# manhofer/Line3D

Hardware: AMD Instinct MI355X
Metric: segment-pair affinities/s (higher is better)
Workload: dtype f32

## Files before the change

### include/line3d_amd.h

```cpp
#ifndef LINE3D_AMD_H
#define LINE3D_AMD_H

#include <stddef.h>
#include <stdint.h>

#ifdef __cplusplus
extern "C" {
#endif

#define L3D_OK 0
#define L3D_ERR_INVALID 1
#define L3D_ERR_HIP 2
#define L3D_ERR_NOMEM 3
#define L3D_ERR_NODEVICE 4
#define L3D_ERR_UNSUPPORTED 5

#define L3D_RDD_MAX_ITER 10
#define L3D_DEF_COLLINEARITY_S 2.0f

typedef struct l3d_ctx l3d_ctx;

typedef struct l3d_match {
    uint32_t segID1;
    uint32_t camID2;
// ... 38 lines not shown

int l3d_replicator_dynamics_diffusion(l3d_ctx* ctx, const l3d_edge* A, int nnz, int n, int iters, l3d_edge* out);

int l3d_similarity_coll3D_batch(l3d_ctx* ctx, const l3d_hypothesis* hyp, int n_hyp,
                                const int32_t* pairs, int n_pairs, float sigma_a, float* sim);

typedef struct l3d_affinity_input {
    int32_t n_views;
    const int32_t* seg_base;
    const int32_t* view_hyp_begin;
    int32_t n_hyp;
    const l3d_hypothesis* hyp;
    const float* score;
    const int32_t* hyp_dense;
    const int32_t* best;
    const int64_t* pot_start;
    const int32_t* pot_tgt;
    const int64_t* coll_start;
    const int32_t* coll_other;
    const float* coll_w;
    float sigma_a;
} l3d_affinity_input;
int l3d_affinity_fill(l3d_ctx* ctx, const l3d_affinity_input* in, l3d_edge** edges, int* n_edges, int32_t** node_hyp, int* n_nodes,
                      int* n_candidates);
int l3d_last_fill_counts(l3d_ctx* ctx, int64_t* n_candidates, int64_t* n_passed);

int l3d_clustering_edges(l3d_ctx* ctx, const l3d_edge* A, int nnz, int n_nodes, int perform_diffusion, int iters, l3d_edge* sorted_out);
int l3d_clustering_edges_grouped(l3d_ctx* ctx, const l3d_edge* A, int nnz, int n_nodes, int perform_diffusion, int iters, l3d_edge* sorted_out,
                                 int32_t** group_start, int* n_groups);
int l3d_perform_clustering_device(l3d_ctx* ctx, const l3d_edge* A, int nnz, int n_nodes, int perform_diffusion, int iters, float c, int32_t* labels,
                                  int* n_components);

int l3d_fit_clusters(l3d_ctx* ctx, const int32_t* group_start, int n_groups, const int32_t* member_hyp, const l3d_hypothesis* hyp,
                     const uint32_t* hyp_cam, int n_hyp, const double* Rinv, double scale_inv, const double* tneg,
                     int32_t** seg_count, double** segs, int* n_segs);
int l3d_fit_labelled_clusters(l3d_ctx* ctx, const int32_t* labels, const int32_t* node_hyp, int n_nodes, const l3d_hypothesis* hyp,
                              const uint32_t* hyp_cam, int n_hyp, const double* Rinv, double scale_inv, const double* tneg,
                              int32_t** group_start, int32_t** member_hyp, int* n_groups, int32_t** seg_count, double** segs, int* n_segs);

typedef struct l3d_refine_params { int32_t max_iterations; int32_t pad; double huber_px; } l3d_refine_params;
int l3d_refine_lines(l3d_ctx* ctx, const int32_t* group_start, int n_groups, const int32_t* member_cam, const float* member_seg, const double* member_pts,
                     const double* cameras, int n_cameras, const l3d_refine_params* params, double* line, double* rms_before, double* rms_after,
                     int32_t* iterations, int32_t* status, int32_t** seg_count, double** segs, int* n_segs);
int l3d_test_refine_host(const int32_t* group_start, int n_groups, const int32_t* member_cam, const float* member_seg, const double* member_pts,
                         const double* cameras, int n_cameras, const l3d_refine_params* params, double* line, double* rms_before, double* rms_after,
                         int32_t* iterations, int32_t* status, int32_t** seg_count, double** segs, int* n_segs);
const char* l3d_refine_last_error(void);


typedef struct l3d_chain_view {
    uint32_t view_id;
    const float* src_segs; int32_t S_src;
    const float* RtKinv_src; const float* C_src;
    const float* tgt_segs; int32_t n_tgt;
    const int32_t* offsets; int32_t N;
    const float* F; const float* RtKinv; const float* centers; const float* P;
    const int32_t* to_be_matched; int32_t n_tbm;
    const uint32_t* local2global;
    const int32_t* source_cam; const int32_t* source_index; int32_t n_sources;
    float sigma_p, sigma_a, spatial_k;
} l3d_chain_view;
typedef int (*l3d_chain_callback)(void* user, int index, int verified, const l3d_match* kept, int n_kept,
                                  const float* best_depths, int n_best, int n_candidates);
int l3d_match_chain(l3d_ctx* ctx, const l3d_chain_view* views, int n_views, l3d_chain_callback cb, void* user);

typedef struct l3d_dense_map {
    int32_t n_views;
    const uint32_t* view_ids;
    const int32_t* seg_base;
} l3d_dense_map;
typedef struct l3d_chain_summary {
    int32_t verified;
    int32_t n_kept;
    int64_t n_candidates;
    float median_depth;
    int32_t pad;
} l3d_chain_summary;
int l3d_match_chain_resident(l3d_ctx* ctx, const l3d_chain_view* views, int n_views, const l3d_dense_map* map,
                             l3d_chain_summary* summary, int64_t* n_pot);
int l3d_chain_kept_list(l3d_ctx* ctx, int index, l3d_match** out, int* n);
int l3d_chain_release_records(l3d_ctx* ctx);
int l3d_chain_records_digest(l3d_ctx* ctx, uint64_t* hash, int32_t* n_kept, int n);
int l3d_chain_products_get(l3d_ctx* ctx, int64_t* pot_start, int32_t* pot_tgt, l3d_match* best_match);

typedef struct l3d_view_geometry {
    double RtKinv[9];
    double C[3];
    float k_lower, k_upper;
    float median_depth;
    int32_t n_segments;
    const float* segments;
} l3d_view_geometry;
int l3d_products_hypotheses(l3d_ctx* ctx, const l3d_view_geometry* geometry, int n_views, int32_t* view_hyp_begin, int32_t** hyp_dense, int* n_hyp);
int l3d_affinity_fill_resident(l3d_ctx* ctx, const int64_t* coll_start, const int32_t* coll_other, const float* coll_w, int coll_changed,
                               float sigma_a, l3d_edge** edges, int* n_edges, int32_t** node_hyp, int* n_nodes, int* n_candidates);
int l3d_resident_edges_get(l3d_ctx* ctx, l3d_edge* out, int nnz);
int l3d_products_hypotheses_get(l3d_ctx* ctx, l3d_hypothesis* hyp, float* score);

typedef struct l3d_shard_chain l3d_shard_chain;
void* l3d_ctx_stream(l3d_ctx* ctx);
int l3d_shard_chain_open(l3d_ctx* ctx, const l3d_chain_view* views, int n_views, int rank, int world, int slot_records,
                         l3d_shard_chain** out, size_t* slot_bytes);
int l3d_shard_chain_enqueue(l3d_shard_chain* chain, int k, void* send_slot, const void* gathered_base);
int l3d_shard_chain_mark(l3d_shard_chain* chain, int k);
int l3d_shard_chain_fetch(l3d_shard_chain* chain, int k, l3d_chain_callback cb, void* user);
int l3d_shard_chain_close(l3d_shard_chain* chain);
typedef int (*l3d_exchange_fn)(void* user, int view, const void* send_slot, void* recv_block, size_t slot_bytes, int world, void* stream);
typedef struct l3d_rccl_link { void* comm; void* all_gather; } l3d_rccl_link;
int l3d_shard_chain_run(l3d_shard_chain* chain, l3d_exchange_fn exchange, void* exchange_user, l3d_chain_callback cb, void* cb_user);
int l3d_exchange_rccl(void* user, int view, const void* send_slot, void* recv_block, size_t slot_bytes, int world, void* stream);
int l3d_exchange_local(void* user, int view, const void* send_slot, void* recv_block, size_t slot_bytes, int world, void* stream);
int l3d_exchange_replay(void* user, int view, const void* send_slot, void* recv_block, size_t slot_bytes, int world, void* stream);
const void* l3d_shard_chain_gathered(l3d_shard_chain* chain);
typedef struct l3d_node_comm l3d_node_comm;
int l3d_node_comm_create(const int* devices, int n, l3d_node_comm** out);
void l3d_node_comm_destroy(l3d_node_comm* comm);
int l3d_node_comm_bind(l3d_node_comm* comm, int rank, void* stream);
void l3d_node_comm_abort(l3d_node_comm* comm);
int l3d_exchange_node(void* user, int view, const void* send_slot, void* recv_block, size_t slot_bytes, int world, void* stream);
int l3d_shard_chain_products(l3d_shard_chain* chain, const l3d_dense_map* map, l3d_chain_summary* summary, int64_t* n_pot);
int l3d_shard_chain_info(l3d_shard_chain* chain, size_t* cand_cap, int* slot_records, int* overflow_bits, int* max_candidates, int* max_kept);
long long l3d_shard_chain_arena_needed(l3d_shard_chain* chain);
int l3d_shard_chain_partition(l3d_shard_chain* chain, int own_begin, int own_end);
int l3d_partition_keep_views(const l3d_chain_view* views, int n_views, int own_begin, int own_end, unsigned char* keep, int* reach);
int l3d_turn_handover_plan(const l3d_chain_view* views, int n_views, int world, int32_t* out, int32_t* info);

int l3d_match_chain_blocks(l3d_ctx* ctx, const l3d_chain_view* views, int n_views, const l3d_dense_map* map, l3d_chain_summary* summary, int64_t* n_pot,
                           int rank, int world, int warmup_views, int window, l3d_exchange_fn exchange, void* exchange_user, int* verdict);

int l3d_match_chain_partition(l3d_ctx* ctx, const l3d_chain_view* views, int n_views, const l3d_dense_map* map, l3d_chain_summary* summary, int64_t* n_pot,
                              int rank, int world, int warmup_views, int window, l3d_exchange_fn exchange, void* exchange_user, int* verdict);
int l3d_partition_info(l3d_ctx* ctx, int info[10], int64_t* n_pot_all);
int l3d_affinity_fill_sharded(l3d_ctx* ctx, const int64_t* coll_start, const int32_t* coll_other, const float* coll_w, int coll_changed, float sigma_a,
                              l3d_exchange_fn exchange, void* exchange_user, int* n_edges, int32_t** node_hyp, int* n_nodes,
                              int64_t* n_candidates_all, int32_t* view_hyp_begin_global, int32_t** hyp_dense_global, int* n_hyp_global);

int l3d_register_segments(l3d_ctx* ctx, const float* segments, int n_segments);
int l3d_unregister_segments(l3d_ctx* ctx, const float* segments);
int l3d_register_segments_batch(l3d_ctx* ctx, const float* const* arrays, const int* n_segments, int n_arrays);

int l3d_set_verify_mode(l3d_ctx* ctx, int mode);
int l3d_set_pair_pretest(l3d_ctx* ctx, int mask);
int l3d_set_option(l3d_ctx* ctx, const char* name, int value);
int l3d_get_option(l3d_ctx* ctx, const char* name, int* value);
int l3d_set_verify_lds_budget(size_t bytes);
int l3d_set_chain_capacities(l3d_ctx* ctx, size_t cand_cap, size_t arena_cap);
int l3d_warm_up(l3d_ctx* ctx);
int l3d_reserve_hint(l3d_ctx* ctx, int n_dense, int n_views, int n_neighbors);
int l3d_profile_enable(l3d_ctx* ctx, int on);
int l3d_profile_only(l3d_ctx* ctx, const char* kernel);
int l3d_profile_reset(l3d_ctx* ctx);
int l3d_profile_get(l3d_ctx* ctx, const char* kernel, int64_t* launches, double* total_ms);
const char* l3d_profile_names(void);
int l3d_last_stats(l3d_ctx* ctx, double stats[4]);

int l3d_test_contract_math(l3d_ctx* ctx, const float* x, int n, float* out_expf, float* out_acosf, double* out_acos);
int l3d_test_sq_threshold(l3d_ctx* ctx, const float* u, int n, float* out_walk, float* out_closed);
int l3d_test_exclusive_sum(l3d_ctx* ctx, const int32_t* in, int n, int32_t* out);

typedef struct l3d_line3d l3d_line3d;

int l3d_line3d_create(int device, int matching_neighbors, float uncertainty_t_upper_2D, float uncertainty_t_lower_2D,
                      float sigma_p, float sigma_a, float min_baseline, int use_collinearity, int verbose,
                      l3d_line3d** out);
int l3d_line3d_create_node(const int* devices, int n_devices, int matching_neighbors, float uncertainty_t_upper_2D, float uncertainty_t_lower_2D,
                           float sigma_p, float sigma_a, float min_baseline, int use_collinearity, int verbose, l3d_line3d** out);
// ... 305 lines not shown
```

### line3d_amd/capi.py

```python
from __future__ import annotations

import ctypes as C
import os

import numpy as np

_HERE = os.path.dirname(os.path.abspath(__file__))
LIB_PATH = os.path.join(_HERE, "libline3d_amd.so")
if os.environ.get("L3D_LIBRARY"):
    LIB_PATH = os.environ["L3D_LIBRARY"]

MATCH_DTYPE = np.dtype([("segID1", "<u4"), ("camID2", "<u4"), ("segID2", "<u4"),
                        ("depths", "<f4", (4,)), ("confidence", "<f4")])
EDGE_DTYPE = np.dtype([("i", "<i4"), ("j", "<i4"), ("w", "<f4")])
HYP_DTYPE = np.dtype([("P1", "<f8", (3,)), ("P2", "<f8", (3,)), ("dir", "<f8", (3,)),
                      ("depth_p1", "<f4"), ("depth_p2", "<f4"),
                      ("k_lower", "<f4"), ("k_upper", "<f4"), ("median_depth", "<f4"), ("pad", "<u4")])
REGION_DTYPE = np.dtype([("minpix", "<u4"), ("n_used", "<i4"), ("steps", "<i4"), ("pts", "<i4"), ("alg", "<i4"), ("scored", "<i4"), ("accepted", "<i4"),
                         ("pad", "<i4"), ("hist_n", "<i4", (8,))] + [(k, "<f8") for k in ("cx", "cy", "x1", "y1", "x2", "y2", "width", "theta", "density",
                                                                "fx1", "fy1", "fx2", "fy2", "fwidth", "p", "nfa")])
assert MATCH_DTYPE.itemsize == 32 and EDGE_DTYPE.itemsize == 12 and HYP_DTYPE.itemsize == 96 and REGION_DTYPE.itemsize == 192

_lib = None
_lib_check = None
# ... 811 lines not shown
               "bucket": np.zeros((M, N, 2), np.uint8)}
        n, m = C.c_int(0), C.c_int(0)
        self._chk(self.lib.l3d_test_detect_pixel_stage(self.h, pix, C.c_int(w), C.c_int(h), C.c_int(ch), C.c_size_t(stride), C.c_int(nw), C.c_int(nh),
                                                       _p(out["grey"]), _p(out["img"]), _p(out["mod"]), _p(out["ang"]), _p(out["bucket"]),
                                                       C.byref(n), C.byref(m)))
        if (n.value, m.value) != (N, M):
            raise L3DError("scaled size (%d, %d), expected (%d, %d)" % (n.value, m.value, N, M))
        return out

    def test_detect_label(self, bucket, active):
        bucket = np.ascontiguousarray(bucket, dtype=np.uint8)
        active = np.ascontiguousarray(active, dtype=np.uint8)
        M, N = active.shape
        assert bucket.shape == (M, N, 2)
        parent, key = np.zeros((2, M, N), np.int32), np.zeros((M, N), np.uint32)
        self._chk(self.lib.l3d_test_detect_label(self.h, _p(bucket), _p(active), C.c_int(N), C.c_int(M), _p(parent), _p(key)))
        return parent, key

    def test_detect_regions(self, mod, ang, key, min_reg):
        mod, ang = np.ascontiguousarray(mod, dtype=np.float64), np.ascontiguousarray(ang, dtype=np.float64)
        key = np.ascontiguousarray(key, dtype=np.uint32)
        M, N = key.shape
        assert mod.shape == (M, N) and ang.shape == (M, N)
        rec, n = C.c_void_p(), C.c_int(0)
        active = np.zeros((M, N), np.uint8)
        self._chk(self.lib.l3d_test_detect_regions(self.h, C.c_int(N), C.c_int(M), _p(mod), _p(ang), _p(key), C.c_int(int(min_reg)),
                                                   C.byref(rec), C.byref(n), _p(active)))
        out = np.zeros(n.value, dtype=REGION_DTYPE)
        if n.value:
            C.memmove(out.ctypes.data, rec, n.value * REGION_DTYPE.itemsize)
        self.lib.l3d_free(rec)
        return out, active

    def test_detect_nfa(self, n, k, p, logNT):
        n, k = np.ascontiguousarray(n, dtype=np.int32), np.ascontiguousarray(k, dtype=np.int32)
        p = np.ascontiguousarray(p, dtype=np.float64)
        out = np.zeros(len(n))
        self._chk(self.lib.l3d_test_detect_nfa(self.h, _p(n), _p(k), _p(p), C.c_double(float(logNT)), C.c_int(len(n)), _p(out)))
        return out

    def test_verify_candidates(self, src_segs, tgt_segs, offsets, P, RtKinv_src, C_src, row_start, cand_meta, cand_depths, sigma_p, sigma_a, spatial_k,
                               path=0, gb=0, split_unit=0, mmax=0, wide_max=0, seg_order=None):
        f = lambda a: np.ascontiguousarray(a, dtype=np.float32)
        src_segs, tgt_segs, P, RtKinv_src, C_src, cand_depths = f(src_segs), f(tgt_segs), f(P), f(RtKinv_src), f(C_src), f(cand_depths)
        offsets, row_start = np.ascontiguousarray(offsets, dtype=np.int32), np.ascontiguousarray(row_start, dtype=np.int32)
        cand_meta = np.ascontiguousarray(cand_meta, dtype=np.uint32)
        S, N, R, n_tgt = len(src_segs), len(offsets), len(cand_meta), len(tgt_segs.reshape(-1, 4))
        assert row_start.shape == (S * N + 1,) and cand_meta.shape == (R, 2) and cand_depths.shape == (R, 4) and P.size == N * 12
        sel = VerifyPath(int(path), int(gb), int(split_unit), int(mmax), int(wide_max), 0, 0, 0, None)
        if seg_order is not None:
            seg_order = np.ascontiguousarray(seg_order, dtype=np.int32)
            assert seg_order.shape == (S,)
            sel.seg_order = seg_order.ctypes.data
        conf, kept, best = np.zeros(R, np.float32), np.zeros(S, np.int32), np.zeros((S, 2), np.float32)
        self._chk(self.lib.l3d_test_verify_candidates(self.h, C.c_int(S), C.c_int(N), _p(src_segs), _p(tgt_segs), C.c_int(n_tgt), _p(offsets), _p(P),
                                                      _p(RtKinv_src), _p(C_src), _p(row_start), _p(cand_meta), _p(cand_depths), C.c_int(R),
                                                      C.c_float(float(sigma_p)), C.c_float(float(sigma_a)), C.c_float(float(spatial_k)), C.byref(sel),
                                                      _p(conf), _p(kept), _p(best)))
        return conf, kept, best, int(sel.mmax_used), int(sel.kernels)

    def test_pair_candidates(self, src_segs, tgt_segs, offsets, F, RtKinv, centers, RtKinv_src, C_src, to_be_matched, path=0, pretest=3, spb=0,
                             seg_range=None, ray_tables=None, cand_cap=0, capacity=0):
        f = lambda a: np.ascontiguousarray(a, dtype=np.float32)
        src_segs, tgt_segs, F, RtKinv, centers, RtKinv_src, C_src = f(src_segs), f(tgt_segs), f(F), f(RtKinv), f(centers), f(RtKinv_src), f(C_src)
        offsets, tbm = np.ascontiguousarray(offsets, dtype=np.int32), np.ascontiguousarray(to_be_matched, dtype=np.int32)
        S, N, n_tgt = len(src_segs.reshape(-1, 4)), len(offsets), len(tgt_segs.reshape(-1, 4))
        assert F.size == N * 9 and RtKinv.size == N * 9 and centers.size == N * 3 and RtKinv_src.size == 9 and C_src.size == 3
        s0, s1 = (0, S) if seg_range is None else seg_range
        if ray_tables is None:
            ray_tables = 1 if path in (1, 2) else 0
        sel = PairPath(int(path), int(pretest), int(spb), int(s0), int(s1), int(ray_tables), int(cand_cap), int(capacity))
        out = dict(row_upper=np.zeros(S * N, np.int32), row_count=np.zeros(S * N, np.int32), row_start=np.zeros(S * N + 1, np.int32),
                   cand_meta=np.zeros((int(capacity), 2), np.uint32), cand_depths=np.zeros((int(capacity), 4), np.float32))
        try:
            self._chk(self.lib.l3d_test_pair_candidates(self.h, C.c_int(S), C.c_int(N), _p(src_segs), _p(tgt_segs), C.c_int(n_tgt), _p(offsets), _p(F), _p(RtKinv),
                                                        _p(centers), _p(RtKinv_src), _p(C_src), _p(tbm), C.c_int(len(tbm)), C.byref(sel), _p(out["row_upper"]),
                                                        _p(out["row_count"]), _p(out["row_start"]), _p(out["cand_meta"]), _p(out["cand_depths"])))
        except L3DError as e:
            e.needed = int(sel.needed)
            raise
        out.update(total=int(sel.total), largest=int(sel.largest), spb_used=int(sel.spb_used), overflow=int(sel.overflow), needed=int(sel.needed))
        return out

    def chain_products_get(self, n_dense: int, n_pot: int, slack: int = 0):
        pot_start = np.zeros(n_dense + 1, np.int64)
        pot_tgt = np.full(n_pot + slack, -1, np.int32)
        best = np.zeros(n_dense, dtype=MATCH_DTYPE)
        self._chk(self.lib.l3d_chain_products_get(self.h, _p(pot_start), _p(pot_tgt), _p(best)))
        return pot_start, pot_tgt, best

    def test_products(self, views, view_ids, seg_base, side_arrays=0, early_pairs=0, rows=None, held=None, slack=64, max_blocks=1024):
        n = len(views)
        arr, keep = (ChainView * max(1, n))(), []
        for k, v in enumerate(views):
            l2g = np.ascontiguousarray(v["l2g"], dtype=np.uint32)
            sc, si = np.ascontiguousarray(v["source_cam"], dtype=np.int32), np.ascontiguousarray(v["source_index"], dtype=np.int32)
            assert len(sc) == len(si)
            keep += [l2g, sc, si]
            e = arr[k]
            e.view_id, e.S_src, e.N, e.n_tbm, e.n_sources = int(v["id"]), int(v["S"]), len(l2g), int(v["n_tbm"]), len(sc)
            e.local2global, e.source_cam, e.source_index = l2g.ctypes.data, sc.ctypes.data, si.ctypes.data
        kept = [np.ascontiguousarray(v["kept"], dtype=MATCH_DTYPE) for v in views]
        n_kept = np.array([len(a) for a in kept], np.int32)
        kept_all = np.concatenate(kept) if n else np.zeros(0, MATCH_DTYPE)
        R = np.array([int(v["R"]) for v in views], np.int64)
        best = np.ascontiguousarray(np.concatenate([np.asarray(v["best"], np.float32).reshape(-1, 2) for v in views]), dtype=np.float32)
        bestpos = np.ascontiguousarray(np.concatenate([np.asarray(v["bestpos"], np.int32).reshape(-1) for v in views]), dtype=np.int32)
        assert len(best) == len(bestpos) == sum(int(v["S"]) for v in views)
        ids, sb = np.ascontiguousarray(view_ids, dtype=np.uint32), np.ascontiguousarray(seg_base, dtype=np.int32)
        assert len(sb) == len(ids) + 1
        dm = DenseMap(len(ids), ids.ctypes.data, sb.ctypes.data)
        blk = [np.full(max_blocks, -9, np.int32) for _ in range(3)]
        sel = ProductsPath()
        sel.side_arrays, sel.early_pairs = int(side_arrays), int(early_pairs)
        sel.dv0, sel.dv1 = (0, -1) if rows is None else (int(rows[0]), int(rows[1]))
        hb = None if held is None else np.ascontiguousarray(held, dtype=np.uint8)
        assert hb is None or len(hb) == n
        sel.held = None if hb is None else hb.ctypes.data
        sel.block_capacity = max_blocks
        sel.block_cap, sel.block_staged, sel.block_g = (b.ctypes.data for b in blk)
        summary = np.zeros(max(1, n), dtype=SUMMARY_DTYPE)
        n_pot = C.c_int64(0)
        self._chk(self.lib.l3d_test_products(self.h, arr, C.c_int(n), C.byref(dm), _p(kept_all), _p(n_kept), _p(R), _p(best), _p(bestpos), C.byref(sel),
                                             _p(summary), C.byref(n_pot)))
        nd = int(sb[-1])
        pot_start, pot_tgt, bm = self.chain_products_get(nd, n_pot.value, slack)
        nb = min(max_blocks, int(sel.n_blocks)) if sel.build == PROD_TRANSPOSED else 0
        report = dict(side_arrays_used=int(sel.side_arrays_used), build=int(sel.build), refused=int(sel.refused), n_blocks=int(sel.n_blocks),
                      max_touch=int(sel.max_touch), early_cap=int(sel.early_cap), early_g=int(sel.early_g),
                      block_cap=blk[0][:nb].tolist(), block_staged=blk[1][:nb].tolist(), block_g=blk[2][:nb].tolist())
        return dict(pot_start=pot_start, pot_tgt=pot_tgt, best=bm, n_pot=int(n_pot.value), summary=summary[:n], report=report)

    def compute_collinearity(self, segs, collin_s=2.0):
        segs = np.ascontiguousarray(segs, dtype=np.float32)
        oi, oj, ow = C.POINTER(C.c_int32)(), C.POINTER(C.c_int32)(), C.POINTER(C.c_float)()
        n = C.c_int(0)
        self._chk(self.lib.l3d_compute_collinearity(self.h, _p(segs), C.c_int(len(segs)), C.c_float(collin_s),
                                                    C.byref(oi), C.byref(oj), C.byref(ow), C.byref(n)))
        k = n.value
        i = np.ctypeslib.as_array(oi, (k,)).copy() if k else np.zeros(0, np.int32)
        j = np.ctypeslib.as_array(oj, (k,)).copy() if k else np.zeros(0, np.int32)
        w = np.ctypeslib.as_array(ow, (k,)).copy() if k else np.zeros(0, np.float32)
        for p in (oi, oj, ow):
            self.lib.l3d_free(p)
        return i, j, w

    def compute_collinearity_batch(self, seg_sets, collin_s=2.0):
        sets = [np.ascontiguousarray(s, dtype=np.float32).reshape(-1, 4) for s in seg_sets]
        n = len(sets)
        ptrs = (C.c_void_p * max(n, 1))(*[s.ctypes.data for s in sets])
        ns = np.array([len(s) for s in sets], np.int32)
        start = np.zeros(n + 1, np.int32)
        oi, oj, ow = C.POINTER(C.c_int32)(), C.POINTER(C.c_int32)(), C.POINTER(C.c_float)()
        self._chk(self.lib.l3d_compute_collinearity_batch(self.h, ptrs, _p(ns), C.c_int(n), C.c_float(collin_s),
                                                          C.byref(oi), C.byref(oj), C.byref(ow), _p(start)))
        total = int(start[n])
        i = np.ctypeslib.as_array(oi, (total,)).copy() if total else np.zeros(0, np.int32)
        j = np.ctypeslib.as_array(oj, (total,)).copy() if total else np.zeros(0, np.int32)
        w = np.ctypeslib.as_array(ow, (total,)).copy() if total else np.zeros(0, np.float32)
        for p in (oi, oj, ow):
            self.lib.l3d_free(p)
        return [(i[start[v]:start[v + 1]], j[start[v]:start[v + 1]], w[start[v]:start[v + 1]]) for v in range(n)]

    def compute_pairwise_matches(self, src_segs, RtKinv_src, C_src, tgt_segs, offsets, F, RtKinv, centers, P,
                                 to_be_matched, in_matches, local2global, k_upper, k_lower, sigma_p, sigma_a,
                                 spatial_k, median_depth=1.0, seg_range=None, want_best=False):
# ... 221 lines not shown
```

### line3d_amd/csrc/l3d_chain.hip

```cpp
#include <algorithm>
#include <condition_variable>
#include <deque>
#include <mutex>
#include <thread>
#include <vector>

#include "l3d_ctx.hpp"
#include "l3d_scan.hpp"
#include "l3d_kept.hpp"
#include "l3d_products.hpp"
#include "l3d_chain_common.hpp"
#include "l3d_chain_partition.hpp"
#include "l3d_runtable.hpp"

#ifndef L3D_AHEAD
#define L3D_AHEAD 4
#define L3D_S1AHEAD 8
#endif

using namespace l3d;

namespace l3d {

constexpr int kLongList = 262144;
// ... 494 lines not shown
            launch_early_transposes(c, reinterpret_cast<const EarlyView*>(PE.e_tab.as<int>() + (size_t)n_views * maxN * 2), early_next, k + 1 - early_next, maxN, early_maxSt, dres, cams, PE.e_cnt.as<int>(),
                                    PE.e_poff.as<unsigned>(), PE.e_boff.as<int>(), PE.e_E.as<unsigned>(), PE.e_T.as<unsigned>(), avg_run, sp);
            early_next = k + 1;
        }
        return L3D_OK;
    };

    const double t_loop0 = now_s();
    double kept_total = 0, t_cb = 0, t_wait = 0, t_d2h = 0;
    struct Item { int k; int verified; ChainResult r; };
    std::mutex mu;
    std::condition_variable cv_work, cv_idle;
    std::deque<Item> work;
    bool done = false, busy = false;
    int deliver_rc = L3D_OK;
    std::string deliver_err;
    std::thread deliverer([&]() {
        if (!cb) return;
        (void)hipSetDevice(c->device);
        for (;;) {
            Item it;
            {
                std::unique_lock<std::mutex> lk(mu);
                cv_work.wait(lk, [&]() { return done || !work.empty(); });
                if (work.empty()) return;
                it = work.front();
                work.pop_front();
                busy = true;
            }
            int rc = L3D_OK;
            std::string err;
            if (deliver_rc == L3D_OK) {
                const l3d_chain_view& v = views[it.k];
                const ViewDev& d = vd[(size_t)it.k];
                if (!it.verified) {
                    if (cb(user, it.k, 0, nullptr, 0, nullptr, 0, 0)) { rc = L3D_ERR_INVALID; err = "callback failed"; }
                } else {
                    const double td0 = now_s();
                    hipError_t e = hipSuccess;
                    l3d_match* kept_host = static_cast<l3d_match*>(c->pin_arena.alloc((size_t)it.r.n_kept * sizeof(Match) + 16, &e));
                    if (e == hipSuccess) e = c->ch_pin_best.reserve((size_t)v.S_src * 8 + 16);
                    if (e == hipSuccess && it.r.n_kept)
                        e = hipMemcpyAsync(kept_host, c->ch_kept.as<Match>() + it.r.kept_base, (size_t)it.r.n_kept * sizeof(Match), hipMemcpyDeviceToHost, c->copy_stream);
                    if (e == hipSuccess && v.S_src) e = hipMemcpyAsync(c->ch_pin_best.p, d.best, (size_t)v.S_src * 8, hipMemcpyDeviceToHost, c->copy_stream);
                    if (e == hipSuccess) e = hipStreamSynchronize(c->copy_stream);
                    if (e != hipSuccess) { rc = L3D_ERR_HIP; err = std::string("chain delivery, view ") + std::to_string(it.k) + ": " + hipGetErrorString(e); }
                    else {
                        float* best = c->ch_pin_best.as<float>();
                        int nb = 0;
                        if (it.r.R > 0)
                            for (int s = 0; s < v.S_src; ++s)
                                if (best[2 * s] != -1.0f) { best[2 * nb] = best[2 * s]; best[2 * nb + 1] = best[2 * s + 1]; ++nb; }
                        kept_total += it.r.n_kept;
                        const double tc0 = now_s();
                        t_d2h += tc0 - td0;
                        if (cb(user, it.k, 1, kept_host, it.r.n_kept, best, nb, it.r.R)) { rc = L3D_ERR_INVALID; err = "callback failed"; }
                        t_cb += now_s() - tc0;
                    }
                }
            }
            {
                std::lock_guard<std::mutex> lk(mu);
                if (rc && deliver_rc == L3D_OK) { deliver_rc = rc; deliver_err = err; }
                busy = false;
            }
            cv_idle.notify_all();
        }
    });
    auto hand_over = [&](int k, int verified, const ChainResult& r) {
        if (!cb) { if (verified) kept_total += r.n_kept; return; }
        { std::lock_guard<std::mutex> lk(mu); work.push_back(Item{ k, verified, r }); }
        cv_work.notify_one();
    };
    auto wait_delivered = [&]() {
        if (!cb) return;
        std::unique_lock<std::mutex> lk(mu);
        cv_idle.wait(lk, [&]() { return work.empty() && !busy; });
    };
    auto hip_ok = [&](hipError_t e, const char* what) {
        if (e == hipSuccess) return true;
        rc_final = fail(c, L3D_ERR_HIP, std::string(what) + ": " + hipGetErrorString(e));
        return false;
    };
    for (int k = 0; k < n_views && rc_final == L3D_OK; ++k) {
        while (k_enq < n_views && k_enq <= k + kAhead) { int rc = enqueue_view(k_enq); if (rc) { rc_final = rc; break; } ++k_enq; }
        if (rc_final) break;
        { std::lock_guard<std::mutex> lk(mu); if (deliver_rc) break; }
        const ViewDev& d = vd[(size_t)k];
        if (!d.verified) { hand_over(k, 0, ChainResult()); continue; }
        const double tw0 = now_s();
        if (!hip_ok(hipEventSynchronize(ev[(size_t)k]), "hipEventSynchronize")) break;
        t_wait += now_s() - tw0;
        const ChainResult r = hres[k];
        if (r.overflow) {
            if (!hip_ok(hipStreamSynchronize(st), "hipStreamSynchronize") || !hip_ok(hipStreamSynchronize(s1), "hipStreamSynchronize")) break;
            if (sp && !hip_ok(hipStreamSynchronize(sp), "hipStreamSynchronize")) break;
            const double t_restart0 = now_s();
            wait_delivered();
            if (r.overflow & 1) cand_cap = (size_t)r.R + (size_t)r.R / 4 + 65536;
            if (r.overflow & 2) {
                size_t new_cap = arena_cap * 2;
                const int n_pre = pre ? pre->k1 - pre->k0 : 0, done = k - k_begin + n_pre, span = k_end - k_begin + n_pre;
                if (done >= 4) {
                    const size_t proj = (size_t)((double)r.kept_base / done * span * (2 * done < span ? 1.5 : 1.15)) + 1048576;
                    new_cap = 2 * done < span ? std::max(new_cap, proj) : std::max(proj, arena_cap + arena_cap / 8);
                }
                const size_t need = (size_t)r.kept_base + (size_t)std::max(0, r.n_want) + 65536;
                new_cap = std::max(new_cap, need);
                {
                    size_t fr = 0, tot = 0;
                    if (hipMemGetInfo(&fr, &tot) == hipSuccess) {
                        if (c->opt.regrow_free_mb > 0) fr = std::min(fr, (size_t)c->opt.regrow_free_mb << 20);
                        const size_t per_rec = sizeof(Match) + 4 + (early && new_cap < 0x7ffffff0ull ? 4 : 0) + (map ? 8 : 0);
                        const size_t reserve = turn_room ? 0 : map ? (size_t)((1ll << 28) * 24) + ((size_t)1 << 30) : (size_t)512 << 20;
                        const size_t fits = turn_room ? turn_room : fr > reserve ? (fr - reserve) / per_rec : 0;
                        if (new_cap > fits) {
                            if (fits < need || fits <= arena_cap) {
                                rc_final = fail(c, L3D_ERR_NOMEM, "match_chain: the kept arena of " + std::to_string(arena_cap) + " records is full at view " + std::to_string(k) + " of " + std::to_string(n_views) + " (" +
                                                                      std::to_string((size_t)r.kept_base) + " records in use, the view keeps " + std::to_string(r.n_want) + ") and an arena of " +
                                                                      std::to_string(need) + " records does not fit beside it (room for " + std::to_string(fits) + " at " + std::to_string(per_rec) + " B per record, " +
                                                                      std::to_string(reserve >> 20) + " MB kept back; " + std::to_string(fr >> 20) + " of " + std::to_string(tot >> 20) +
                                                                      " MB free): l3d_set_chain_capacities sizes the arena up front");
                                break;
                            }
                            new_cap = fits;
                        }
                    }
                    (void)hipGetLastError();
                }
                void* np = nullptr;
                const double t_m0 = now_s();
                {
                    const hipError_t me = hipMalloc(&np, new_cap * sizeof(Match));
                    if (me != hipSuccess) {
                        size_t fr = 0, tot = 0;
                        (void)hipMemGetInfo(&fr, &tot);
                        rc_final = fail(c, L3D_ERR_NOMEM, "match_chain: growing the kept arena to " + std::to_string(new_cap * sizeof(Match) >> 20) + " MB at view " + std::to_string(k) + " of " + std::to_string(n_views) +
                                                          " (" + std::to_string((size_t)r.kept_base * sizeof(Match) >> 20) + " MB in use, " + std::to_string(fr >> 20) + " of " + std::to_string(tot >> 20) + " MB free): " + hipGetErrorString(me));
                        break;
                    }
                }
                const double t_m1 = now_s();
                if (!hip_ok(hipMemcpy(np, c->ch_kept.p, (size_t)r.kept_base * sizeof(Match), hipMemcpyDeviceToDevice), "hipMemcpy")) break;
                const double t_m2 = now_s();
                (void)hipFree(c->ch_kept.p);
                if (c->opt.timing) fprintf(stderr, "[l3d match_chain]   arena of %zu MB: hipMalloc %.2f ms, copy of %zu MB %.2f ms, hipFree of the old one %.2f ms\n", new_cap * sizeof(Match) >> 20, (t_m1 - t_m0) * 1e3,
                                           (size_t)r.kept_base * sizeof(Match) >> 20, (t_m2 - t_m1) * 1e3, (now_s() - t_m2) * 1e3);
                c->ch_kept.p = np; c->ch_kept.cap = new_cap * sizeof(Match);
                {
                    void* nc = nullptr;
                    if (!hip_ok(hipMalloc(&nc, new_cap * 4 + 64), "hipMalloc (side words of the kept arena)")) break;
                    if (!hip_ok(hipMemcpy(nc, c->ch_keptcam.p, (size_t)r.kept_base * 4, hipMemcpyDeviceToDevice), "hipMemcpy")) { (void)hipFree(nc); break; }
                    (void)hipFree(c->ch_keptcam.p);
                    c->ch_keptcam.p = nc; c->ch_keptcam.cap = new_cap * 4 + 64;
                }
                if (early && new_cap < 0x7ffffff0ull) {
                    void* ne = nullptr;
                    if (!hip_ok(hipMalloc(&ne, new_cap * 4 + 64), "hipMalloc (transposed entries of the kept arena)")) break;
                    if (!hip_ok(hipMemcpy(ne, PE.e_E.p, (size_t)r.kept_base * 4, hipMemcpyDeviceToDevice), "hipMemcpy")) { (void)hipFree(ne); break; }
                    (void)hipFree(PE.e_E.p);
                    PE.e_E.p = ne; PE.e_E.cap = new_cap * 4 + 64;
                }
                arena_cap = new_cap;
            }
            { int rc = reserve_caps(); if (rc) { rc_final = rc; break; } }
            if (c->opt.timing) fprintf(stderr, "[l3d match_chain] view %d of %d overflowed (%d): candidates %zu, arena %zu records; regrown in %.2f ms, %.2f ms into the loop\n", k, n_views, r.overflow, cand_cap, arena_cap,
                                       (now_s() - t_restart0) * 1e3, (now_s() - t_loop0) * 1e3);
            for (int j = k; j < k_p1; ++j) {
                if (!vd[(size_t)j].verified || views[j].S_src == 0) continue;
                if (j < k_enq) {
                    if (!hip_ok(hipMemsetAsync(vd[(size_t)j].rowcnt, 0, (size_t)views[j].S_src * views[j].N * 4, st), "hipMemsetAsync")) break;
                    if (!fused_rows) launch_row_count(pair_args(j), vd[(size_t)j].rowcnt, st);
                }
                enqueue_fillA(j, st);
            }
            if (rc_final) break;
            k_enq = k;
            early_next = std::min(early_next, k);
            --k;
            continue;
        }
        raw_sum += r.R;
        kept_seen += r.n_kept; views_seen += 1;
        hand_over(k, 1, r);
    }
    { std::lock_guard<std::mutex> lk(mu); done = true; }
    cv_work.notify_one();
    deliverer.join();
    if (rc_final == L3D_OK && deliver_rc) rc_final = fail(c, deliver_rc, deliver_err);
    const double t_prod0 = now_s();
    if (rc_final == L3D_OK && map) {
        std::vector<ProdChainView> pv((size_t)n_views);
        for (int k = 0; k < n_views; ++k) pv[(size_t)k] = ProdChainView{ vd[(size_t)k].verified ? vd[(size_t)k].best : nullptr, vd[(size_t)k].verified ? vd[(size_t)k].bestpos : nullptr, vd[(size_t)k].verified ? 1 : 0,
                                                                         vd[(size_t)k].verified ? vd[(size_t)k].rt : nullptr };
        ProdEarly pe;
        const bool early_done = early && arena_cap < 0x7ffffff0ull;
        if (early_done) {
            if (early_next < n_views) {
                const double avg_run = views_seen > 0 ? kept_seen / views_seen / std::max(1.0, (double)L.maxS * std::max(1, maxN)) : 1.0;
                launch_early_transposes(c, reinterpret_cast<const EarlyView*>(PE.e_tab.as<int>() + (size_t)n_views * maxN * 2), early_next, n_views - early_next, maxN, early_maxSt, c->ch_res.as<ChainResult>(),
                                        c->ch_keptcam.as<unsigned>(), PE.e_cnt.as<int>(), PE.e_poff.as<unsigned>(), PE.e_boff.as<int>(), PE.e_E.as<unsigned>(), PE.e_T.as<unsigned>(), avg_run, st);
                early_next = n_views;
            }
            hipEvent_t e = get_local_event(c);
            (void)hipEventRecord(e, sp);
            (void)hipStreamWaitEvent(st, e, 0);
            put_local_event(c, e);
            pe.pcnt_kq = PE.e_cnt.as<int>(); pe.poff_kq = PE.e_poff.as<unsigned>(); pe.boff = PE.e_boff.as<int>(); pe.E = PE.e_E.as<unsigned>();
            pe.boff_off_host = PE.e_boff_off.data(); pe.maxN = maxN;
        }
        rc_final = build_products(c, views, n_views, pv.data(), hres, map, summary, n_pot, 0, -1, nullptr, c->ch_keptcam.as<unsigned>(), early_done ? &pe : nullptr);
    }
    if (c->opt.timing)
        fprintf(stderr, "[l3d match_chain] setup %.2f ms | enqueue + watch loop %.2f ms (waiting: view results %.2f, stage-1 statistics %.2f) | delivery thread: d2h %.2f, callback %.2f\n",
                (t_loop0 - t_setup0) * 1e3, (t_prod0 - t_loop0) * 1e3, t_wait * 1e3, t_ev1 * 1e3, t_d2h * 1e3, t_cb * 1e3);
    if (c->opt.timing && map) fprintf(stderr, "[l3d match_chain] products on the device %.2f ms\n", (now_s() - t_prod0) * 1e3);
    const double t_tail0 = now_s();
    (void)hipStreamSynchronize(s1);
    if (sp) (void)hipStreamSynchronize(sp);
    (void)hipStreamSynchronize(st);
    if (c->opt.timing) fprintf(stderr, "[l3d match_chain] hipSetDevice %.3f ms, final syncs %.3f ms\n", (t_setup0 - t_enter) * 1e3, (now_s() - t_tail0) * 1e3);
    for (hipEvent_t e : ev) { if (cb) put_event(c, e); else put_local_event(c, e); }
    for (hipEvent_t e : ev1) put_local_event(c, e);
    c->stats[1] = raw_sum;
    c->stats[3] = kept_total;
    if (rc_final == L3D_OK && !c->test_cand_cap && !c->test_arena_cap) {
        c->chain_seen_views = n_views; c->chain_seen_pairs = pairs; c->chain_seen_cand_cap = cand_cap; c->chain_seen_arena_cap = arena_cap; c->chain_seen_kept = kept_seen;
    }
    return rc_final;
}

extern "C" int l3d_match_chain(l3d_ctx* c, const l3d_chain_view* views, int n_views, l3d_chain_callback cb, void* user)
{
    if (c && n_views > 0 && !cb) return fail(c, L3D_ERR_INVALID, "l3d_match_chain: bad argument");
    return run_chain(c, views, n_views, cb, user, nullptr, nullptr, nullptr);
}

extern "C" int l3d_match_chain_resident(l3d_ctx* c, const l3d_chain_view* views, int n_views, const l3d_dense_map* map, l3d_chain_summary* summary, int64_t* n_pot)
{
    if (!c) return L3D_ERR_INVALID;
    if (!map || !map->view_ids || !map->seg_base || map->n_views < 0 || (n_views > 0 && !summary)) return fail(c, L3D_ERR_INVALID, "l3d_match_chain_resident: bad argument");
    if (n_pot) *n_pot = 0;
    return run_chain(c, views, n_views, nullptr, nullptr, map, summary, n_pot);
}

void l3d::warm_chain() { touch_kernel(reinterpret_cast<const void*>(&k_exist_count)); }
```

### line3d_amd/csrc/l3d_ctx.hpp

```cpp
#pragma once

#include <algorithm>
#include <chrono>
#include <cstdio>
#include <cstdlib>
#include <cstring>
#include <map>
#include <mutex>
#include <string>
#include <unordered_map>
#include <vector>

#include "../../include/line3d_amd.h"
#include "l3d_kernels.hpp"
#include "l3d_options.hpp"

namespace l3d {

struct DevBuf {
    void* p = nullptr;
    size_t cap = 0;
    hipError_t reserve(size_t bytes)
    {
        if (bytes <= cap) return hipSuccess;
        if (p) { hipError_t e = hipFree(p); p = nullptr; cap = 0; if (e != hipSuccess) return e; }
        size_t want = bytes + bytes / 4 + 256;
        hipError_t e = hipMalloc(&p, want);
        if (e == hipSuccess) cap = want;
        return e;
    }
    hipError_t reserve_exact(size_t bytes)
    {
        if (bytes <= cap) return hipSuccess;
        if (p) { hipError_t e = hipFree(p); p = nullptr; cap = 0; if (e != hipSuccess) return e; }
        hipError_t e = hipMalloc(&p, bytes + 256);
        if (e == hipSuccess) cap = bytes + 256;
        return e;
    }
    template <class T> T* as() const { return reinterpret_cast<T*>(p); }
    void release() { if (p) (void)hipFree(p); p = nullptr; cap = 0; }
};

struct PinBuf {
    void* p = nullptr;
    size_t cap = 0;
    unsigned flags = hipHostMallocDefault;
    hipError_t reserve(size_t bytes)
    {
        if (bytes <= cap) return hipSuccess;
        if (p) { (void)hipHostFree(p); p = nullptr; cap = 0; }
        size_t want = bytes + bytes / 2 + 4096;
        hipError_t e = hipHostMalloc(&p, want, flags);
        if (e == hipSuccess) cap = want;
        return e;
    }
    template <class T> T* as() const { return reinterpret_cast<T*>(p); }
    void release() { if (p) (void)hipHostFree(p); p = nullptr; cap = 0; }
};

struct PinArena {
    static constexpr size_t kChunk = 64u << 20;
    std::vector<PinBuf> chunks;
    size_t cur = 0, used = 0;
    void reset() { cur = 0; used = 0; }
    void* alloc(size_t bytes, hipError_t* err)
    {
        *err = hipSuccess;
        bytes = (bytes + 255) & ~(size_t)255;
        for (;;) {
            if (cur < chunks.size()) {
                if (used + bytes <= chunks[cur].cap) { void* r = static_cast<char*>(chunks[cur].p) + used; used += bytes; return r; }
                ++cur; used = 0;
                continue;
            }
            chunks.emplace_back();
            *err = chunks.back().reserve(std::max(bytes, kChunk));
            if (*err != hipSuccess) { chunks.pop_back(); return nullptr; }
        }
    }
    void release() { for (auto& b : chunks) b.release(); chunks.clear(); reset(); }
};

struct ProductsPart {
    bool active = false;
    int rank = 0, world = 1;
    int own_dv0 = 0, own_dv1 = 0;
    int row_dv0 = 0, row_dv1 = 0;
    int held_dv0 = 0, held_dv1 = 0;
    long long n_pot_all = 0;
    int recovery_rounds = 0;
    int blocks_rerun = 0;
};

struct ProductsReport {
    int build = 0;
    int refused = 0;
    int n_blocks = 0, max_touch = 0;
    int early_cap = -1, early_g = -1;
    std::vector<int> block_cap, block_staged, block_g;
};

struct Products {
    bool valid = false, hyp_valid = false;
    ProductsPart part;
    ProductsReport report;
    int n_dense = 0, n_views_all = 0, n_chain = 0, n_hyp = 0;
    long long n_pot = 0, total_kept = 0;
    DevBuf keys, keys2, flag, pos, tmp, pot_start, pot_tgt, best_ref, median, tables, ttab, rowstage, tstage;
    DevBuf e_cnt, e_poff, e_boff, e_E, e_T, e_tab;
    std::vector<int> e_boff_off;
    DevBuf geo, hyp_of, score, hyp_dense, best_hyp, coll, aux;
    long long coll_n = 0;
    unsigned long long coll_sig = 0;
    std::vector<int> seg_base;
    std::vector<unsigned> view_ids;
    std::vector<l3d::ChainResult> res;
    std::vector<int> chain_view;
    std::vector<char> chain_verified;
    std::vector<int> view_hyp_begin;
    std::vector<std::vector<int>> early_src_index, early_src_cam;
    std::vector<unsigned> chain_view_id;
    void release()
    {
        DevBuf* b[] = { &keys, &keys2, &flag, &pos, &tmp, &pot_start, &pot_tgt, &best_ref, &median, &tables, &ttab, &rowstage, &tstage, &e_cnt, &e_poff, &e_boff, &e_E, &e_T, &e_tab, &geo, &hyp_of, &score, &hyp_dense, &best_hyp, &coll, &aux };
        for (DevBuf* x : b) x->release();
        valid = hyp_valid = false; coll_n = 0; coll_sig = 0;
    }
};

struct FillPart { int h0 = 0, h1 = 0; unsigned long long pos_base = 0; const int* loc2glob = nullptr; int assume_symmetric = 0; };

struct DetectBufs {
    DevBuf lens;
    DevBuf rflags, smask, valid;
    DevBuf vgrey, vaux, vimg, vdef;
    DevBuf pixels, undist, grey, aux, img, mod, ang, bucket, active, parent, size, count, keys, keys2, vals, vals2, flag, pos, start, tmp, cand, ckeys, ckeys2, cvals, cvals2, cimg, cimg2, prm, out, ktab, scal;
    DevBuf jcoef, jplanes;
    PinBuf jstage;
    DevBuf ingest;
    std::vector<unsigned char> ingest_host;
    hipEvent_t dev_event = nullptr;
    int tab_w = 0, tab_h = 0;
    int vdef_n = 0, vdef_m = 0;
    void release()
    {
        for (DevBuf* x : all()) x->release();
        jstage.release();
        if (dev_event) { (void)hipEventDestroy(dev_event); dev_event = nullptr; }
        tab_w = tab_h = 0;
        vdef_n = vdef_m = 0;
    }
    size_t held()
    {
        size_t n = 0;
        for (DevBuf* x : all()) n += x->cap;
        return n;
    }
    std::vector<DevBuf*> all()
    {
        return { &pixels, &undist, &grey, &aux, &img, &mod, &ang, &bucket, &active, &parent, &size, &count, &keys, &keys2, &vals, &vals2, &flag, &pos, &start, &tmp, &cand, &ckeys, &ckeys2, &cvals, &cvals2, &cimg, &cimg2, &prm, &out, &ktab, &scal, &jcoef, &jplanes, &ingest, &lens, &rflags, &smask, &valid, &vgrey, &vaux, &vimg, &vdef };
    }
};

struct ProfEntry {
    std::vector<std::pair<hipEvent_t, hipEvent_t>> pending;
    int64_t launches = 0;
    double ms = 0.0;
};

}

struct l3d_ctx {
    int device = 0;
    l3d::Options opt;
    hipStream_t stream = nullptr;
    hipStream_t copy_stream = nullptr;
    hipStream_t prod_stream = nullptr;
    hipStream_t stage1_stream = nullptr;
    std::string err;
    std::mutex err_mu;
    l3d::DevBuf src_segs, tgt_segs, tables, tbm, l2g, exist, mask, rowcnt, row_start, cand_meta, cand_depths, cand_conf;
    l3d::DevBuf kept_cnt, kept_start, best, kept, scal, stamps, vw_scratch;
    l3d::PinBuf pin_tab, pin_ex, pin_scal, pin_best, pin_kept;
    l3d::DevBuf ch_tables, ch_mask, ch_rowcnt, ch_cursor, ch_best, ch_kept, ch_keptcam, ch_res, ch_flags, ch_send, ch_gathered, ch_stage, ch_rowA, ch_ringA_meta, ch_ringA_depths, ch_segorder, ch_rays, ch_rt, ch_rtinfo, ch_rtjobs, ch_existpart;
    l3d::PinBuf ch_pin_tables, ch_pin_res, ch_pin_kept, ch_pin_best;
    l3d::DevBuf ch_hdr;
    l3d::DevBuf ch_bestpos;
    l3d::Products products;
    l3d::DetectBufs det;
    std::vector<l3d::RayJob> ray_jobs;
    l3d::PinArena pin_arena;
    std::vector<int> h_cnt;
    int mmax_seen = 0;
    l3d::DevBuf vw_bstart, vw_segstate;
    size_t part_arena_seen = 0;
    bool turn_share = false;
    bool fill_collective_only = false;
    void (*fill_gate)(void*, int) = nullptr;
    void* fill_gate_user = nullptr;
    size_t turn_arena_room = 0;
    bool records_released = false;
    std::vector<int> shard_view_kept;
    size_t test_cand_cap = 0, test_arena_cap = 0;
    int chain_seen_views = 0; double chain_seen_pairs = 0; size_t chain_seen_cand_cap = 0, chain_seen_arena_cap = 0; double chain_seen_kept = 0;
    unsigned long long* pair_dbg = nullptr;
    int wedge_pretest = 3;
    int verify_mode = 0;
    l3d::DevBuf g0, g1, g2, g3, g4, g5, g6, g7;
// ... 129 lines not shown
```

### line3d_amd/csrc/l3d_products.hip

```cpp
#include "l3d_sort.hpp"

#include <algorithm>
#include <vector>

#include "l3d_products.hpp"
#include "l3d_linalg.hpp"
#include "l3d_unproject.hpp"
#include "l3d_runtable.hpp"

using namespace l3d;

namespace l3d {

struct ProdView {
    long long kept_base;
    int n_kept, R;
    int dense_base, S;
    int early, pad;
    const int* bestpos;
    const float2* best;
};
struct ProdBlock {
    int d0, d1;
    long long slots;
// ... 322 lines not shown
    const ChainResult r = res[v.k];
    const int St = v.St[q];
    unsigned long long off = r.kept_base;
    for (int j = 0; j < q; ++j) off += (unsigned)pcnt_kq[(size_t)v.k * maxN + j];
    if (threadIdx.x == 0) poff_kq[(size_t)v.k * maxN + q] = (unsigned)off;
    if (r.overflow || r.n_kept == 0 || St <= 0) return;
    pair_transpose_wg(qt_arena + r.kept_base, v.rt + (size_t)q * v.S, v.rt + (size_t)(q + 1) * v.S, v.S, St, g, boff + v.boff_off[q], E + off, T ? T + off : nullptr, cap, s_h, s_w, &s_kb);
}

template <int MODE>
__global__ __launch_bounds__(256) void k_prod_early_rt(const ProdView* __restrict__ pv, const ProdViewQ* __restrict__ vq, const ProdSrc* __restrict__ ps, const int* __restrict__ ps_slot,
                                                       const int* __restrict__ src_list, int d0, int d1, int* __restrict__ cnt, const int* __restrict__ bstart,
                                                       unsigned* __restrict__ ent, unsigned long long* __restrict__ best_ref, int* __restrict__ list_len)
{
    const int q = src_list ? src_list[blockIdx.y] : (int)blockIdx.y;
    const ProdSrc e = ps[q];
    const int slot = ps_slot[q];
    if (slot < 0 || (MODE != 0 && e.alias_base < 0)) return;
    const ProdView v = pv[e.view], s = pv[e.src];
    const ProdViewQ sq = vq[e.src];
    if (!sq.rt || s.n_kept == 0) return;
    const int* r0 = sq.rt + (size_t)slot * s.S;
    const int* r1 = r0 + s.S;
    constexpr int g = 16;
    const int grp = threadIdx.x / g, gl = threadIdx.x % g, ngrp = 256 / g;
    int n_mine = 0;
    for (int sg = blockIdx.x * ngrp + grp; sg < s.S; sg += gridDim.x * ngrp) {
        const int ra = r0[sg], rb = r1[sg];
        for (int i = ra + gl; i < rb; i += g) {
            const unsigned w = sq.qt[i];
            const int u = (int)(w & 0xffffu);
            if (MODE == 0) {
                ++n_mine;
                if (u < v.S && !e.pad) atomicMin(&best_ref[v.dense_base + u], ((unsigned long long)e.rank << 40) | (unsigned long long)(s.kept_base + i));
            } else if (u < v.S && sg < e.alias_S) {
                const int ai = v.dense_base + u, di = e.alias_base + sg;
                if (ai >= d0 && ai < d1) {
                    if (MODE == 1) atomicAdd(&cnt[ai - d0], 1);
                    else ent[bstart[ai - d0] + atomicSub(&cnt[ai - d0], 1) - 1] = (unsigned)di;
                }
                if (di >= d0 && di < d1) {
                    if (MODE == 1) atomicAdd(&cnt[di - d0], 1);
                    else ent[bstart[di - d0] + atomicSub(&cnt[di - d0], 1) - 1] = (unsigned)ai;
                }
            }
        }
    }
    if (MODE == 0) {
        for (int d = 32; d > 0; d >>= 1) n_mine += __shfl_down(n_mine, d);
        if ((threadIdx.x & 63) == 0 && n_mine) atomicAdd(&list_len[e.view], n_mine);
    }
}

template <bool SCATTER>
__global__ __launch_bounds__(256) void k_prodt_early(const Match* __restrict__ arena, const ProdView* __restrict__ pv, const ProdSrc* __restrict__ ps,
                                                     const int* __restrict__ src_list, const unsigned* __restrict__ chain_view_id, int d0, int d1, int* __restrict__ cnt,
                                                     const int* __restrict__ bstart, unsigned* __restrict__ ent)
{
    const int q = src_list[blockIdx.y];
    const ProdSrc e = ps[q];
    if (e.alias_base < 0) return;
    const ProdView v = pv[e.view], s = pv[e.src];
    const unsigned vid = chain_view_id[e.view];
    for (int i = blockIdx.x * 256 + threadIdx.x; i < s.n_kept; i += gridDim.x * 256) {
        const Match r = arena[s.kept_base + i];
        if (r.camID2 != vid || (int)r.segID2 >= v.S || (int)r.segID1 >= e.alias_S) continue;
        const int ai = v.dense_base + (int)r.segID2, di = e.alias_base + (int)r.segID1;
        if (ai >= d0 && ai < d1) {
            if (!SCATTER) atomicAdd(&cnt[ai - d0], 1);
            else ent[bstart[ai - d0] + atomicSub(&cnt[ai - d0], 1) - 1] = (unsigned)di;
        }
        if (di >= d0 && di < d1) {
            if (!SCATTER) atomicAdd(&cnt[di - d0], 1);
            else ent[bstart[di - d0] + atomicSub(&cnt[di - d0], 1) - 1] = (unsigned)ai;
        }
    }
}

template <bool WRITE>
__global__ __launch_bounds__(256) void k_prodv_rows(const ProdRowView* __restrict__ rv, int x0, int d0, const ProdViewQ* __restrict__ vq, const ProdTouch* __restrict__ tl,
                                                    const ProdPair* __restrict__ pairs, const int* __restrict__ poff, const int* __restrict__ boff, const unsigned* __restrict__ E,
                                                    const int* __restrict__ bstart, const unsigned* __restrict__ ent, int* __restrict__ ucnt, const int* __restrict__ ustart,
                                                    long long base, int* __restrict__ pot_tgt, int* __restrict__ stage,
                                                    const unsigned* __restrict__ poff_kq, int maxN)
{
    constexpr int kWords = 512;
    __shared__ unsigned s_bm[4][kWords];
    const int wave = threadIdx.x >> 6, lane = threadIdx.x & 63;
    const ProdRowView v = rv[x0 + blockIdx.y];
    const int u = blockIdx.x * 4 + wave;
    if (u >= v.S) return;
    unsigned* bm = s_bm[wave];
    const int row = v.dense_base + u - d0;
    const unsigned* fq = nullptr;
    const int* frt = nullptr;
    if (v.own_k >= 0) { const ProdViewQ o = vq[v.own_k]; if (o.rt) { fq = o.qt; frt = o.rt; } }
    const int e0 = bstart ? bstart[row] : 0, ne = bstart ? bstart[row + 1] - e0 : 0;
    int total = 0;
    long long o = WRITE ? base + ustart[row] : 0;
    if (!WRITE && stage && lane == 63) stage[(size_t)row * 64 + 63] = 0;
    if (WRITE && stage && stage[(size_t)row * 64 + 63] == -2) {
        const int n = ustart[row + 1] - ustart[row];
        if (lane < n) pot_tgt[o + lane] = stage[(size_t)row * 64 + lane];
        return;
    }
    for (int t0 = v.t0; t0 < v.t1; t0 += 64) {
        const int j = t0 + lane;
        ProdTouch e;
        e.y_base = 0; e.y_S = 0; e.fq = -1; e.pair = -1;
        int f_a = 0, f_n = 0, b_a = 0, b_n = 0;
        if (j < v.t1) {
            e = tl[j];
            if (e.fq >= 0 && frt) { f_a = frt[(size_t)e.fq * v.S + u]; f_n = frt[(size_t)(e.fq + 1) * v.S + u] - f_a; }
            if (e.pair >= 0) {
                const ProdPair pr = pairs[e.pair];
                const int* bo = boff + pr.off_off;
                const int a = bo[u];
                b_n = bo[u + 1] - a;
                b_a = (poff_kq ? (int)poff_kq[(size_t)pr.k * maxN + pr.q] : poff[e.pair]) + a;
            }
        }
        const int cnt = min(64, v.t1 - t0);
        if (v.t1 - v.t0 <= 64) {
            const int mine = f_n + b_n;
            int incl = mine;
            for (int d = 1; d < 64; d <<= 1) { const int x = __shfl_up(incl, d); if (lane >= d) incl += x; }
            const int excl = incl - mine, tot = __shfl(incl, 63);
            if (tot + ne <= 64) {
                int id = 0x7fffffff;
                int l = 0;
                for (int step = 32; step > 0; step >>= 1) { const int cand = l + step; const int ex = __shfl(excl, cand & 63); if (cand < 64 && ex <= lane) l = cand; }
                const int off = lane - __shfl(excl, l), ofn = __shfl(f_n, l), ofa = __shfl(f_a, l), oba = __shfl(b_a, l), oyS = __shfl(e.y_S, l), oyb = __shfl(e.y_base, l);
                if (lane < tot) {
                    const unsigned t = off < ofn ? (fq[ofa + off] & 0xffffu) : E[oba + off - ofn];
                    if ((int)t < oyS) id = oyb + (int)t;
                } else if (lane < tot + ne) id = (int)ent[e0 + lane - tot];
                int rank = 0;
                for (int k = 0; k < 64; ++k) { const int other = __shfl(id, k); rank += (other < id || (other == id && k < lane)) ? 1 : 0; }
                const int sorted = __builtin_amdgcn_ds_permute(rank << 2, id);
                const int before = __shfl_up(sorted, 1);
                const bool keep = sorted != 0x7fffffff && (lane == 0 || before != sorted);
                const unsigned long long km = __ballot(keep);
                if (!WRITE) {
                    const int n = __popcll(km);
                    if (lane == 0) ucnt[row] = n;
                    if (stage && n < 64) {
                        if (keep) stage[(size_t)row * 64 + __popcll(km & ((1ull << lane) - 1ull))] = sorted;
                        if (lane == 63) stage[(size_t)row * 64 + 63] = -2;
                    }
                }
                else if (keep) pot_tgt[o + __popcll(km & ((1ull << lane) - 1ull))] = sorted;
                return;
            }
        }
        for (int k = 0; k < cnt; ++k) {
            const int fn = __shfl(f_n, k), bn = __shfl(b_n, k);
            if (fn + bn + ne == 0) continue;
            const int fa = __shfl(f_a, k), ba = __shfl(b_a, k), yS = __shfl(e.y_S, k), yb = __shfl(e.y_base, k);
            const int nw = (yS + 31) >> 5;
            for (int w = lane; w < nw; w += 64) bm[w] = 0u;
            __builtin_amdgcn_fence(__ATOMIC_SEQ_CST, "workgroup");
            __builtin_amdgcn_wave_barrier();
            for (int i = lane; i < fn; i += 64) { const unsigned t = fq[fa + i] & 0xffffu; if ((int)t < yS) atomicOr(&bm[t >> 5], 1u << (t & 31u)); }
            for (int i = lane; i < bn; i += 64) { const unsigned t = E[ba + i]; if ((int)t < yS) atomicOr(&bm[t >> 5], 1u << (t & 31u)); }
            for (int i = lane; i < ne; i += 64) { const unsigned t = ent[e0 + i] - (unsigned)yb; if (t < (unsigned)yS) atomicOr(&bm[t >> 5], 1u << (t & 31u)); }
            __builtin_amdgcn_fence(__ATOMIC_SEQ_CST, "workgroup");
            __builtin_amdgcn_wave_barrier();
            if (!WRITE) {
                for (int w = lane; w < nw; w += 64) total += __popc(bm[w]);
            } else {
                for (int wb = 0; wb < nw; wb += 64) {
                    const int w = wb + lane;
                    unsigned word = w < nw ? bm[w] : 0u;
                    if (__ballot(word != 0u) == 0ull) continue;
                    const int pc = __popc(word);
                    int incl = pc;
                    for (int d = 1; d < 64; d <<= 1) { const int x = __shfl_up(incl, d); if (lane >= d) incl += x; }
                    long long p = o + (incl - pc);
                    while (word) { const int bit = __ffs(word) - 1; pot_tgt[p++] = yb + (w << 5) + bit; word &= word - 1u; }
                    o += __shfl(incl, 63);
                }
            }
            __builtin_amdgcn_fence(__ATOMIC_SEQ_CST, "workgroup");
            __builtin_amdgcn_wave_barrier();
        }
    }
    if (!WRITE) {
        for (int d = 32; d > 0; d >>= 1) total += __shfl_down(total, d);
        if (lane == 0) ucnt[row] = total;
    }
}

__global__ __launch_bounds__(256) void k_prodt_row_starts(const int* __restrict__ ustart, int rows, long long base, long long* __restrict__ pot_start_at)
{
    const int r = blockIdx.x * 256 + threadIdx.x;
    if (r <= rows) pot_start_at[r] = base + ustart[r];
}

}

namespace {

int bits_for(int n) { int b = 1; while ((1ll << b) <= (long long)n) ++b; return b; }

}

void l3d::launch_prod_shift_rows(const long long* piece, long long n_rows, long long base, long long* pot_start_at, hipStream_t st)
{
    if (n_rows > 0) hipLaunchKernelGGL(k_prod_shift_rows, dim3((unsigned)((n_rows + 255) / 256)), dim3(256), 0, st, piece, n_rows, base, pot_start_at);
}

void l3d::launch_early_transposes(l3d_ctx* c, const EarlyView* views_dev, int k0, int nb, int maxN, int maxSt, const ChainResult* res,
                                  const unsigned* qt_arena, int* pcnt_kq, unsigned* poff_kq, int* boff, unsigned* E, unsigned* T, double avg_run, hipStream_t st)
{
    if (maxN <= 0 || nb <= 0) return;
    int g = 1;
    while (g < 64 && g < avg_run / 4.0) g <<= 1;
    if (c->opt.prod_pair_g >= 0) g = c->opt.prod_pair_g;
    int cap = 0;
    if (T) {
        cap = 12288;
        while (cap > 1024 && ((size_t)maxSt + 2 + 2 * (size_t)cap) * 4 > 64 * 1024) cap -= 1024;
        if (((size_t)maxSt + 2 + 2 * (size_t)cap) * 4 > 64 * 1024) cap = 0;
    }
    c->products.report.early_cap = cap; c->products.report.early_g = g;
    ProfScope p(c, "prod_keys", st);
    hipLaunchKernelGGL(k_prode_counts, dim3((unsigned)maxN, (unsigned)nb), dim3(256), 0, st, views_dev, k0, maxN, res, pcnt_kq);
    hipLaunchKernelGGL(k_prode_transpose, dim3((unsigned)maxN, (unsigned)nb), dim3(kPairThreads), ((size_t)maxSt + 2 + 2 * (size_t)cap) * 4, st, views_dev, k0, maxN, res, qt_arena, (const int*)pcnt_kq, poff_kq, g,
                       boff, E, cap ? T : (unsigned*)nullptr, cap);
}

int l3d::build_products(l3d_ctx* c, const l3d_chain_view* views, int n_views, const ProdChainView* pvh, const ChainResult* hres,
                        const l3d_dense_map* map, l3d_chain_summary* summary, int64_t* n_pot_out, int dv0, int dv1, const char* held, const unsigned* qt_arena, const ProdEarly* early)
{
    Products& P = c->products;
    P.valid = false; P.hyp_valid = false;
    c->records_released = false;
    ProductsReport& rep = P.report;
    rep.build = 0; rep.refused = 0; rep.n_blocks = 0; rep.max_touch = 0;
    rep.block_cap.clear(); rep.block_staged.clear(); rep.block_g.clear();
    hipStream_t st = c->stream;
    const int nv = map->n_views;
    if (nv <= 0) return fail(c, L3D_ERR_INVALID, "products: empty dense map");
    for (int i = 0; i < nv; ++i) {
        if (map->seg_base[i + 1] < map->seg_base[i] || (i && map->view_ids[i] <= map->view_ids[i - 1]) || map->seg_base[0] != 0)
            return fail(c, L3D_ERR_INVALID, "products: the dense map must ascend");
    }
    const int nd = map->seg_base[nv];
    if (nd <= 0) return fail(c, L3D_ERR_INVALID, "products: no segments");
    const bool partial = dv1 >= 0;
    if (!partial) { dv0 = 0; dv1 = nv; }
    if (dv0 < 0 || dv1 > nv || dv0 > dv1) return fail(c, L3D_ERR_INVALID, "products: bad view range");
    P.seg_base.assign(map->seg_base, map->seg_base + nv + 1);
    P.view_ids.assign(map->view_ids, map->view_ids + nv);
    P.res.assign(hres, hres + n_views);
    P.n_dense = nd; P.n_views_all = nv; P.n_chain = n_views;
    P.chain_view.assign((size_t)n_views, -1);
    P.chain_verified.assign((size_t)n_views, 0);
    for (int k = 0; k < n_views; ++k) P.chain_verified[(size_t)k] = pvh[k].verified ? 1 : 0;
    P.chain_view_id.resize((size_t)n_views);
    P.early_src_index.assign((size_t)n_views, {}); P.early_src_cam.assign((size_t)n_views, {});
    auto view_of = [&](unsigned id) { auto it = std::lower_bound(P.view_ids.begin(), P.view_ids.end(), id); return it != P.view_ids.end() && *it == id ? (int)(it - P.view_ids.begin()) : -1; };

    std::vector<ProdView> pv((size_t)n_views);
    std::vector<ProdSrc> ps;
    std::vector<int> ps_alias_view;
    long long total_kept = 0, early_slots = 0;
    for (int k = 0; k < n_views; ++k) if (pvh[k].verified) total_kept = std::max(total_kept, (long long)hres[k].kept_base + hres[k].n_kept);
    if (total_kept > kBestIndexMask) return fail(c, L3D_ERR_UNSUPPORTED, "products: " + std::to_string(total_kept) + " kept matches in the arena -- best-match references hold 40-bit positions");
    int max_kept = 0, maxS = 1;
    for (int k = 0; k < n_views; ++k) {
        const l3d_chain_view& v = views[k];
        const int vi = view_of(v.view_id);
        if (vi < 0 || P.seg_base[(size_t)vi + 1] - P.seg_base[(size_t)vi] != v.S_src) return fail(c, L3D_ERR_INVALID, "products: a chain view is missing from the dense map");
        P.chain_view[(size_t)k] = vi; P.chain_view_id[(size_t)k] = v.view_id;
        ProdView& o = pv[(size_t)k];
        o.kept_base = pvh[k].verified ? hres[k].kept_base : 0; o.n_kept = pvh[k].verified ? hres[k].n_kept : 0; o.R = pvh[k].verified ? hres[k].R : 0;
        o.dense_base = P.seg_base[(size_t)vi]; o.S = v.S_src; o.early = pvh[k].verified ? 0 : 1; o.pad = 0;
        o.bestpos = pvh[k].bestpos; o.best = pvh[k].best;
        max_kept = std::max(max_kept, o.n_kept); maxS = std::max(maxS, o.S);
        if (!pvh[k].verified) {
            P.early_src_index[(size_t)k].assign(v.source_index, v.source_index + v.n_sources);
            P.early_src_cam[(size_t)k].assign(v.source_cam, v.source_cam + v.n_sources);
            for (int q = 0; q < v.n_sources; ++q) {
                const int si = v.source_index[q];
                if (si < 0 || si >= k || !pvh[si].verified) continue;
                ProdSrc e;
                e.view = k; e.src = si; e.rank = q; e.pad = 0;
                const int av = view_of((unsigned)v.source_cam[q]);
                e.alias_base = av >= 0 ? P.seg_base[(size_t)av] : -1; e.alias_S = av >= 0 ? P.seg_base[(size_t)av + 1] - P.seg_base[(size_t)av] : 0;
                e.out_off = 0;
                early_slots += 2 * (long long)hres[si].n_kept;
                ps.push_back(e);
                ps_alias_view.push_back(av);
            }
        }
    }
    const long long slots_all = 2 * total_kept + early_slots;
    const int nb = bits_for(nd);
    P.total_kept = total_kept;

    std::vector<std::vector<int>> touch_view((size_t)nv), touch_src((size_t)nv);
    for (int k = 0; k < n_views; ++k) {
        if (!pvh[k].verified || hres[k].n_kept == 0) continue;
        touch_view[(size_t)P.chain_view[(size_t)k]].push_back(k);
        for (int q = 0; q < views[k].N; ++q) {
            const int t = view_of(views[k].local2global[q]);
            if (t >= 0 && t != P.chain_view[(size_t)k]) touch_view[(size_t)t].push_back(k);
        }
    }
    for (size_t q = 0; q < ps.size(); ++q) {
        if (hres[ps[q].src].n_kept == 0) continue;
        const int a = P.chain_view[(size_t)ps[q].view], b = ps_alias_view[q];
        touch_src[(size_t)a].push_back((int)q);
        if (b >= 0 && b != a) touch_src[(size_t)b].push_back((int)q);
    }
    long long budget = 1ll << 28;
    if (c->opt.prod_block_keys > 0) budget = c->opt.prod_block_keys;
    else if (slots_all > budget) {
        size_t fr = 0, tot = 0;
        if (hipMemGetInfo(&fr, &tot) == hipSuccess) budget = std::max(budget, std::min<long long>((long long)(fr / 4 / 24), (1ll << 30) - 64));
    }
    std::vector<ProdBlock> blocks;
    std::vector<long long> off_tab;
    auto plan_blocks = [&]() -> int {
        blocks.clear(); off_tab.clear();
        std::vector<int> mark_v((size_t)n_views, -1), mark_s(ps.size(), -1);
        int x = dv0;
        while (x < dv1) {
            const int bi = (int)blocks.size();
            ProdBlock B;
            B.d0 = P.seg_base[(size_t)x]; B.slots = 0;
            B.off_view = off_tab.size();
            off_tab.resize(off_tab.size() + (size_t)n_views + ps.size(), -1);
            B.off_src = B.off_view + (size_t)n_views;
            int x1 = x;
            for (; x1 < dv1; ++x1) {
                long long add = 0;
                for (int k : touch_view[(size_t)x1]) if (mark_v[(size_t)k] != bi) add += 2 * (long long)hres[k].n_kept;
                for (int q : touch_src[(size_t)x1]) if (mark_s[(size_t)q] != bi) add += 2 * (long long)hres[ps[(size_t)q].src].n_kept;
                if (x1 > x && B.slots + add > budget) break;
                for (int k : touch_view[(size_t)x1]) if (mark_v[(size_t)k] != bi) { mark_v[(size_t)k] = bi; off_tab[B.off_view + (size_t)k] = B.slots; B.slots += 2 * (long long)hres[k].n_kept; }
                for (int q : touch_src[(size_t)x1]) if (mark_s[(size_t)q] != bi) { mark_s[(size_t)q] = bi; off_tab[B.off_src + (size_t)q] = B.slots; B.slots += 2 * (long long)hres[ps[(size_t)q].src].n_kept; }
            }
            B.d1 = P.seg_base[(size_t)x1];
            if (B.slots > 0x7ffffff0ll) return fail(c, L3D_ERR_UNSUPPORTED, "products: one view and its neighbours hold more than 2^30 kept matches");
            blocks.push_back(B);
            x = x1;
        }
        return L3D_OK;
    };
    if (int rc = plan_blocks()) return rc;
    long long max_slots = 0;
    for (const ProdBlock& B : blocks) max_slots = std::max(max_slots, B.slots);
    long long n_keys_max = max_slots + 1;

    auto al = [](size_t b) { return (b + 255) & ~(size_t)255; };
    const size_t o_pv = 0, o_ps = o_pv + al(pv.size() * sizeof(ProdView)), o_ids = o_ps + al(ps.size() * sizeof(ProdSrc) + 16),
                 o_sb = o_ids + al((size_t)nv * 4), o_cv = o_sb + al((size_t)(nv + 1) * 4), o_off = o_cv + al((size_t)n_views * 4), o_evq = o_off + al(off_tab.size() * 8 + 16),
                 o_slot = o_evq + al((size_t)n_views * sizeof(ProdViewQ) + 16), tab_total = o_slot + al(ps.size() * 4 + 16);
    HIPCHK(c, P.tables.reserve(tab_total));
    bool native_rt = qt_arena != nullptr && c->opt.prod_transpose != 0;
    for (int k = 0; k < n_views; ++k) if (pvh[k].verified && hres[k].n_kept > 0 && !pvh[k].rt) native_rt = false;
    std::vector<ProdViewQ> evq((size_t)n_views);
    for (int k = 0; k < n_views; ++k) {
        const bool has = native_rt && pvh[k].verified && hres[k].n_kept > 0;
        evq[(size_t)k] = ProdViewQ{ has ? qt_arena + hres[k].kept_base : nullptr, has ? pvh[k].rt : nullptr, 0, views[k].N };
    }
    std::vector<int> ps_slot(ps.size() + 1, -1);
    for (size_t q = 0; q < ps.size(); ++q) {
        const l3d_chain_view& sv = views[ps[q].src];
        for (int j = 0; j < sv.N; ++j) if (sv.local2global[j] == P.chain_view_id[(size_t)ps[q].view]) { ps_slot[q] = j; break; }
    }
    char* tb = P.tables.as<char>();
    std::vector<char> tblob(tab_total);
    {
        auto put = [&](size_t off, const void* src, size_t bytes) { if (bytes) memcpy(tblob.data() + off, src, bytes); };
        put(o_pv, pv.data(), pv.size() * sizeof(ProdView)); put(o_ps, ps.data(), ps.size() * sizeof(ProdSrc)); put(o_ids, P.view_ids.data(), (size_t)nv * 4);
        put(o_sb, P.seg_base.data(), (size_t)(nv + 1) * 4); put(o_cv, P.chain_view_id.data(), (size_t)n_views * 4); put(o_off, off_tab.data(), off_tab.size() * 8);
        put(o_evq, evq.data(), evq.size() * sizeof(ProdViewQ)); put(o_slot, ps_slot.data(), ps_slot.size() * 4);
    }
    HIPCHK(c, hipMemcpyAsync(tb, tblob.data(), tblob.size(), hipMemcpyHostToDevice, st));
    const ProdView* dpv = reinterpret_cast<const ProdView*>(tb + o_pv);
    const ProdSrc* dps = reinterpret_cast<const ProdSrc*>(tb + o_ps);
    const unsigned* dids = reinterpret_cast<const unsigned*>(tb + o_ids);
    const int* dsb = reinterpret_cast<const int*>(tb + o_sb);
    const unsigned* dcv = reinterpret_cast<const unsigned*>(tb + o_cv);
    const long long* doff = reinterpret_cast<const long long*>(tb + o_off);
    const ProdViewQ* devq = reinterpret_cast<const ProdViewQ*>(tb + o_evq);
    const int* dslot = reinterpret_cast<const int*>(tb + o_slot);

    const double t_res0 = now_s();
    HIPCHK(c, P.pot_start.reserve(((size_t)nd + 2) * 8));
    HIPCHK(c, P.best_ref.reserve((size_t)nd * 8 + 64));
    HIPCHK(c, P.median.reserve((size_t)n_views * 8 + 64));
    if (c->opt.timing) fprintf(stderr, "[l3d products] %zu block(s) of up to %lld keys, table of up to %lld entries: buffers reserved in %.2f ms\n", blocks.size(), n_keys_max, slots_all, (now_s() - t_res0) * 1e3);
    int* d_list_len = reinterpret_cast<int*>(P.median.as<float>() + n_views);
    HIPCHK(c, hipMemsetAsync(d_list_len, 0, (size_t)n_views * 4, st));
    const Match* arena = c->ch_kept.as<Match>();
    HIPCHK(c, hipMemsetAsync(P.best_ref.p, 0xff, (size_t)nd * 8, st));
    const unsigned gx = (unsigned)std::max(1, std::min(512, (max_kept + 1023) / 1024));
    {
        ProfScope p(c, "prod_keys", st);
        if (!ps.empty() && native_rt)
            hipLaunchKernelGGL(HIP_KERNEL_NAME(k_prod_early_rt<0>), dim3((unsigned)std::max(1, std::min(256, (maxS + 15) / 16)), (unsigned)ps.size()), dim3(256), 0, st, dpv, devq, dps, dslot, (const int*)nullptr, 0, 0,
                               (int*)nullptr, (const int*)nullptr, (unsigned*)nullptr, P.best_ref.as<unsigned long long>(), d_list_len);
        else if (!ps.empty()) hipLaunchKernelGGL(k_prod_keys_early, dim3(gx, (unsigned)ps.size()), dim3(256), 0, st, arena, dpv, dps, (const long long*)nullptr, dcv, nb, 0, 0,
                                                 (unsigned long long*)nullptr, P.best_ref.as<unsigned long long>(), d_list_len);
        hipLaunchKernelGGL(k_prod_best, dim3((maxS + 255) / 256, n_views), dim3(256), 0, st, dpv, P.best_ref.as<long long>());
        hipLaunchKernelGGL(k_prod_median, dim3(n_views), dim3(256), 0, st, dpv, P.median.as<float>());
    }
    constexpr int kSortInstead = -12345;
    auto transposed = [&](long long& n_pot_out) -> int {
        const double t_t0 = now_s();
        auto seg_count = [&](int x) { return P.seg_base[(size_t)x + 1] - P.seg_base[(size_t)x]; };
        for (int x = dv0; x < dv1; ++x) if (seg_count(x) > 16000) { rep.refused = 1; return kSortInstead; }
        const bool rebuild = !native_rt;
        const bool use_early = early && !rebuild && early->E && early->boff && early->poff_kq;
        std::vector<int> nbv_off((size_t)n_views + 1, 0), nbv;
        for (int k = 0; k < n_views; ++k) {
            nbv_off[(size_t)k] = (int)nbv.size();
            if (pvh[k].verified) for (int q = 0; q < views[k].N; ++q) nbv.push_back(view_of(views[k].local2global[q]));
        }
        nbv_off[(size_t)n_views] = (int)nbv.size();
        std::vector<std::vector<int>> T((size_t)nv);
        for (int x = 0; x < nv; ++x) T[(size_t)x].reserve(32);
        for (int k = 0; k < n_views; ++k) {
            if (!pvh[k].verified) continue;
            const int vi = P.chain_view[(size_t)k];
            for (int q = 0; q < views[k].N; ++q) {
                const int t = nbv[(size_t)nbv_off[(size_t)k] + q];
                if (t >= 0) { T[(size_t)vi].push_back(t); T[(size_t)t].push_back(vi); }
            }
        }
        for (size_t q = 0; q < ps.size(); ++q) {
            const int a = P.chain_view[(size_t)ps[q].view], b = ps_alias_view[q];
            if (b >= 0) { T[(size_t)a].push_back(b); T[(size_t)b].push_back(a); }
        }
        for (int x = 0; x < nv; ++x) { std::vector<int>& t = T[(size_t)x]; std::sort(t.begin(), t.end()); t.erase(std::unique(t.begin(), t.end()), t.end()); }
        std::vector<int> nb_off((size_t)n_views, 0);
        std::vector<ProdNbQ> nbt;
        std::vector<unsigned> ids_sorted;
        std::vector<int> qs_sorted;
        std::vector<std::vector<ProdPair>> pairs_of((size_t)nv);
        std::vector<int> own_k((size_t)nv, -1);
        std::vector<std::pair<unsigned, int>> byid;
        nbt.reserve(nbv.size()); ids_sorted.reserve(nbv.size()); qs_sorted.reserve(nbv.size());
        for (int k = 0; k < n_views; ++k) {
            nb_off[(size_t)k] = (int)nbt.size();
            if (!pvh[k].verified) continue;
            const int vi = P.chain_view[(size_t)k], N = views[k].N;
            if (hres[k].n_kept > 0) own_k[(size_t)vi] = k;
            byid.clear();
            for (int q = 0; q < N; ++q) {
                const int t = nbv[(size_t)nbv_off[(size_t)k] + q];
                nbt.push_back(ProdNbQ{ t >= 0 ? P.seg_base[(size_t)t] : -1, t >= 0 ? seg_count(t) : 0 });
                byid.push_back({ views[k].local2global[q], q });
                if (t >= 0 && hres[k].n_kept > 0) pairs_of[(size_t)t].push_back(ProdPair{ k, q, 0, 0 });
            }
            std::sort(byid.begin(), byid.end());
            for (auto& e : byid) { ids_sorted.push_back(e.first); qs_sorted.push_back(e.second); }
        }
        std::vector<ProdRowView> rv((size_t)nv);
        std::vector<ProdPair> pairs;
        std::vector<ProdTouch> tl;
        pairs.reserve(nbv.size()); tl.reserve(2 * nbv.size() + 64);
        int max_touch = 0;
        for (int x = 0; x < nv; ++x) {
            ProdRowView& r = rv[(size_t)x];
            r.dense_base = P.seg_base[(size_t)x]; r.S = seg_count(x); r.own_k = own_k[(size_t)x]; r.t0 = r.t1 = 0; r.pad = 0;
            if (x < dv0 || x >= dv1) continue;
            const int pair0 = (int)pairs.size();
            for (const ProdPair& pr : pairs_of[(size_t)x]) pairs.push_back(pr);
            r.t0 = (int)tl.size();
            for (int y : T[(size_t)x]) {
                ProdTouch e;
                e.y_base = P.seg_base[(size_t)y]; e.y_S = seg_count(y); e.fq = -1; e.pair = -1;
                if (r.own_k >= 0) for (int q = 0; q < views[r.own_k].N; ++q) if (nbv[(size_t)nbv_off[(size_t)r.own_k] + q] == y) { e.fq = q; break; }
                for (int p = pair0; p < (int)pairs.size(); ++p) if (P.chain_view[(size_t)pairs[(size_t)p].k] == y) { e.pair = p; break; }
                tl.push_back(e);
            }
            r.t1 = (int)tl.size();
            max_touch = std::max(max_touch, r.t1 - r.t0);
        }
        rep.max_touch = max_touch;
        std::vector<int> pair_begin((size_t)nv + 1, 0);
        {
            int p = 0;
            for (int x = 0; x < nv; ++x) { pair_begin[(size_t)x] = p; if (x >= dv0 && x < dv1) p += (int)pairs_of[(size_t)x].size(); }
            pair_begin[(size_t)nv] = p;
        }
        struct TBlock { int x0, x1; size_t item0, n_items, src0, n_srcs; long long rec_n, rt_n, boff_n, early_n; int maxS, pair0, pair1; };
        std::vector<TBlock> tblocks;
        std::vector<int> items;
        std::vector<int> srcs;
        const long long t_budget = c->opt.prod_block_keys > 0 ? c->opt.prod_block_keys : (1ll << 30) - 64;
        {
            std::vector<int> mark_v((size_t)n_views, -1), mark_s(ps.size(), -1);
            int x = dv0;
            while (x < dv1) {
                const int bi = (int)tblocks.size();
                TBlock B;
                B.x0 = x; B.item0 = items.size(); B.src0 = srcs.size(); B.rec_n = 0; B.rt_n = 0; B.boff_n = 0; B.early_n = 0; B.maxS = 1; B.pair0 = pair_begin[(size_t)x];
                int x1 = x;
                for (; x1 < dv1; ++x1) {
                    long long add = 0;
                    for (int k : touch_view[(size_t)x1]) if (mark_v[(size_t)k] != bi) add += hres[k].n_kept;
                    for (int q : touch_src[(size_t)x1]) if (mark_s[(size_t)q] != bi) add += 2 * (long long)hres[ps[(size_t)q].src].n_kept;
                    if (x1 > x && B.rec_n + B.early_n + add > t_budget) break;
                    for (int k : touch_view[(size_t)x1]) if (mark_v[(size_t)k] != bi) {
                        mark_v[(size_t)k] = bi; items.push_back(k); B.rec_n += hres[k].n_kept; B.rt_n += ((long long)views[k].N + 1) * views[k].S_src;
                    }
                    for (int q : touch_src[(size_t)x1]) if (mark_s[(size_t)q] != bi) { mark_s[(size_t)q] = bi; srcs.push_back(q); B.early_n += 2 * (long long)hres[ps[(size_t)q].src].n_kept; }
                    B.maxS = std::max(B.maxS, seg_count(x1));
                    for (int p = pair_begin[(size_t)x1]; p < pair_begin[(size_t)x1 + 1]; ++p) {
                        if (use_early) { pairs[(size_t)p].off_off = early->boff_off_host[(size_t)pairs[(size_t)p].k * early->maxN + pairs[(size_t)p].q]; continue; }
                        pairs[(size_t)p].off_off = (int)B.boff_n; B.boff_n += seg_count(x1) + 1;
                    }
                }
                B.x1 = x1; B.n_items = items.size() - B.item0; B.n_srcs = srcs.size() - B.src0; B.pair1 = pair_begin[(size_t)x1];
                if (B.rec_n > 0x7ffffff0ll || B.early_n > 0x7ffffff0ll || B.boff_n > 0x7ffffff0ll || B.rt_n > 0x7ffffff0ll)
                    return fail(c, L3D_ERR_UNSUPPORTED, "products: one view and its neighbours hold more than 2^31 kept matches");
                tblocks.push_back(B);
                x = x1;
            }
        }
        long long max_rec = 0, max_rt = 0, max_boff = 0, max_early = 0;
        int max_rows = 0, max_pairs = 0;
        for (const TBlock& B : tblocks) {
            max_rec = std::max(max_rec, B.rec_n); max_rt = std::max(max_rt, B.rt_n); max_boff = std::max(max_boff, B.boff_n); max_early = std::max(max_early, B.early_n);
            max_rows = std::max(max_rows, P.seg_base[(size_t)B.x1] - P.seg_base[(size_t)B.x0]); max_pairs = std::max(max_pairs, B.pair1 - B.pair0);
        }
        std::vector<ProdViewQ> vqh((size_t)n_views);
        for (int k = 0; k < n_views; ++k) {
            ProdViewQ& o = vqh[(size_t)k];
            o.nb_off = nb_off[(size_t)k]; o.N = views[k].N;
            const bool has = pvh[k].verified && hres[k].n_kept > 0 && !rebuild;
            o.qt = has ? qt_arena + hres[k].kept_base : nullptr; o.rt = has ? pvh[k].rt : nullptr;
        }
        const size_t q_vq = 0, q_nb = q_vq + al(vqh.size() * sizeof(ProdViewQ) + 16), q_ids = q_nb + al(nbt.size() * sizeof(ProdNbQ) + 16), q_qs = q_ids + al(ids_sorted.size() * 4 + 16),
                     q_rv = q_qs + al(qs_sorted.size() * 4 + 16), q_tl = q_rv + al(rv.size() * sizeof(ProdRowView)), q_pr = q_tl + al(tl.size() * sizeof(ProdTouch) + 16),
                     q_sr = q_pr + al(pairs.size() * sizeof(ProdPair) + 16), q_job = q_sr + al(srcs.size() * 4 + 16), q_total = q_job + al((size_t)n_views * sizeof(RtJob) + 16);
        HIPCHK(c, P.ttab.reserve(q_total));
        char* tt = P.ttab.as<char>();
        std::vector<char> blob(q_job);
        auto put = [&](size_t off, const void* src, size_t bytes) { if (bytes) memcpy(blob.data() + off, src, bytes); };
        put(q_vq, vqh.data(), vqh.size() * sizeof(ProdViewQ)); put(q_nb, nbt.data(), nbt.size() * sizeof(ProdNbQ)); put(q_ids, ids_sorted.data(), ids_sorted.size() * 4);
        put(q_qs, qs_sorted.data(), qs_sorted.size() * 4); put(q_rv, rv.data(), rv.size() * sizeof(ProdRowView)); put(q_tl, tl.data(), tl.size() * sizeof(ProdTouch));
        put(q_pr, pairs.data(), pairs.size() * sizeof(ProdPair)); put(q_sr, srcs.data(), srcs.size() * 4);
        HIPCHK(c, hipMemcpyAsync(tt, blob.data(), blob.size(), hipMemcpyHostToDevice, st));
        const ProdViewQ* dvq = reinterpret_cast<const ProdViewQ*>(tt + q_vq);
        const ProdNbQ* dnb = reinterpret_cast<const ProdNbQ*>(tt + q_nb);
        const unsigned* dids = reinterpret_cast<const unsigned*>(tt + q_ids);
        const int* dqs = reinterpret_cast<const int*>(tt + q_qs);
        const ProdRowView* drv = reinterpret_cast<const ProdRowView*>(tt + q_rv);
        const ProdTouch* dtl = reinterpret_cast<const ProdTouch*>(tt + q_tl);
        const ProdPair* dpr = reinterpret_cast<const ProdPair*>(tt + q_pr);
        const int* dsr = reinterpret_cast<const int*>(tt + q_sr);
        RtJob* djob = reinterpret_cast<RtJob*>(tt + q_job);
        const size_t ra = ((size_t)max_rows + 18 + 63) & ~(size_t)63;
        const size_t pa = ((size_t)max_pairs + 2 + 63) & ~(size_t)63;
        const double t_res1 = now_s();
        HIPCHK(c, P.keys2.reserve(((use_early ? 0 : (size_t)max_rec) + (size_t)max_early) * 4 + 256));
        HIPCHK(c, P.flag.reserve((5 * ra + 2 * pa + (size_t)max_boff) * 4 + 256));
        if (rebuild) { HIPCHK(c, P.keys.reserve((size_t)max_rec * 4 + 256)); HIPCHK(c, P.pos.reserve((size_t)max_rt * 4 + 256)); HIPCHK(c, P.tstage.reserve((size_t)max_rec * 4 + 256)); }
        size_t tbs = 0;
        HIPCHK(c, exclusive_sum_int(nullptr, tbs, nullptr, nullptr, std::max(max_rows, max_pairs) + 1, st));
        HIPCHK(c, P.tmp.reserve(tbs + 256));
        if (tblocks.size() > 1) HIPCHK(c, P.pot_tgt.reserve(((size_t)slots_all + 2) * 4));
        if (c->opt.timing) fprintf(stderr, "[l3d products] transposed (%s side arrays): %zu block(s), <= %lld records, %d pairs, %d rows, a row touches <= %d views: tables in %.2f ms, buffers in %.2f ms\n",
                                   rebuild ? "rebuilt" : "the chain's", tblocks.size(), max_rec, max_pairs, max_rows, max_touch, (t_res1 - t_t0) * 1e3, (now_s() - t_res1) * 1e3);
        unsigned* E = use_early ? const_cast<unsigned*>(early->E) : P.keys2.as<unsigned>();
        int* cnt = P.flag.as<int>();
        int *bstart = cnt + ra, *ucnt = cnt + 2 * ra, *ustart = cnt + 3 * ra, *spare = cnt + 4 * ra, *pcnt = cnt + 5 * ra, *poff = pcnt + pa, *boff = use_early ? const_cast<int*>(early->boff) : poff + pa;
        const unsigned* poff_kq = use_early ? early->poff_kq : nullptr;
        const int e_maxN = use_early ? early->maxN : 0;
        int* err = spare + ra - 8;
        HIPCHK(c, hipMemsetAsync(err, 0, 4, st));
        long long base = 0;
        std::vector<RtJob> jobs;
        for (const TBlock& B : tblocks) {
            const int d0 = P.seg_base[(size_t)B.x0], d1 = P.seg_base[(size_t)B.x1], rows = d1 - d0, n_pairs = B.pair1 - B.pair0;
            int scal[2] = { 0, 0 };
            rep.block_cap.push_back(-1); rep.block_staged.push_back(0); rep.block_g.push_back(-1);
            if (rows > 0) {
                unsigned* ent = use_early ? P.keys2.as<unsigned>() : E + B.rec_n;
                {
                    ProfScope p(c, "prod_keys", st);
                    if (rebuild) {
                        jobs.clear();
                        long long qo = 0, ro = 0;
                        int max_n = 0, max_cells = 0;
                        for (size_t i = 0; i < B.n_items; ++i) {
                            const int k = items[B.item0 + i];
                            RtJob j;
                            j.recs = arena + hres[k].kept_base; j.qt = P.keys.as<unsigned>() + qo; j.rt = P.pos.as<int>() + ro;
                            j.ids = dids + nb_off[(size_t)k]; j.qs = dqs + nb_off[(size_t)k]; j.n = hres[k].n_kept; j.S = views[k].S_src; j.N = views[k].N; j.pad = 0;
                            j.skey = P.tstage.as<unsigned>() + qo;
                            vqh[(size_t)k].qt = j.qt; vqh[(size_t)k].rt = j.rt;
                            qo += j.n; ro += ((long long)j.N + 1) * j.S;
                            max_n = std::max(max_n, j.n); max_cells = std::max(max_cells, (j.N + 1) * j.S);
                            jobs.push_back(j);
                        }
                        HIPCHK(c, hipMemcpyAsync(djob, jobs.data(), jobs.size() * sizeof(RtJob), hipMemcpyHostToDevice, st));
                        HIPCHK(c, hipMemcpyAsync(tt + q_vq, vqh.data(), vqh.size() * sizeof(ProdViewQ), hipMemcpyHostToDevice, st));
                        launch_qt_from_records(djob, (int)jobs.size(), max_n, err, st);
                        launch_rt_from_qt(djob, (int)jobs.size(), max_cells, st);
                        HIPCHK(c, hipMemcpyAsync(&scal[1], err, 4, hipMemcpyDeviceToHost, st));
                        HIPCHK(c, hipStreamSynchronize(st));
                        if (scal[1]) { rep.refused = 2; return kSortInstead; }
                    }
                    if (n_pairs > 0 && !use_early) {
                        hipLaunchKernelGGL(k_prodv_pair_counts, dim3((unsigned)n_pairs), dim3(256), 0, st, dpr + B.pair0, dvq, dpv, pcnt);
                        HIPCHK(c, hipMemsetAsync(pcnt + n_pairs, 0, 4, st));
                        size_t t1 = tbs;
                        HIPCHK(c, exclusive_sum_int(P.tmp.p, t1, pcnt, poff, n_pairs + 1, st));
                        double recs = 0, cells = 0;
                        for (size_t i = 0; i < B.n_items; ++i) { const int k = items[B.item0 + i]; recs += hres[k].n_kept; cells += (double)views[k].N * views[k].S_src; }
                        int g = 1;
                        while (g < 64 && g < recs / std::max(1.0, cells) / 4.0) g <<= 1;
                        if (c->opt.prod_pair_g >= 0) g = c->opt.prod_pair_g;
                        int cap = 12288;
                        unsigned* T = nullptr;
                        while (cap > 1024 && ((size_t)B.maxS + 2 + 2 * (size_t)cap) * 4 > 64 * 1024) cap -= 1024;
                        if (((size_t)B.maxS + 2 + 2 * (size_t)cap) * 4 <= 64 * 1024) { HIPCHK(c, P.tstage.reserve((size_t)max_rec * 4 + 256)); T = P.tstage.as<unsigned>(); } else cap = 0;
                        hipLaunchKernelGGL(k_prodv_pair_transpose, dim3((unsigned)n_pairs), dim3(kPairThreads), ((size_t)B.maxS + 2 + 2 * (size_t)cap) * 4, st, dpr + B.pair0, dvq, dpv, dnb,
                                           (const int*)poff, g, boff, E, T, cap);
                        rep.block_cap.back() = cap; rep.block_g.back() = g;
                    }
                    if (B.n_srcs) {
                        HIPCHK(c, hipMemsetAsync(cnt, 0, ((size_t)rows + 1) * 4, st));
                        const dim3 eg((unsigned)std::max(1, std::min(256, (maxS + 15) / 16)), (unsigned)B.n_srcs);
                        if (!rebuild) hipLaunchKernelGGL(HIP_KERNEL_NAME(k_prod_early_rt<1>), eg, dim3(256), 0, st, dpv, dvq, dps, dslot, dsr + B.src0, d0, d1, cnt, (const int*)bstart, ent,
                                                         (unsigned long long*)nullptr, (int*)nullptr);
                        else hipLaunchKernelGGL(HIP_KERNEL_NAME(k_prodt_early<false>), dim3(gx, (unsigned)B.n_srcs), dim3(256), 0, st, arena, dpv, dps, dsr + B.src0, dcv, d0, d1, cnt, (const int*)bstart, ent);
                        size_t t1 = tbs;
                        HIPCHK(c, exclusive_sum_int(P.tmp.p, t1, cnt, bstart, rows + 1, st));
                        if (!rebuild) hipLaunchKernelGGL(HIP_KERNEL_NAME(k_prod_early_rt<2>), eg, dim3(256), 0, st, dpv, dvq, dps, dslot, dsr + B.src0, d0, d1, cnt, (const int*)bstart, ent,
                                                         (unsigned long long*)nullptr, (int*)nullptr);
                        else hipLaunchKernelGGL(HIP_KERNEL_NAME(k_prodt_early<true>), dim3(gx, (unsigned)B.n_srcs), dim3(256), 0, st, arena, dpv, dps, dsr + B.src0, dcv, d0, d1, cnt, (const int*)bstart, ent);
                    }
                }
                const dim3 rg((unsigned)((B.maxS + 3) / 4), (unsigned)(B.x1 - B.x0));
                const int* bs = B.n_srcs ? bstart : nullptr;
                int* stage = nullptr;
                if (2.0 * (double)B.rec_n <= 48.0 * rows && (size_t)rows * 256 <= ((size_t)1 << 30)) { HIPCHK(c, P.rowstage.reserve((size_t)rows * 256 + 256)); stage = P.rowstage.as<int>(); }
                rep.block_staged.back() = stage ? 1 : 0;
                {
                    ProfScope p(c, "prod_rows", st);
                    HIPCHK(c, hipMemsetAsync(ucnt + rows, 0, 4, st));
                    hipLaunchKernelGGL(HIP_KERNEL_NAME(k_prodv_rows<false>), rg, dim3(256), 0, st, drv, B.x0, d0, dvq, dtl, dpr, (const int*)poff - B.pair0, (const int*)boff,
                                       (const unsigned*)E, bs, (const unsigned*)ent, ucnt, (const int*)ustart, base, (int*)nullptr, stage, poff_kq, e_maxN);
                    size_t t1 = tbs;
                    HIPCHK(c, exclusive_sum_int(P.tmp.p, t1, ucnt, ustart, rows + 1, st));
                }
                HIPCHK(c, hipMemcpyAsync(&scal[0], ustart + rows, 4, hipMemcpyDeviceToHost, st));
                HIPCHK(c, hipMemcpyAsync(&scal[1], err, 4, hipMemcpyDeviceToHost, st));
                HIPCHK(c, hipStreamSynchronize(st));
                if (scal[1]) { rep.refused = 2; return kSortInstead; }
                if (tblocks.size() == 1) HIPCHK(c, P.pot_tgt.reserve(((size_t)scal[0] + 2) * 4));
                {
                    ProfScope p(c, "prod_rows", st);
                    hipLaunchKernelGGL(HIP_KERNEL_NAME(k_prodv_rows<true>), rg, dim3(256), 0, st, drv, B.x0, d0, dvq, dtl, dpr, (const int*)poff - B.pair0, (const int*)boff,
                                       (const unsigned*)E, bs, (const unsigned*)ent, ucnt, (const int*)ustart, base, P.pot_tgt.as<int>(), stage, poff_kq, e_maxN);
                    hipLaunchKernelGGL(k_prodt_row_starts, dim3((unsigned)((rows + 256) / 256)), dim3(256), 0, st, (const int*)ustart, rows, base, P.pot_start.as<long long>() + d0);
                }
            } else {
                hipLaunchKernelGGL(k_prod_fill_rows, dim3(1), dim3(256), 0, st, P.pot_start.as<long long>(), (long long)d0, (long long)d0 + 1, base);
            }
            base += scal[0];
        }
        if (tblocks.empty()) HIPCHK(c, P.pot_tgt.reserve(64));
        rep.build = 1; rep.n_blocks = (int)tblocks.size();
        n_pot_out = base;
        return L3D_OK;
    };
    long long n_pot = 0;
    bool rows_built = false;
    if (c->opt.prod_transpose != 0) {
        const int rc = transposed(n_pot);
        if (rc == L3D_OK) rows_built = true;
        else if (rc != kSortInstead) return rc;
        else if (c->opt.timing) fprintf(stderr, "[l3d products] transposed build refused (a slice is not ordered by segment, or a target outside the bit space): sorting instead\n");
    }
    if (!rows_built) {
        if (blocks.size() > 1 && max_kept > 0) {
            HIPCHK(c, P.flag.reserve((size_t)n_views * nv + 256));
            HIPCHK(c, hipMemsetAsync(P.flag.p, 0, (size_t)n_views * nv, st));
            hipLaunchKernelGGL(k_prod_names, dim3(gx, n_views), dim3(256), 0, st, arena, dpv, dids, nv, P.flag.as<unsigned char>());
            std::vector<unsigned char> names((size_t)n_views * nv);
            HIPCHK(c, hipMemcpyAsync(names.data(), P.flag.p, names.size(), hipMemcpyDeviceToHost, st));
            HIPCHK(c, hipStreamSynchronize(st));
            bool added = false;
            for (int k = 0; k < n_views; ++k) for (int t = 0; t < nv; ++t) {
                std::vector<int>& tv = touch_view[(size_t)t];
                if (names[(size_t)k * nv + t] && std::find(tv.begin(), tv.end(), k) == tv.end()) { tv.push_back(k); added = true; }
            }
            if (added) {
                if (int rc = plan_blocks()) return rc;
                max_slots = 0;
                for (const ProdBlock& B : blocks) max_slots = std::max(max_slots, B.slots);
                n_keys_max = max_slots + 1;
                HIPCHK(c, P.ttab.reserve(off_tab.size() * 8 + 256));
                HIPCHK(c, hipMemcpyAsync(P.ttab.p, off_tab.data(), off_tab.size() * 8, hipMemcpyHostToDevice, st));
                HIPCHK(c, hipStreamSynchronize(st));
                doff = P.ttab.as<long long>();
            }
        }
        rep.build = 2; rep.n_blocks = (int)blocks.size();
        rep.block_cap.clear(); rep.block_staged.clear(); rep.block_g.clear();
        HIPCHK(c, P.keys.reserve((size_t)n_keys_max * 8 + 64));
        HIPCHK(c, P.keys2.reserve((size_t)n_keys_max * 8 + 64));
        HIPCHK(c, P.flag.reserve(((size_t)n_keys_max + 2) * 4));
        HIPCHK(c, P.pos.reserve(((size_t)n_keys_max + 2) * 4));
        HIPCHK(c, P.pot_tgt.reserve(((size_t)slots_all + 2) * 4));
        unsigned long long* keys = P.keys.as<unsigned long long>();
        unsigned long long* keys2 = P.keys2.as<unsigned long long>();
        size_t tb1 = 0, tb2 = 0;
        HIPCHK(c, sort_keys_u64(nullptr, tb1, keys, keys2, (int)n_keys_max, 0, std::min(64, 2 * nb), st));
        HIPCHK(c, exclusive_sum_int(nullptr, tb2, P.flag.as<int>(), P.pos.as<int>(), (int)n_keys_max + 1, st));
        HIPCHK(c, P.tmp.reserve(std::max(tb1, tb2) + 256));
        long long base = 0;
        for (size_t bi = 0; bi < blocks.size(); ++bi) {
            const ProdBlock& B = blocks[bi];
            const long long n_keys = B.slots + 1;
            {
                ProfScope p(c, "prod_keys", st);
                HIPCHK(c, hipMemsetAsync(keys + B.slots, 0xff, 8, st));
                if (max_kept > 0) hipLaunchKernelGGL(k_prod_keys, dim3(gx, n_views), dim3(256), 0, st, arena, dpv, doff + B.off_view, dids, dsb, nv, nb, B.d0, B.d1, keys);
                if (!ps.empty()) hipLaunchKernelGGL(k_prod_keys_early, dim3(gx, (unsigned)ps.size()), dim3(256), 0, st, arena, dpv, dps, doff + B.off_src, dcv, nb, B.d0, B.d1,
                                                    keys, P.best_ref.as<unsigned long long>(), d_list_len);
            }
            {
                ProfScope p(c, "prod_sort", st);
                size_t t1 = tb1, t2 = tb2;
                HIPCHK(c, sort_keys_u64(P.tmp.p, t1, keys, keys2, (int)n_keys, 0, std::min(64, 2 * nb), st));
                const unsigned nblk = (unsigned)((n_keys + 255) / 256);
                HIPCHK(c, hipMemsetAsync(P.flag.as<int>() + n_keys, 0, 4, st));
                hipLaunchKernelGGL(k_prod_flags, dim3(nblk), dim3(256), 0, st, keys2, n_keys, P.flag.as<int>());
                HIPCHK(c, exclusive_sum_int(P.tmp.p, t2, P.flag.as<int>(), P.pos.as<int>(), (int)n_keys + 1, st));
                hipLaunchKernelGGL(k_prod_csr, dim3(nblk), dim3(256), 0, st, keys2, P.flag.as<int>(), P.pos.as<int>(), n_keys, nb, B.d0, B.d1, base, P.pot_start.as<long long>(), P.pot_tgt.as<int>());
            }
            if (bi + 1 < blocks.size()) {
                int n_unique = 0;
                HIPCHK(c, hipMemcpyAsync(&n_unique, P.pos.as<int>() + n_keys, 4, hipMemcpyDeviceToHost, st));
                HIPCHK(c, hipStreamSynchronize(st));
                base += n_unique;
            }
        }
        const long long last_keys = blocks.empty() ? 0 : blocks.back().slots + 1;
        int n_last = 0;
        if (!blocks.empty()) HIPCHK(c, hipMemcpyAsync(&n_last, P.pos.as<int>() + last_keys, 4, hipMemcpyDeviceToHost, st));
        HIPCHK(c, hipStreamSynchronize(st));
        n_pot = base + n_last;
    }
    std::vector<float> med((size_t)2 * n_views, 1.0f);
    HIPCHK(c, hipMemcpyAsync(med.data(), P.median.p, (size_t)n_views * 8, hipMemcpyDeviceToHost, st));
    HIPCHK(c, hipStreamSynchronize(st));
    { hipError_t e_ = hipGetLastError(); if (e_ != hipSuccess) return fail(c, L3D_ERR_HIP, std::string("products: ") + hipGetErrorString(e_)); }
    P.n_pot = n_pot;
    if (held) {
        const long long r0 = dv0 >= dv1 ? (long long)nd + 1 : (long long)P.seg_base[(size_t)dv0], r1 = dv0 >= dv1 ? (long long)nd + 1 : (long long)P.seg_base[(size_t)dv1] + 1;
        if (r0 > 0) hipLaunchKernelGGL(k_prod_fill_rows, dim3((unsigned)((std::min<long long>(r0, nd + 1) + 255) / 256)), dim3(256), 0, st, P.pot_start.as<long long>(), 0ll, std::min<long long>(r0, nd + 1), 0ll);
        if (r1 <= nd) hipLaunchKernelGGL(k_prod_fill_rows, dim3((unsigned)(((long long)nd + 1 - r1 + 255) / 256)), dim3(256), 0, st, P.pot_start.as<long long>(), r1, (long long)nd + 1, n_pot);
        HIPCHK(c, hipStreamSynchronize(st));
        if (c->opt.part_release != 0) { P.keys.release(); P.keys2.release(); P.flag.release(); P.pos.release(); P.tmp.release(); }
    }
    for (int k = 0; k < n_views; ++k) {
        l3d_chain_summary& s = summary[k];
        s.verified = pvh[k].verified; s.n_kept = pvh[k].verified ? hres[k].n_kept : reinterpret_cast<const int*>(med.data() + n_views)[k];
        s.n_candidates = pvh[k].verified ? hres[k].R : 0;
        s.median_depth = med[(size_t)k]; s.pad = 0;
    }
    if (n_pot_out) *n_pot_out = n_pot;
    P.valid = !partial;
    return L3D_OK;
}

namespace l3d {

struct ViewGeo {
    double RtKinv[9], C[3];
    float k_lower, k_upper, median_depth;
    int pad;
    const float4* segs;
};

__global__ __launch_bounds__(256) void k_hyp_flag(const long long* __restrict__ best_ref, int nd, int* __restrict__ flag)
{
    const int d = blockIdx.x * 256 + threadIdx.x;
    if (d < nd) flag[d] = best_ref[d] >= 0 ? 1 : 0;
}

__global__ __launch_bounds__(256) void k_hyp_build(const Match* __restrict__ arena, const long long* __restrict__ best_ref, const int* __restrict__ hyp_of,
                                                   const int* __restrict__ seg_base, int nv, const ViewGeo* __restrict__ geo, int nd,
                                                   Hypothesis* __restrict__ hyp, float* __restrict__ score, int* __restrict__ hyp_dense, int* __restrict__ best_hyp,
                                                   int* __restrict__ view_hyp_begin)
{
    const int d = blockIdx.x * 256 + threadIdx.x;
    if (d <= nv) view_hyp_begin[d] = hyp_of[seg_base[d]];
    if (d >= nd) return;
    const long long ref = best_ref[d];
    if (ref < 0) { best_hyp[d] = -1; return; }
    int lo = 0, hi = nv;
    while (hi - lo > 1) { const int mid = (lo + hi) >> 1; if (seg_base[mid] <= d) lo = mid; else hi = mid; }
    const ViewGeo g = geo[lo];
    const Match r = arena[ref & kBestIndexMask];
    const bool rev = (ref & kBestReversed) != 0;
    const float d1 = rev ? r.depths[2] : r.depths[0], d2 = rev ? r.depths[3] : r.depths[1];
    const float conf = rev ? 0.0f : r.confidence;
    const float4 sg = g.segs[d - seg_base[lo]];
    la::M3 M;
    for (int i = 0; i < 9; ++i) M.m[i] = g.RtKinv[i];
    la::V3 P1, P2, dir;
    unproject_segment_f64(M, la::V3{ g.C[0], g.C[1], g.C[2] }, sg.x, sg.y, sg.z, sg.w, d1, d2, P1, P2, dir);
    const int h = hyp_of[d];
    Hypothesis o;
    o.P1[0] = P1.x; o.P1[1] = P1.y; o.P1[2] = P1.z; o.P2[0] = P2.x; o.P2[1] = P2.y; o.P2[2] = P2.z; o.dir[0] = dir.x; o.dir[1] = dir.y; o.dir[2] = dir.z;
    o.depth_p1 = d1; o.depth_p2 = d2; o.k_lower = g.k_lower; o.k_upper = g.k_upper; o.median_depth = g.median_depth; o.pad = 0;
    hyp[h] = o;
    score[h] = fminf(conf, 1.0f);
    hyp_dense[h] = d;
    best_hyp[d] = h;
}

__global__ __launch_bounds__(256) void k_prod_best_records(const Match* __restrict__ arena, const long long* __restrict__ best_ref, const int* __restrict__ seg_base, int nv,
                                                           const unsigned* __restrict__ early_cam, int nd, Match* __restrict__ out)
{
    const int d = blockIdx.x * 256 + threadIdx.x;
    if (d >= nd) return;
    const long long ref = best_ref[d];
    Match o;
    o.segID1 = 0xffffffffu; o.camID2 = 0; o.segID2 = 0; o.depths[0] = o.depths[1] = o.depths[2] = o.depths[3] = 0.0f; o.confidence = 0.0f;
    if (ref >= 0) {
        int lo = 0, hi = nv;
        while (hi - lo > 1) { const int mid = (lo + hi) >> 1; if (seg_base[mid] <= d) lo = mid; else hi = mid; }
        const Match r = arena[ref & kBestIndexMask];
        if (ref & kBestReversed) {
            o.segID1 = r.segID2; o.segID2 = r.segID1; o.camID2 = early_cam ? early_cam[d] : 0;
            o.depths[0] = r.depths[2]; o.depths[1] = r.depths[3]; o.depths[2] = r.depths[0]; o.depths[3] = r.depths[1];
        } else o = r;
    }
    out[d] = o;
}

}

extern "C" {

int l3d_products_hypotheses(l3d_ctx* c, const l3d_view_geometry* geometry, int n_views, int32_t* view_hyp_begin, int32_t** hyp_dense_out, int* n_hyp_out)
{
    if (!c) return L3D_ERR_INVALID;
    Products& P = c->products;
// ... 28 lines not shown
    HIPCHK(c, hipMemsetAsync(flag + nd, 0, 4, st));
    ProfScope p(c, "hypotheses", st);
    hipLaunchKernelGGL(k_hyp_flag, dim3((nd + 255) / 256), dim3(256), 0, st, P.best_ref.as<long long>(), nd, flag);
    size_t tb = 0;
    HIPCHK(c, exclusive_sum_int(nullptr, tb, flag, hyp_of, nd + 1, st));
    HIPCHK(c, P.tmp.reserve(tb + 256));
    HIPCHK(c, exclusive_sum_int(P.tmp.p, tb, flag, hyp_of, nd + 1, st));
    HIPCHK(c, c->aff_hyp.reserve((size_t)nd * sizeof(Hypothesis) + 64));
    HIPCHK(c, P.score.reserve((size_t)nd * 4 + 64));
    HIPCHK(c, P.hyp_dense.reserve((size_t)nd * 4 + 64));
    HIPCHK(c, P.best_hyp.reserve((size_t)nd * 4 + 64));
    hipLaunchKernelGGL(k_hyp_build, dim3((std::max(nd, nv + 1) + 255) / 256), dim3(256), 0, st, c->ch_kept.as<Match>(), P.best_ref.as<long long>(), hyp_of,
                       reinterpret_cast<const int*>(gb + o_sb), nv, reinterpret_cast<const ViewGeo*>(gb + o_geo), nd, c->aff_hyp.as<Hypothesis>(), P.score.as<float>(),
                       P.hyp_dense.as<int>(), P.best_hyp.as<int>(), reinterpret_cast<int*>(gb + o_vhb));
    HIPCHK(c, hipMemcpyAsync(view_hyp_begin, gb + o_vhb, (size_t)(nv + 1) * 4, hipMemcpyDeviceToHost, st));
    HIPCHK(c, hipStreamSynchronize(st));
    const int nh = view_hyp_begin[nv];
    int32_t* hd = static_cast<int32_t*>(malloc((size_t)nh * 4 + 4));
    if (!hd) return fail(c, L3D_ERR_NOMEM, "malloc");
    if (nh > 0) {
        hipError_t e = hipMemcpyAsync(hd, P.hyp_dense.p, (size_t)nh * 4, hipMemcpyDeviceToHost, st);
        if (e == hipSuccess) e = hipStreamSynchronize(st);
        if (e != hipSuccess) { free(hd); return fail(c, L3D_ERR_HIP, std::string("l3d_products_hypotheses: ") + hipGetErrorString(e)); }
    }
    { hipError_t e_ = hipGetLastError(); if (e_ != hipSuccess) { free(hd); return fail(c, L3D_ERR_HIP, std::string("l3d_products_hypotheses: ") + hipGetErrorString(e_)); } }
    P.view_hyp_begin.assign(view_hyp_begin, view_hyp_begin + nv + 1);
    P.n_hyp = nh; P.hyp_valid = true;
    c->resident_hyp = nh;
    *hyp_dense_out = hd; *n_hyp_out = nh;
    return L3D_OK;
}

int l3d_products_hypotheses_get(l3d_ctx* c, l3d_hypothesis* hyp, float* score)
{
    if (!c) return L3D_ERR_INVALID;
    Products& P = c->products;
    if (!P.valid || !P.hyp_valid) return fail(c, L3D_ERR_INVALID, "no resident hypotheses");
    HIPCHK(c, hipSetDevice(c->device));
    if (hyp && P.n_hyp) HIPCHK(c, hipMemcpyAsync(hyp, c->aff_hyp.p, (size_t)P.n_hyp * sizeof(Hypothesis), hipMemcpyDeviceToHost, c->stream));
    if (score && P.n_hyp) HIPCHK(c, hipMemcpyAsync(score, P.score.p, (size_t)P.n_hyp * 4, hipMemcpyDeviceToHost, c->stream));
    HIPCHK(c, hipStreamSynchronize(c->stream));
    return L3D_OK;
}

int l3d_chain_kept_list(l3d_ctx* c, int index, l3d_match** out, int* n)
{
    if (!c) return L3D_ERR_INVALID;
    Products& P = c->products;
    if (!out || !n) return fail(c, L3D_ERR_INVALID, "bad argument");
    *out = nullptr; *n = 0;
    if (!P.valid || index < 0 || index >= P.n_chain) return fail(c, L3D_ERR_INVALID, "l3d_chain_kept_list: no such view in the resident products");
    if (c->records_released) return fail(c, L3D_ERR_INVALID, "l3d_chain_kept_list: the kept records of this chain were released (l3d_chain_release_records)");
    HIPCHK(c, hipSetDevice(c->device));
    auto fetch = [&](int k, std::vector<l3d_match>& v) -> int {
        const ChainResult& r = P.res[(size_t)k];
        v.resize((size_t)r.n_kept);
        if (r.n_kept) HIPCHK(c, hipMemcpy(v.data(), c->ch_kept.as<Match>() + r.kept_base, (size_t)r.n_kept * sizeof(Match), hipMemcpyDeviceToHost));
        return L3D_OK;
    };
    std::vector<l3d_match> lst;
    if (P.chain_verified[(size_t)index]) { if (int rc = fetch(index, lst)) return rc; }
    if (!P.chain_verified[(size_t)index]) {
        lst.clear();
        std::vector<l3d_match> src;
        const unsigned vid = P.chain_view_id[(size_t)index];
        for (size_t q = 0; q < P.early_src_index[(size_t)index].size(); ++q) {
            if (int rc = fetch(P.early_src_index[(size_t)index][q], src)) return rc;
            for (const l3d_match& mp : src) {
                if (mp.camID2 != vid) continue;
                l3d_match r;
                r.segID1 = mp.segID2; r.segID2 = mp.segID1; r.confidence = 0.0f; r.camID2 = (uint32_t)P.early_src_cam[(size_t)index][q];
                r.depths[0] = mp.depths[2]; r.depths[1] = mp.depths[3]; r.depths[2] = mp.depths[0]; r.depths[3] = mp.depths[1];
                lst.push_back(r);
            }
        }
    }
    l3d_match* o = static_cast<l3d_match*>(malloc(lst.size() * sizeof(l3d_match) + 32));
    if (!o) return fail(c, L3D_ERR_NOMEM, "malloc");
    if (!lst.empty()) memcpy(o, lst.data(), lst.size() * sizeof(l3d_match));
    *out = o; *n = (int)lst.size();
    return L3D_OK;
}

int l3d_chain_products_get(l3d_ctx* c, int64_t* pot_start, int32_t* pot_tgt, l3d_match* best_match)
{
    if (!c) return L3D_ERR_INVALID;
    Products& P = c->products;
    if (!P.valid) return fail(c, L3D_ERR_INVALID, "no resident products");
    if (best_match && c->records_released) return fail(c, L3D_ERR_INVALID, "l3d_chain_products_get: the kept records of this chain were released (l3d_chain_release_records)");
    HIPCHK(c, hipSetDevice(c->device));
    hipStream_t st = c->stream;
    if (pot_start) HIPCHK(c, hipMemcpyAsync(pot_start, P.pot_start.p, ((size_t)P.n_dense + 1) * 8, hipMemcpyDeviceToHost, st));
    if (pot_tgt && P.n_pot) HIPCHK(c, hipMemcpyAsync(pot_tgt, P.pot_tgt.p, (size_t)P.n_pot * 4, hipMemcpyDeviceToHost, st));
    if (best_match) {
        std::vector<unsigned> cam((size_t)P.n_dense, 0u);
        bool any_early = false;
        std::vector<long long> ref((size_t)P.n_dense);
        HIPCHK(c, hipMemcpyAsync(ref.data(), P.best_ref.p, (size_t)P.n_dense * 8, hipMemcpyDeviceToHost, st));
        HIPCHK(c, hipStreamSynchronize(st));
        for (int k = 0; k < P.n_chain; ++k) {
            if (P.chain_verified[(size_t)k]) continue;
            any_early = true;
            const int vi = P.chain_view[(size_t)k];
            for (int d = P.seg_base[(size_t)vi]; d < P.seg_base[(size_t)vi + 1]; ++d) {
                if (ref[(size_t)d] < 0) continue;
                const long long idx = ref[(size_t)d] & kBestIndexMask;
                for (size_t q = 0; q < P.early_src_index[(size_t)k].size(); ++q) {
                    const ChainResult& r = P.res[(size_t)P.early_src_index[(size_t)k][q]];
                    if (idx >= r.kept_base && idx < (long long)r.kept_base + r.n_kept) { cam[(size_t)d] = (unsigned)P.early_src_cam[(size_t)k][q]; break; }
                }
            }
        }
        HIPCHK(c, P.keys.reserve((size_t)P.n_dense * (sizeof(Match) + 4) + 256));
        Match* dout = P.keys.as<Match>();
        unsigned* dcam = reinterpret_cast<unsigned*>(P.keys.as<char>() + (((size_t)P.n_dense * sizeof(Match) + 255) & ~(size_t)255));
        if (any_early) HIPCHK(c, hipMemcpyAsync(dcam, cam.data(), (size_t)P.n_dense * 4, hipMemcpyHostToDevice, st));
        HIPCHK(c, P.flag.reserve(((size_t)P.n_views_all + 2) * 4 + 256));
        int* dsb = P.flag.as<int>();
        HIPCHK(c, hipMemcpyAsync(dsb, P.seg_base.data(), ((size_t)P.n_views_all + 1) * 4, hipMemcpyHostToDevice, st));
        hipLaunchKernelGGL(k_prod_best_records, dim3((P.n_dense + 255) / 256), dim3(256), 0, st, c->ch_kept.as<Match>(), P.best_ref.as<long long>(), dsb, P.n_views_all,
                           any_early ? dcam : nullptr, P.n_dense, dout);
        HIPCHK(c, hipMemcpyAsync(best_match, dout, (size_t)P.n_dense * sizeof(Match), hipMemcpyDeviceToHost, st));
    }
    HIPCHK(c, hipStreamSynchronize(st));
    return L3D_OK;
}

int l3d_test_products(l3d_ctx* c, const l3d_chain_view* views, int n_views, const l3d_dense_map* map, const l3d_match* kept, const int32_t* n_kept,
                      const int64_t* n_candidates, const float* best, const int32_t* bestpos, l3d_test_products_path* sel,
                      l3d_chain_summary* summary, int64_t* n_pot)
{
    if (!c) return L3D_ERR_INVALID;
    if (!views || n_views <= 0 || !map || !map->view_ids || !map->seg_base || !n_kept || !n_candidates || !best || !bestpos || !sel || !summary)
        return fail(c, L3D_ERR_INVALID, "l3d_test_products: bad argument");
    if ((sel->side_arrays | 1) != 1 || (sel->early_pairs | 1) != 1 || (sel->early_pairs && !sel->side_arrays))
        return fail(c, L3D_ERR_INVALID, "l3d_test_products: side_arrays and early_pairs are 0 or 1, early_pairs needs side_arrays");
    if (n_pot) *n_pot = 0;
    sel->side_arrays_used = 0; sel->build = 0; sel->refused = 0; sel->n_blocks = 0; sel->max_touch = 0; sel->early_cap = -1; sel->early_g = -1;
    const size_t nvs = (size_t)n_views;
    std::vector<ChainResult> hres(nvs);
    std::vector<ProdChainView> pvh(nvs);
    std::vector<size_t> seg_off(nvs + 1, 0), rt_off(nvs + 1, 0);
    long long total = 0;
    int maxN = 0, maxS = 1;
    for (int k = 0; k < n_views; ++k) {
        const l3d_chain_view& v = views[k];
        const std::string w = "l3d_test_products: view " + std::to_string(k);
        if (v.S_src < 0 || v.S_src > 16384 || v.N < 0 || v.N > 255 || (v.N > 0 && !v.local2global)) return fail(c, L3D_ERR_INVALID, w + ": segments or neighbours out of range");
        if (v.n_sources < 0 || (v.n_sources > 0 && (!v.source_cam || !v.source_index))) return fail(c, L3D_ERR_INVALID, w + ": bad source list");
        if (n_kept[k] < 0 || (n_kept[k] > 0 && (!kept || v.n_tbm <= 0))) return fail(c, L3D_ERR_INVALID, w + ": records without a list to hold them");
        if (n_candidates[k] < 0 || n_candidates[k] > 0x7fffffffll) return fail(c, L3D_ERR_INVALID, w + ": candidate count out of range");
        const bool verified = v.n_tbm > 0;
        if (verified) for (int s = 0; s < v.S_src; ++s) {
            const int p = bestpos[seg_off[(size_t)k] + (size_t)s];
            if (p < -1 || p >= n_kept[k]) return fail(c, L3D_ERR_INVALID, w + ": a best position outside the list");
        }
        ChainResult& r = hres[(size_t)k];
        r.kept_base = (uint64_t)total; r.n_kept = verified ? n_kept[k] : 0; r.R = verified ? (int)n_candidates[k] : 0; r.overflow = 0; r.n_want = 0;
        total += r.n_kept;
        seg_off[(size_t)k + 1] = seg_off[(size_t)k] + (size_t)v.S_src;
        rt_off[(size_t)k + 1] = rt_off[(size_t)k] + (verified ? ((size_t)v.N + 1) * (size_t)v.S_src : 0);
        maxN = std::max(maxN, v.N); maxS = std::max(maxS, v.S_src);
    }
    if (total > 0x7ffffff0ll) return fail(c, L3D_ERR_INVALID, "l3d_test_products: too many records");
    HIPCHK(c, hipSetDevice(c->device));
    hipStream_t st = c->stream;
// ... 137 lines not shown
```

### line3d_amd/csrc/l3d_products.hpp

```cpp
#pragma once

#include "l3d_ctx.hpp"

namespace l3d {

struct ProdChainView {
    const float2* best;
    const int* bestpos;
    int verified;
    const int* rt;
};

struct ProdEarly {
    const int* pcnt_kq = nullptr;
    const unsigned* poff_kq = nullptr;
    const int* boff = nullptr;
    const unsigned* E = nullptr;
    const int* boff_off_host = nullptr;
    int maxN = 0;
};
int build_products(l3d_ctx* c, const l3d_chain_view* views, int n_views, const ProdChainView* pv, const ChainResult* hres,
                   const l3d_dense_map* map, l3d_chain_summary* summary, int64_t* n_pot, int dv0 = 0, int dv1 = -1, const char* held = nullptr,
                   const unsigned* qt_arena = nullptr, const ProdEarly* early = nullptr);

struct EarlyView { const int* rt; const int* St; const int* boff_off; int k, S, N, pad; };
void launch_early_transposes(l3d_ctx* c, const EarlyView* views_dev, int k0, int nb, int maxN, int maxSt, const ChainResult* res,
                             const unsigned* qt_arena, int* pcnt_kq, unsigned* poff_kq, int* boff, unsigned* E, unsigned* T, double avg_run, hipStream_t st);

void launch_prod_shift_rows(const long long* piece, long long n_rows, long long base, long long* pot_start_at, hipStream_t st);

constexpr long long kBestReversed = 1ll << 62;
constexpr long long kBestIndexMask = (1ll << 40) - 1;

}
```

### line3d_amd/csrc/l3d_sort.hip

```cpp
#include "l3d_rocprim_arch.gen.hpp"
#include <hipcub/hipcub.hpp>

#include "l3d_sort.hpp"
#include "l3d_kernels.hpp"

namespace l3d {

namespace {

inline size_t al256(size_t b) { return (b + 255) & ~(size_t)255; }

__global__ __launch_bounds__(256) void k_widen_keys(const unsigned* __restrict__ in, unsigned long long* __restrict__ out, int n)
{
    const int i = blockIdx.x * 256 + threadIdx.x;
    if (i < n) out[i] = in[i];
}
__global__ __launch_bounds__(256) void k_narrow_keys(const unsigned long long* __restrict__ in, unsigned* __restrict__ out, int n)
{
    const int i = blockIdx.x * 256 + threadIdx.x;
    if (i < n) out[i] = (unsigned)in[i];
}

constexpr int kScanTile = 2048;
__global__ __launch_bounds__(256) void k_scan_tile_sums(const int* __restrict__ in, int n, int* __restrict__ sums)
{
    __shared__ int s_w[4];
    const int base = blockIdx.x * kScanTile + threadIdx.x * 8;
    int t = 0;
#pragma unroll
    for (int k = 0; k < 8; ++k) if (base + k < n) t += in[base + k];
    for (int o = 32; o > 0; o >>= 1) t += __shfl_down(t, o);
    if ((threadIdx.x & 63) == 0) s_w[threadIdx.x >> 6] = t;
    __syncthreads();
    if (threadIdx.x == 0) sums[blockIdx.x] = s_w[0] + s_w[1] + s_w[2] + s_w[3];
}
__global__ __launch_bounds__(256) void k_scan_tile(const int* __restrict__ in, int n, const int* __restrict__ offsets, int* __restrict__ out)
{
    __shared__ int s_w[4];
    const int lane = threadIdx.x & 63, wave = threadIdx.x >> 6;
    const int base = blockIdx.x * kScanTile + threadIdx.x * 8;
    int v[8], t = 0;
#pragma unroll
    for (int k = 0; k < 8; ++k) { v[k] = base + k < n ? in[base + k] : 0; t += v[k]; }
    int incl = t;
    for (int o = 1; o < 64; o <<= 1) { const int u = __shfl_up(incl, o); if (lane >= o) incl += u; }
    if (lane == 63) s_w[wave] = incl;
    __syncthreads();
    int run = incl - t + (offsets ? offsets[blockIdx.x] : 0);
    for (int w = 0; w < wave; ++w) run += s_w[w];
#pragma unroll
    for (int k = 0; k < 8; ++k) { if (base + k < n) out[base + k] = run; run += v[k]; }
}

}

hipError_t sort_pairs_u64_u32(void* tmp, size_t& bytes, const unsigned long long* keys_in, unsigned long long* keys_out, const unsigned* vals_in, unsigned* vals_out,
                              int n, int begin_bit, int end_bit, hipStream_t st)
{
    return hipcub::DeviceRadixSort::SortPairs(tmp, bytes, keys_in, keys_out, vals_in, vals_out, n, begin_bit, end_bit, st);
}

hipError_t sort_pairs_u32_u32(void* tmp, size_t& bytes, const unsigned* keys_in, unsigned* keys_out, const unsigned* vals_in, unsigned* vals_out,
                              int n, int begin_bit, int end_bit, hipStream_t st)
{
    size_t inner = 0;
    hipError_t e = sort_pairs_u64_u32(nullptr, inner, nullptr, nullptr, nullptr, nullptr, n, begin_bit, end_bit, st);
    if (e != hipSuccess) return e;
    const size_t kb = al256((size_t)(n > 0 ? n : 1) * 8), need = al256(inner) + 2 * kb + 256;
    if (!tmp) { bytes = need; return hipSuccess; }
    if (bytes < need) return hipErrorInvalidValue;
    if (n <= 0) return hipSuccess;
    unsigned char* p = static_cast<unsigned char*>(tmp);
    unsigned long long* a = reinterpret_cast<unsigned long long*>(p + al256(inner));
    unsigned long long* b = reinterpret_cast<unsigned long long*>(p + al256(inner) + kb);
    const unsigned grid = (unsigned)((n + 255) / 256);
    hipLaunchKernelGGL(k_widen_keys, dim3(grid), dim3(256), 0, st, keys_in, a, n);
    e = sort_pairs_u64_u32(p, inner, a, b, vals_in, vals_out, n, begin_bit, end_bit, st);
    if (e != hipSuccess) return e;
    hipLaunchKernelGGL(k_narrow_keys, dim3(grid), dim3(256), 0, st, b, keys_out, n);
    return hipGetLastError();
}

hipError_t sort_keys_u64(void* tmp, size_t& bytes, const unsigned long long* keys_in, unsigned long long* keys_out, int n, int begin_bit, int end_bit, hipStream_t st)
{
    return hipcub::DeviceRadixSort::SortKeys(tmp, bytes, keys_in, keys_out, n, begin_bit, end_bit, st);
}

hipError_t exclusive_sum_int(void* tmp, size_t& bytes, const int* in, int* out, int n, hipStream_t st)
{
    size_t need = 256;
    for (long long m = n; m > kScanTile;) { m = (m + kScanTile - 1) / kScanTile; need += 2 * al256((size_t)m * 4); }
    if (!tmp) { bytes = need; return hipSuccess; }
    if (bytes < need) return hipErrorInvalidValue;
    if (n <= 0) return hipSuccess;
    if (n <= kScanTile) { hipLaunchKernelGGL(k_scan_tile, dim3(1), dim3(256), 0, st, in, n, (const int*)nullptr, out); return hipGetLastError(); }
    const int tiles = (n + kScanTile - 1) / kScanTile;
    unsigned char* p = static_cast<unsigned char*>(tmp);
    int* sums = reinterpret_cast<int*>(p);
    int* offs = reinterpret_cast<int*>(p + al256((size_t)tiles * 4));
    unsigned char* rest = p + 2 * al256((size_t)tiles * 4);
    size_t rest_bytes = bytes - 2 * al256((size_t)tiles * 4);
    hipLaunchKernelGGL(k_scan_tile_sums, dim3(tiles), dim3(256), 0, st, in, n, sums);
    const hipError_t e = exclusive_sum_int(rest, rest_bytes, sums, offs, tiles, st);
    if (e != hipSuccess) return e;
    hipLaunchKernelGGL(k_scan_tile, dim3(tiles), dim3(256), 0, st, in, n, (const int*)offs, out);
    return hipGetLastError();
}

__global__ void k_sort_touch() {}
void warm_sort() { touch_kernel(reinterpret_cast<const void*>(&k_sort_touch)); }

}
```

### line3d_amd/csrc/l3d_sort.hpp

```cpp
#pragma once

#include <hip/hip_runtime.h>

#include <cstddef>

namespace l3d {

hipError_t sort_pairs_u64_u32(void* tmp, size_t& bytes, const unsigned long long* keys_in, unsigned long long* keys_out, const unsigned* vals_in, unsigned* vals_out,
                              int n, int begin_bit, int end_bit, hipStream_t st);
hipError_t sort_pairs_u32_u32(void* tmp, size_t& bytes, const unsigned* keys_in, unsigned* keys_out, const unsigned* vals_in, unsigned* vals_out,
                              int n, int begin_bit, int end_bit, hipStream_t st);
hipError_t sort_keys_u64(void* tmp, size_t& bytes, const unsigned long long* keys_in, unsigned long long* keys_out, int n, int begin_bit, int end_bit, hipStream_t st);
hipError_t exclusive_sum_int(void* tmp, size_t& bytes, const int* in, int* out, int n, hipStream_t st);

}
```

Baseline: 116.9 billion.

## Plan product schedule ahead on host and drop the count round trip

Builds the host-side products schedule (view maps, touch lists, pairs) once all views are enqueued, overlapping it with GPU chain work instead of doing it after. The transposed build now writes row totals to device memory and reads the entry count back with the median copy through pinned memory, against a host-computed bound with write guards, which removes a synchronizing device-to-host read. It also adds a single-pass front-sum scan kernel, side work on a separate stream joined by an event, and a report API. The trade-offs are more state and cache-validity checks, plus possible wasted overallocation when the bound is loose.

```diff
diff --git a/include/line3d_amd.h b/include/line3d_amd.h
--- a/include/line3d_amd.h
+++ b/include/line3d_amd.h
@@ -144,6 +144,7 @@
 int l3d_chain_release_records(l3d_ctx* ctx);
 int l3d_chain_records_digest(l3d_ctx* ctx, uint64_t* hash, int32_t* n_kept, int n);
 int l3d_chain_products_get(l3d_ctx* ctx, int64_t* pot_start, int32_t* pot_tgt, l3d_match* best_match);
+int l3d_products_report(l3d_ctx* ctx, int32_t out[6]);
 
 typedef struct l3d_view_geometry {
     double RtKinv[9];
diff --git a/line3d_amd/capi.py b/line3d_amd/capi.py
--- a/line3d_amd/capi.py
+++ b/line3d_amd/capi.py
@@ -917,6 +917,11 @@
         out.update(total=int(sel.total), largest=int(sel.largest), spb_used=int(sel.spb_used), overflow=int(sel.overflow), needed=int(sel.needed))
         return out
 
+    def products_report(self):
+        out = np.zeros(6, np.int32)
+        self._chk(self.lib.l3d_products_report(self.h, _p(out)))
+        return dict(zip(("build", "refused", "n_blocks", "max_touch", "planned_ahead", "no_round_trip"), (int(x) for x in out)))
+
     def chain_products_get(self, n_dense: int, n_pot: int, slack: int = 0):
         pot_start = np.zeros(n_dense + 1, np.int64)
         pot_tgt = np.full(n_pot + slack, -1, np.int32)
diff --git a/line3d_amd/csrc/l3d_chain.hip b/line3d_amd/csrc/l3d_chain.hip
--- a/line3d_amd/csrc/l3d_chain.hip
+++ b/line3d_amd/csrc/l3d_chain.hip
@@ -600,9 +600,14 @@
         rc_final = fail(c, L3D_ERR_HIP, std::string(what) + ": " + hipGetErrorString(e));
         return false;
     };
+    std::vector<ProdChainView> pv((size_t)(map ? n_views : 0));
+    if (map) for (int k = 0; k < n_views; ++k) pv[(size_t)k] = ProdChainView{ vd[(size_t)k].verified ? vd[(size_t)k].best : nullptr, vd[(size_t)k].verified ? vd[(size_t)k].bestpos : nullptr, vd[(size_t)k].verified ? 1 : 0,
+                                                                                      vd[(size_t)k].verified ? vd[(size_t)k].rt : nullptr };
+    bool planned = false;
     for (int k = 0; k < n_views && rc_final == L3D_OK; ++k) {
         while (k_enq < n_views && k_enq <= k + kAhead) { int rc = enqueue_view(k_enq); if (rc) { rc_final = rc; break; } ++k_enq; }
         if (rc_final) break;
+        if (map && !planned && k_enq == n_views) { plan_products(c, views, n_views, pv.data(), map); planned = true; }
         { std::lock_guard<std::mutex> lk(mu); if (deliver_rc) break; }
         const ViewDev& d = vd[(size_t)k];
         if (!d.verified) { hand_over(k, 0, ChainResult()); continue; }
@@ -707,10 +712,8 @@
     deliverer.join();
     if (rc_final == L3D_OK && deliver_rc) rc_final = fail(c, deliver_rc, deliver_err);
     const double t_prod0 = now_s();
+    if (rc_final != L3D_OK && map) plan_products(c, nullptr, 0, nullptr, nullptr);
     if (rc_final == L3D_OK && map) {
-        std::vector<ProdChainView> pv((size_t)n_views);
-        for (int k = 0; k < n_views; ++k) pv[(size_t)k] = ProdChainView{ vd[(size_t)k].verified ? vd[(size_t)k].best : nullptr, vd[(size_t)k].verified ? vd[(size_t)k].bestpos : nullptr, vd[(size_t)k].verified ? 1 : 0,
-                                                                         vd[(size_t)k].verified ? vd[(size_t)k].rt : nullptr };
         ProdEarly pe;
         const bool early_done = early && arena_cap < 0x7ffffff0ull;
         if (early_done) {
diff --git a/line3d_amd/csrc/l3d_ctx.hpp b/line3d_amd/csrc/l3d_ctx.hpp
--- a/line3d_amd/csrc/l3d_ctx.hpp
+++ b/line3d_amd/csrc/l3d_ctx.hpp
@@ -6,6 +6,7 @@
 #include <cstdlib>
 #include <cstring>
 #include <map>
+#include <memory>
 #include <mutex>
 #include <string>
 #include <unordered_map>
@@ -96,9 +97,13 @@
     int build = 0;
     int refused = 0;
     int n_blocks = 0, max_touch = 0;
+    int planned_ahead = 0;
+    int no_round_trip = 0;
     int early_cap = -1, early_g = -1;
     std::vector<int> block_cap, block_staged, block_g;
 };
+
+struct ProdSchedule;
 
 struct Products {
     bool valid = false, hyp_valid = false;
@@ -107,6 +112,8 @@
     int n_dense = 0, n_views_all = 0, n_chain = 0, n_hyp = 0;
     long long n_pot = 0, total_kept = 0;
     DevBuf keys, keys2, flag, pos, tmp, pot_start, pot_tgt, best_ref, median, tables, ttab, rowstage, tstage;
+    PinBuf pin_tables, pin_ttab, pin_out;
+    std::shared_ptr<ProdSchedule> sched;
     DevBuf e_cnt, e_poff, e_boff, e_E, e_T, e_tab;
     std::vector<int> e_boff_off;
     DevBuf geo, hyp_of, score, hyp_dense, best_hyp, coll, aux;
@@ -124,6 +131,7 @@
     {
         DevBuf* b[] = { &keys, &keys2, &flag, &pos, &tmp, &pot_start, &pot_tgt, &best_ref, &median, &tables, &ttab, &rowstage, &tstage, &e_cnt, &e_poff, &e_boff, &e_E, &e_T, &e_tab, &geo, &hyp_of, &score, &hyp_dense, &best_hyp, &coll, &aux };
         for (DevBuf* x : b) x->release();
+        pin_tables.release(); pin_ttab.release(); pin_out.release();
         valid = hyp_valid = false; coll_n = 0; coll_sig = 0;
     }
 };
diff --git a/line3d_amd/csrc/l3d_products.hip b/line3d_amd/csrc/l3d_products.hip
--- a/line3d_amd/csrc/l3d_products.hip
+++ b/line3d_amd/csrc/l3d_products.hip
@@ -428,7 +428,7 @@
                                                     const ProdPair* __restrict__ pairs, const int* __restrict__ poff, const int* __restrict__ boff, const unsigned* __restrict__ E,
                                                     const int* __restrict__ bstart, const unsigned* __restrict__ ent, int* __restrict__ ucnt, const int* __restrict__ ustart,
                                                     long long base, int* __restrict__ pot_tgt, int* __restrict__ stage,
-                                                    const unsigned* __restrict__ poff_kq, int maxN)
+                                                    const unsigned* __restrict__ poff_kq, int maxN, long long pot_cap)
 {
     constexpr int kWords = 512;
     __shared__ unsigned s_bm[4][kWords];
@@ -444,10 +444,11 @@
     const int e0 = bstart ? bstart[row] : 0, ne = bstart ? bstart[row + 1] - e0 : 0;
     int total = 0;
     long long o = WRITE ? base + ustart[row] : 0;
+    const bool fits = !WRITE || base + ustart[row + 1] <= pot_cap;
     if (!WRITE && stage && lane == 63) stage[(size_t)row * 64 + 63] = 0;
     if (WRITE && stage && stage[(size_t)row * 64 + 63] == -2) {
         const int n = ustart[row + 1] - ustart[row];
-        if (lane < n) pot_tgt[o + lane] = stage[(size_t)row * 64 + lane];
+        if (lane < n && fits) pot_tgt[o + lane] = stage[(size_t)row * 64 + lane];
         return;
     }
     for (int t0 = v.t0; t0 < v.t1; t0 += 64) {
@@ -495,7 +496,7 @@
                         if (lane == 63) stage[(size_t)row * 64 + 63] = -2;
                     }
                 }
-                else if (keep) pot_tgt[o + __popcll(km & ((1ull << lane) - 1ull))] = sorted;
+                else if (keep && fits) pot_tgt[o + __popcll(km & ((1ull << lane) - 1ull))] = sorted;
                 return;
             }
         }
@@ -523,7 +524,7 @@
                     int incl = pc;
                     for (int d = 1; d < 64; d <<= 1) { const int x = __shfl_up(incl, d); if (lane >= d) incl += x; }
                     long long p = o + (incl - pc);
-                    while (word) { const int bit = __ffs(word) - 1; pot_tgt[p++] = yb + (w << 5) + bit; word &= word - 1u; }
+                    while (word && fits) { const int bit = __ffs(word) - 1; pot_tgt[p++] = yb + (w << 5) + bit; word &= word - 1u; }
                     o += __shfl(incl, 63);
                 }
             }
@@ -537,10 +538,11 @@
     }
 }
 
-__global__ __launch_bounds__(256) void k_prodt_row_starts(const int* __restrict__ ustart, int rows, long long base, long long* __restrict__ pot_start_at)
+__global__ __launch_bounds__(256) void k_prodt_row_starts(const int* __restrict__ ustart, int rows, long long base, long long* __restrict__ pot_start_at, int* __restrict__ n_rows_out)
 {
     const int r = blockIdx.x * 256 + threadIdx.x;
     if (r <= rows) pot_start_at[r] = base + ustart[r];
+    if (r == rows && n_rows_out) *n_rows_out = ustart[r];
 }
 
 }
@@ -549,6 +551,193 @@
 
 int bits_for(int n) { int b = 1; while ((1ll << b) <= (long long)n) ++b; return b; }
 
+}
+
+struct l3d::ProdSchedule {
+    bool valid = false;
+    const l3d_chain_view* views = nullptr;
+    const l3d_dense_map* map = nullptr;
+    int n_views = 0, dv0 = 0, dv1 = 0;
+    bool with_transposed = false;
+    std::vector<char> verified, nz;
+    int nv = 0, nd = 0, maxS = 1;
+    std::vector<int> seg_base, chain_view;
+    std::vector<unsigned> view_ids, chain_view_id;
+    std::vector<std::vector<int>> early_src_index, early_src_cam;
+    std::vector<ProdSrc> ps;
+    std::vector<int> ps_alias_view, ps_slot;
+    std::vector<std::vector<int>> touch_view, touch_src;
+    bool too_wide = false;
+    std::vector<int> nbv_off, nbv, nb_off, qs_sorted, own_k, pair_begin;
+    std::vector<ProdNbQ> nbt;
+    std::vector<unsigned> ids_sorted;
+    std::vector<ProdRowView> rv;
+    std::vector<ProdPair> pairs;
+    std::vector<ProdTouch> tl;
+    int max_touch = 0;
+
+    bool made_from(const l3d_chain_view* v, int n, const l3d_dense_map* m, int a, int b, bool wt, const std::vector<char>& ver, const std::vector<char>& z) const
+    {
+        return valid && views == v && n_views == n && map == m && dv0 == a && dv1 == b && with_transposed == wt && verified == ver && nz == z;
+    }
+};
+
+namespace {
+
+int make_schedule(ProdSchedule& S, const l3d_chain_view* views, int n_views, const l3d_dense_map* map, int dv0, int dv1, bool with_transposed,
+                  const std::vector<char>& verified, const std::vector<char>& nz, std::string& err)
+{
+    S.valid = false;
+    S.views = views; S.map = map; S.n_views = n_views; S.dv0 = dv0; S.dv1 = dv1; S.with_transposed = with_transposed; S.verified = verified; S.nz = nz;
+    const int nv = map->n_views;
+    S.nv = nv;
+    if (nv <= 0) { err = "products: empty dense map"; return L3D_ERR_INVALID; }
+    for (int i = 0; i < nv; ++i) {
+        if (map->seg_base[i + 1] < map->seg_base[i] || (i && map->view_ids[i] <= map->view_ids[i - 1]) || map->seg_base[0] != 0) { err = "products: the dense map must ascend"; return L3D_ERR_INVALID; }
+    }
+    S.nd = map->seg_base[nv];
+    if (S.nd <= 0) { err = "products: no segments"; return L3D_ERR_INVALID; }
+    if (dv0 < 0 || dv1 > nv || dv0 > dv1) { err = "products: bad view range"; return L3D_ERR_INVALID; }
+    S.seg_base.assign(map->seg_base, map->seg_base + nv + 1);
+    S.view_ids.assign(map->view_ids, map->view_ids + nv);
+    S.chain_view.assign((size_t)n_views, -1);
+    S.chain_view_id.resize((size_t)n_views);
+    S.early_src_index.assign((size_t)n_views, {}); S.early_src_cam.assign((size_t)n_views, {});
+    auto view_of = [&](unsigned id) { auto it = std::lower_bound(S.view_ids.begin(), S.view_ids.end(), id); return it != S.view_ids.end() && *it == id ? (int)(it - S.view_ids.begin()) : -1; };
+    auto seg_count = [&](int x) { return S.seg_base[(size_t)x + 1] - S.seg_base[(size_t)x]; };
+    S.ps.clear(); S.ps_alias_view.clear();
+    S.maxS = 1;
+    for (int k = 0; k < n_views; ++k) {
+        const l3d_chain_view& v = views[k];
+        const int vi = view_of(v.view_id);
+        if (vi < 0 || seg_count(vi) != v.S_src) { err = "products: a chain view is missing from the dense map"; return L3D_ERR_INVALID; }
+        S.chain_view[(size_t)k] = vi; S.chain_view_id[(size_t)k] = v.view_id;
+        S.maxS = std::max(S.maxS, v.S_src);
+        if (!verified[(size_t)k]) {
+            S.early_src_index[(size_t)k].assign(v.source_index, v.source_index + v.n_sources);
+            S.early_src_cam[(size_t)k].assign(v.source_cam, v.source_cam + v.n_sources);
+            for (int q = 0; q < v.n_sources; ++q) {
+                const int si = v.source_index[q];
+                if (si < 0 || si >= k || !verified[(size_t)si]) continue;
+                ProdSrc e;
+                e.view = k; e.src = si; e.rank = q; e.pad = 0;
+                const int av = view_of((unsigned)v.source_cam[q]);
+                e.alias_base = av >= 0 ? S.seg_base[(size_t)av] : -1; e.alias_S = av >= 0 ? seg_count(av) : 0;
+                e.out_off = 0;
+                S.ps.push_back(e);
+                S.ps_alias_view.push_back(av);
+            }
+        }
+    }
+    const std::vector<ProdSrc>& ps = S.ps;
+    S.nbv_off.assign((size_t)n_views + 1, 0); S.nbv.clear();
+    for (int k = 0; k < n_views; ++k) {
+        S.nbv_off[(size_t)k] = (int)S.nbv.size();
+        if (verified[(size_t)k]) for (int q = 0; q < views[k].N; ++q) S.nbv.push_back(view_of(views[k].local2global[q]));
+    }
+    S.nbv_off[(size_t)n_views] = (int)S.nbv.size();
+    const std::vector<int>&nbv = S.nbv, &nbv_off = S.nbv_off;
+    S.touch_view.assign((size_t)nv, {}); S.touch_src.assign((size_t)nv, {});
+    for (int k = 0; k < n_views; ++k) {
+        if (!nz[(size_t)k]) continue;
+        S.touch_view[(size_t)S.chain_view[(size_t)k]].push_back(k);
+        for (int q = 0; q < views[k].N; ++q) {
+            const int t = nbv[(size_t)nbv_off[(size_t)k] + q];
+            if (t >= 0 && t != S.chain_view[(size_t)k]) S.touch_view[(size_t)t].push_back(k);
+        }
+    }
+    for (size_t q = 0; q < ps.size(); ++q) {
+        if (!nz[(size_t)ps[q].src]) continue;
+        const int a = S.chain_view[(size_t)ps[q].view], b = S.ps_alias_view[q];
+        S.touch_src[(size_t)a].push_back((int)q);
+        if (b >= 0 && b != a) S.touch_src[(size_t)b].push_back((int)q);
+    }
+    S.ps_slot.assign(ps.size() + 1, -1);
+    for (size_t q = 0; q < ps.size(); ++q) {
+        const l3d_chain_view& sv = views[ps[q].src];
+        for (int j = 0; j < sv.N; ++j) if (sv.local2global[j] == S.chain_view_id[(size_t)ps[q].view]) { S.ps_slot[q] = j; break; }
+    }
+    S.too_wide = false;
+    for (int x = dv0; x < dv1; ++x) if (seg_count(x) > 16000) S.too_wide = true;
+    S.nb_off.clear(); S.nbt.clear(); S.ids_sorted.clear(); S.qs_sorted.clear(); S.own_k.clear(); S.rv.clear(); S.pairs.clear(); S.tl.clear(); S.pair_begin.clear();
+    S.max_touch = 0;
+    if (with_transposed && !S.too_wide) {
+        std::vector<std::vector<int>> T((size_t)nv);
+        for (int x = 0; x < nv; ++x) T[(size_t)x].reserve(32);
+        for (int k = 0; k < n_views; ++k) {
+            if (!verified[(size_t)k]) continue;
+            const int vi = S.chain_view[(size_t)k];
+            for (int q = 0; q < views[k].N; ++q) {
+                const int t = nbv[(size_t)nbv_off[(size_t)k] + q];
+                if (t >= 0) { T[(size_t)vi].push_back(t); T[(size_t)t].push_back(vi); }
+            }
+        }
+        for (size_t q = 0; q < ps.size(); ++q) {
+            const int a = S.chain_view[(size_t)ps[q].view], b = S.ps_alias_view[q];
+            if (b >= 0) { T[(size_t)a].push_back(b); T[(size_t)b].push_back(a); }
+        }
+        for (int x = 0; x < nv; ++x) { std::vector<int>& t = T[(size_t)x]; std::sort(t.begin(), t.end()); t.erase(std::unique(t.begin(), t.end()), t.end()); }
+        S.nb_off.assign((size_t)n_views, 0);
+        std::vector<std::vector<ProdPair>> pairs_of((size_t)nv);
+        S.own_k.assign((size_t)nv, -1);
+        std::vector<std::pair<unsigned, int>> byid;
+        S.nbt.reserve(nbv.size()); S.ids_sorted.reserve(nbv.size()); S.qs_sorted.reserve(nbv.size());
+        for (int k = 0; k < n_views; ++k) {
+            S.nb_off[(size_t)k] = (int)S.nbt.size();
+            if (!verified[(size_t)k]) continue;
+            const int vi = S.chain_view[(size_t)k], N = views[k].N;
+            if (nz[(size_t)k]) S.own_k[(size_t)vi] = k;
+            byid.clear();
+            for (int q = 0; q < N; ++q) {
+                const int t = nbv[(size_t)nbv_off[(size_t)k] + q];
+                S.nbt.push_back(ProdNbQ{ t >= 0 ? S.seg_base[(size_t)t] : -1, t >= 0 ? seg_count(t) : 0 });
+                byid.push_back({ views[k].local2global[q], q });
+                if (t >= 0 && nz[(size_t)k]) pairs_of[(size_t)t].push_back(ProdPair{ k, q, 0, 0 });
+            }
+            std::sort(byid.begin(), byid.end());
+            for (auto& e : byid) { S.ids_sorted.push_back(e.first); S.qs_sorted.push_back(e.second); }
+        }
+        S.rv.resize((size_t)nv);
+        std::vector<ProdPair>& pairs = S.pairs;
+        pairs.reserve(nbv.size()); S.tl.reserve(2 * nbv.size() + 64);
+        for (int x = 0; x < nv; ++x) {
+            ProdRowView& r = S.rv[(size_t)x];
+            r.dense_base = S.seg_base[(size_t)x]; r.S = seg_count(x); r.own_k = S.own_k[(size_t)x]; r.t0 = r.t1 = 0; r.pad = 0;
+            if (x < dv0 || x >= dv1) continue;
+            const int pair0 = (int)pairs.size();
+            for (const ProdPair& pr : pairs_of[(size_t)x]) pairs.push_back(pr);
+            r.t0 = (int)S.tl.size();
+            for (int y : T[(size_t)x]) {
+                ProdTouch e;
+                e.y_base = S.seg_base[(size_t)y]; e.y_S = seg_count(y); e.fq = -1; e.pair = -1;
+                if (r.own_k >= 0) for (int q = 0; q < views[r.own_k].N; ++q) if (nbv[(size_t)nbv_off[(size_t)r.own_k] + q] == y) { e.fq = q; break; }
+                for (int p = pair0; p < (int)pairs.size(); ++p) if (S.chain_view[(size_t)pairs[(size_t)p].k] == y) { e.pair = p; break; }
+                S.tl.push_back(e);
+            }
+            r.t1 = (int)S.tl.size();
+            S.max_touch = std::max(S.max_touch, r.t1 - r.t0);
+        }
+        S.pair_begin.assign((size_t)nv + 1, 0);
+        int p = 0;
+        for (int x = 0; x < nv; ++x) { S.pair_begin[(size_t)x] = p; if (x >= dv0 && x < dv1) p += (int)pairs_of[(size_t)x].size(); }
+        S.pair_begin[(size_t)nv] = p;
+    }
+    S.valid = true;
+    return L3D_OK;
+}
+
+}
+
+void l3d::plan_products(l3d_ctx* c, const l3d_chain_view* views, int n_views, const ProdChainView* pvh, const l3d_dense_map* map)
+{
+    Products& P = c->products;
+    if (!P.sched) P.sched = std::make_shared<ProdSchedule>();
+    P.sched->valid = false;
+    if (!map || !map->view_ids || !map->seg_base || n_views <= 0) return;
+    std::vector<char> verified((size_t)n_views);
+    for (int k = 0; k < n_views; ++k) verified[(size_t)k] = pvh[k].verified ? 1 : 0;
+    std::string err;
+    (void)make_schedule(*P.sched, views, n_views, map, 0, map->n_views, c->opt.prod_transpose != 0, verified, verified, err);
 }
 
 void l3d::launch_prod_shift_rows(const long long* piece, long long n_rows, long long base, long long* pot_start_at, hipStream_t st)
@@ -583,84 +772,54 @@
     P.valid = false; P.hyp_valid = false;
     c->records_released = false;
     ProductsReport& rep = P.report;
-    rep.build = 0; rep.refused = 0; rep.n_blocks = 0; rep.max_touch = 0;
+    rep.build = 0; rep.refused = 0; rep.n_blocks = 0; rep.max_touch = 0; rep.planned_ahead = 0; rep.no_round_trip = 0;
     rep.block_cap.clear(); rep.block_staged.clear(); rep.block_g.clear();
     hipStream_t st = c->stream;
     const int nv = map->n_views;
-    if (nv <= 0) return fail(c, L3D_ERR_INVALID, "products: empty dense map");
-    for (int i = 0; i < nv; ++i) {
-        if (map->seg_base[i + 1] < map->seg_base[i] || (i && map->view_ids[i] <= map->view_ids[i - 1]) || map->seg_base[0] != 0)
-            return fail(c, L3D_ERR_INVALID, "products: the dense map must ascend");
-    }
-    const int nd = map->seg_base[nv];
-    if (nd <= 0) return fail(c, L3D_ERR_INVALID, "products: no segments");
     const bool partial = dv1 >= 0;
     if (!partial) { dv0 = 0; dv1 = nv; }
-    if (dv0 < 0 || dv1 > nv || dv0 > dv1) return fail(c, L3D_ERR_INVALID, "products: bad view range");
-    P.seg_base.assign(map->seg_base, map->seg_base + nv + 1);
-    P.view_ids.assign(map->view_ids, map->view_ids + nv);
+    if (!P.sched) P.sched = std::make_shared<ProdSchedule>();
+    ProdSchedule& S = *P.sched;
+    {
+        std::vector<char> verified((size_t)n_views), nz((size_t)n_views);
+        for (int k = 0; k < n_views; ++k) { verified[(size_t)k] = pvh[k].verified ? 1 : 0; nz[(size_t)k] = pvh[k].verified && hres[k].n_kept > 0 ? 1 : 0; }
+        const bool ahead = S.made_from(views, n_views, map, dv0, dv1, c->opt.prod_transpose != 0, verified, nz);
+        if (!ahead) {
+            std::string err;
+            if (int rc = make_schedule(S, views, n_views, map, dv0, dv1, c->opt.prod_transpose != 0, verified, nz, err)) return fail(c, rc, err);
+        }
+        S.valid = false;
+        rep.planned_ahead = ahead ? 1 : 0;
+        if (c->opt.timing) fprintf(stderr, "[l3d products] schedule tables %s\n", ahead ? "made ahead, while the chain ran" : "made now");
+    }
+    const int nd = S.nd;
+    P.seg_base = S.seg_base; P.view_ids = S.view_ids; P.chain_view = S.chain_view; P.chain_view_id = S.chain_view_id;
+    P.early_src_index = S.early_src_index; P.early_src_cam = S.early_src_cam;
     P.res.assign(hres, hres + n_views);
     P.n_dense = nd; P.n_views_all = nv; P.n_chain = n_views;
-    P.chain_view.assign((size_t)n_views, -1);
     P.chain_verified.assign((size_t)n_views, 0);
     for (int k = 0; k < n_views; ++k) P.chain_verified[(size_t)k] = pvh[k].verified ? 1 : 0;
-    P.chain_view_id.resize((size_t)n_views);
-    P.early_src_index.assign((size_t)n_views, {}); P.early_src_cam.assign((size_t)n_views, {});
-    auto view_of = [&](unsigned id) { auto it = std::lower_bound(P.view_ids.begin(), P.view_ids.end(), id); return it != P.view_ids.end() && *it == id ? (int)(it - P.view_ids.begin()) : -1; };
 
     std::vector<ProdView> pv((size_t)n_views);
-    std::vector<ProdSrc> ps;
-    std::vector<int> ps_alias_view;
+    const std::vector<ProdSrc>& ps = S.ps;
     long long total_kept = 0, early_slots = 0;
     for (int k = 0; k < n_views; ++k) if (pvh[k].verified) total_kept = std::max(total_kept, (long long)hres[k].kept_base + hres[k].n_kept);
     if (total_kept > kBestIndexMask) return fail(c, L3D_ERR_UNSUPPORTED, "products: " + std::to_string(total_kept) + " kept matches in the arena -- best-match references hold 40-bit positions");
-    int max_kept = 0, maxS = 1;
+    int max_kept = 0;
+    const int maxS = S.maxS;
     for (int k = 0; k < n_views; ++k) {
-        const l3d_chain_view& v = views[k];
-        const int vi = view_of(v.view_id);
-        if (vi < 0 || P.seg_base[(size_t)vi + 1] - P.seg_base[(size_t)vi] != v.S_src) return fail(c, L3D_ERR_INVALID, "products: a chain view is missing from the dense map");
-        P.chain_view[(size_t)k] = vi; P.chain_view_id[(size_t)k] = v.view_id;
         ProdView& o = pv[(size_t)k];
         o.kept_base = pvh[k].verified ? hres[k].kept_base : 0; o.n_kept = pvh[k].verified ? hres[k].n_kept : 0; o.R = pvh[k].verified ? hres[k].R : 0;
-        o.dense_base = P.seg_base[(size_t)vi]; o.S = v.S_src; o.early = pvh[k].verified ? 0 : 1; o.pad = 0;
+        o.dense_base = P.seg_base[(size_t)P.chain_view[(size_t)k]]; o.S = views[k].S_src; o.early = pvh[k].verified ? 0 : 1; o.pad = 0;
         o.bestpos = pvh[k].bestpos; o.best = pvh[k].best;
-        max_kept = std::max(max_kept, o.n_kept); maxS = std::max(maxS, o.S);
-        if (!pvh[k].verified) {
-            P.early_src_index[(size_t)k].assign(v.source_index, v.source_index + v.n_sources);
-            P.early_src_cam[(size_t)k].assign(v.source_cam, v.source_cam + v.n_sources);
-            for (int q = 0; q < v.n_sources; ++q) {
-                const int si = v.source_index[q];
-                if (si < 0 || si >= k || !pvh[si].verified) continue;
-                ProdSrc e;
-                e.view = k; e.src = si; e.rank = q; e.pad = 0;
-                const int av = view_of((unsigned)v.source_cam[q]);
-                e.alias_base = av >= 0 ? P.seg_base[(size_t)av] : -1; e.alias_S = av >= 0 ? P.seg_base[(size_t)av + 1] - P.seg_base[(size_t)av] : 0;
-                e.out_off = 0;
-                early_slots += 2 * (long long)hres[si].n_kept;
-                ps.push_back(e);
-                ps_alias_view.push_back(av);
-            }
-        }
-    }
+        max_kept = std::max(max_kept, o.n_kept);
+    }
+    for (const ProdSrc& e : ps) early_slots += 2 * (long long)hres[e.src].n_kept;
     const long long slots_all = 2 * total_kept + early_slots;
     const int nb = bits_for(nd);
     P.total_kept = total_kept;
 
-    std::vector<std::vector<int>> touch_view((size_t)nv), touch_src((size_t)nv);
-    for (int k = 0; k < n_views; ++k) {
-        if (!pvh[k].verified || hres[k].n_kept == 0) continue;
-        touch_view[(size_t)P.chain_view[(size_t)k]].push_back(k);
-        for (int q = 0; q < views[k].N; ++q) {
-            const int t = view_of(views[k].local2global[q]);
-            if (t >= 0 && t != P.chain_view[(size_t)k]) touch_view[(size_t)t].push_back(k);
-        }
-    }
-    for (size_t q = 0; q < ps.size(); ++q) {
-        if (hres[ps[q].src].n_kept == 0) continue;
-        const int a = P.chain_view[(size_t)ps[q].view], b = ps_alias_view[q];
-        touch_src[(size_t)a].push_back((int)q);
-        if (b >= 0 && b != a) touch_src[(size_t)b].push_back((int)q);
-    }
+    std::vector<std::vector<int>>&touch_view = S.touch_view, &touch_src = S.touch_src;
     long long budget = 1ll << 28;
     if (c->opt.prod_block_keys > 0) budget = c->opt.prod_block_keys;
     else if (slots_all > budget) {
@@ -713,20 +872,18 @@
         const bool has = native_rt && pvh[k].verified && hres[k].n_kept > 0;
         evq[(size_t)k] = ProdViewQ{ has ? qt_arena + hres[k].kept_base : nullptr, has ? pvh[k].rt : nullptr, 0, views[k].N };
     }
-    std::vector<int> ps_slot(ps.size() + 1, -1);
-    for (size_t q = 0; q < ps.size(); ++q) {
-        const l3d_chain_view& sv = views[ps[q].src];
-        for (int j = 0; j < sv.N; ++j) if (sv.local2global[j] == P.chain_view_id[(size_t)ps[q].view]) { ps_slot[q] = j; break; }
-    }
+    const std::vector<int>& ps_slot = S.ps_slot;
     char* tb = P.tables.as<char>();
-    std::vector<char> tblob(tab_total);
+    HIPCHK(c, P.pin_tables.reserve(tab_total));
     {
-        auto put = [&](size_t off, const void* src, size_t bytes) { if (bytes) memcpy(tblob.data() + off, src, bytes); };
+        char* tblob = P.pin_tables.as<char>();
+        memset(tblob, 0, tab_total);
+        auto put = [&](size_t off, const void* src, size_t bytes) { if (bytes) memcpy(tblob + off, src, bytes); };
         put(o_pv, pv.data(), pv.size() * sizeof(ProdView)); put(o_ps, ps.data(), ps.size() * sizeof(ProdSrc)); put(o_ids, P.view_ids.data(), (size_t)nv * 4);
         put(o_sb, P.seg_base.data(), (size_t)(nv + 1) * 4); put(o_cv, P.chain_view_id.data(), (size_t)n_views * 4); put(o_off, off_tab.data(), off_tab.size() * 8);
         put(o_evq, evq.data(), evq.size() * sizeof(ProdViewQ)); put(o_slot, ps_slot.data(), ps_slot.size() * 4);
     }
-    HIPCHK(c, hipMemcpyAsync(tb, tblob.data(), tblob.size(), hipMemcpyHostToDevice, st));
+    HIPCHK(c, hipMemcpyAsync(tb, P.pin_tables.p, tab_total, hipMemcpyHostToDevice, st));
     const ProdView* dpv = reinterpret_cast<const ProdView*>(tb + o_pv);
     const ProdSrc* dps = reinterpret_cast<const ProdSrc*>(tb + o_ps);
     const unsigned* dids = reinterpret_cast<const unsigned*>(tb + o_ids);
@@ -742,100 +899,51 @@
     HIPCHK(c, P.median.reserve((size_t)n_views * 8 + 64));
     if (c->opt.timing) fprintf(stderr, "[l3d products] %zu block(s) of up to %lld keys, table of up to %lld entries: buffers reserved in %.2f ms\n", blocks.size(), n_keys_max, slots_all, (now_s() - t_res0) * 1e3);
     int* d_list_len = reinterpret_cast<int*>(P.median.as<float>() + n_views);
-    HIPCHK(c, hipMemsetAsync(d_list_len, 0, (size_t)n_views * 4, st));
+    int* d_n_rows = d_list_len + n_views;
     const Match* arena = c->ch_kept.as<Match>();
-    HIPCHK(c, hipMemsetAsync(P.best_ref.p, 0xff, (size_t)nd * 8, st));
     const unsigned gx = (unsigned)std::max(1, std::min(512, (max_kept + 1023) / 1024));
-    {
-        ProfScope p(c, "prod_keys", st);
-        if (!ps.empty() && native_rt)
-            hipLaunchKernelGGL(HIP_KERNEL_NAME(k_prod_early_rt<0>), dim3((unsigned)std::max(1, std::min(256, (maxS + 15) / 16)), (unsigned)ps.size()), dim3(256), 0, st, dpv, devq, dps, dslot, (const int*)nullptr, 0, 0,
-                               (int*)nullptr, (const int*)nullptr, (unsigned*)nullptr, P.best_ref.as<unsigned long long>(), d_list_len);
-        else if (!ps.empty()) hipLaunchKernelGGL(k_prod_keys_early, dim3(gx, (unsigned)ps.size()), dim3(256), 0, st, arena, dpv, dps, (const long long*)nullptr, dcv, nb, 0, 0,
-                                                 (unsigned long long*)nullptr, P.best_ref.as<unsigned long long>(), d_list_len);
-        hipLaunchKernelGGL(k_prod_best, dim3((maxS + 255) / 256, n_views), dim3(256), 0, st, dpv, P.best_ref.as<long long>());
-        hipLaunchKernelGGL(k_prod_median, dim3(n_views), dim3(256), 0, st, dpv, P.median.as<float>());
-    }
+    struct SideWork {
+        l3d_ctx* c; hipStream_t sb; hipEvent_t up, done; bool launched = false, joined = false;
+        ~SideWork() { if (launched && !joined) (void)hipStreamSynchronize(sb); put_local_event(c, up); put_local_event(c, done); }
+    } side{ c, nullptr, get_local_event(c), get_local_event(c) };
+    (void)hipEventRecord(side.up, st);
+    auto launch_side = [&]() -> int {
+        if (!c->prod_stream) HIPCHK(c, hipStreamCreateWithFlags(&c->prod_stream, hipStreamNonBlocking));
+        hipStream_t sb = side.sb = c->prod_stream;
+        (void)hipStreamWaitEvent(sb, side.up, 0);
+        side.launched = true;
+        HIPCHK(c, hipMemsetAsync(d_list_len, 0, (size_t)n_views * 4, sb));
+        HIPCHK(c, hipMemsetAsync(P.best_ref.p, 0xff, (size_t)nd * 8, sb));
+        {
+            ProfScope p(c, "prod_keys", sb);
+            if (!ps.empty() && native_rt)
+                hipLaunchKernelGGL(HIP_KERNEL_NAME(k_prod_early_rt<0>), dim3((unsigned)std::max(1, std::min(256, (maxS + 15) / 16)), (unsigned)ps.size()), dim3(256), 0, sb, dpv, devq, dps, dslot, (const int*)nullptr, 0, 0,
+                                   (int*)nullptr, (const int*)nullptr, (unsigned*)nullptr, P.best_ref.as<unsigned long long>(), d_list_len);
+            else if (!ps.empty()) hipLaunchKernelGGL(k_prod_keys_early, dim3(gx, (unsigned)ps.size()), dim3(256), 0, sb, arena, dpv, dps, (const long long*)nullptr, dcv, nb, 0, 0,
+                                                     (unsigned long long*)nullptr, P.best_ref.as<unsigned long long>(), d_list_len);
+            hipLaunchKernelGGL(k_prod_best, dim3((maxS + 255) / 256, n_views), dim3(256), 0, sb, dpv, P.best_ref.as<long long>());
+            hipLaunchKernelGGL(k_prod_median, dim3(n_views), dim3(256), 0, sb, dpv, P.median.as<float>());
+        }
+        (void)hipEventRecord(side.done, sb);
+        return L3D_OK;
+    };
     constexpr int kSortInstead = -12345;
+    bool n_pot_pending = false;
+    long long n_pot_bound = 0;
     auto transposed = [&](long long& n_pot_out) -> int {
         const double t_t0 = now_s();
         auto seg_count = [&](int x) { return P.seg_base[(size_t)x + 1] - P.seg_base[(size_t)x]; };
-        for (int x = dv0; x < dv1; ++x) if (seg_count(x) > 16000) { rep.refused = 1; return kSortInstead; }
+        if (S.too_wide) { rep.refused = 1; return kSortInstead; }
         const bool rebuild = !native_rt;
         const bool use_early = early && !rebuild && early->E && early->boff && early->poff_kq;
-        std::vector<int> nbv_off((size_t)n_views + 1, 0), nbv;
-        for (int k = 0; k < n_views; ++k) {
-            nbv_off[(size_t)k] = (int)nbv.size();
-            if (pvh[k].verified) for (int q = 0; q < views[k].N; ++q) nbv.push_back(view_of(views[k].local2global[q]));
-        }
-        nbv_off[(size_t)n_views] = (int)nbv.size();
-        std::vector<std::vector<int>> T((size_t)nv);
-        for (int x = 0; x < nv; ++x) T[(size_t)x].reserve(32);
-        for (int k = 0; k < n_views; ++k) {
-            if (!pvh[k].verified) continue;
-            const int vi = P.chain_view[(size_t)k];
-            for (int q = 0; q < views[k].N; ++q) {
-                const int t = nbv[(size_t)nbv_off[(size_t)k] + q];
-                if (t >= 0) { T[(size_t)vi].push_back(t); T[(size_t)t].push_back(vi); }
-            }
-        }
-        for (size_t q = 0; q < ps.size(); ++q) {
-            const int a = P.chain_view[(size_t)ps[q].view], b = ps_alias_view[q];
-            if (b >= 0) { T[(size_t)a].push_back(b); T[(size_t)b].push_back(a); }
-        }
-        for (int x = 0; x < nv; ++x) { std::vector<int>& t = T[(size_t)x]; std::sort(t.begin(), t.end()); t.erase(std::unique(t.begin(), t.end()), t.end()); }
-        std::vector<int> nb_off((size_t)n_views, 0);
-        std::vector<ProdNbQ> nbt;
-        std::vector<unsigned> ids_sorted;
-        std::vector<int> qs_sorted;
-        std::vector<std::vector<ProdPair>> pairs_of((size_t)nv);
-        std::vector<int> own_k((size_t)nv, -1);
-        std::vector<std::pair<unsigned, int>> byid;
-        nbt.reserve(nbv.size()); ids_sorted.reserve(nbv.size()); qs_sorted.reserve(nbv.size());
-        for (int k = 0; k < n_views; ++k) {
-            nb_off[(size_t)k] = (int)nbt.size();
-            if (!pvh[k].verified) continue;
-            const int vi = P.chain_view[(size_t)k], N = views[k].N;
-            if (hres[k].n_kept > 0) own_k[(size_t)vi] = k;
-            byid.clear();
-            for (int q = 0; q < N; ++q) {
-                const int t = nbv[(size_t)nbv_off[(size_t)k] + q];
-                nbt.push_back(ProdNbQ{ t >= 0 ? P.seg_base[(size_t)t] : -1, t >= 0 ? seg_count(t) : 0 });
-                byid.push_back({ views[k].local2global[q], q });
-                if (t >= 0 && hres[k].n_kept > 0) pairs_of[(size_t)t].push_back(ProdPair{ k, q, 0, 0 });
-            }
-            std::sort(byid.begin(), byid.end());
-            for (auto& e : byid) { ids_sorted.push_back(e.first); qs_sorted.push_back(e.second); }
-        }
-        std::vector<ProdRowView> rv((size_t)nv);
-        std::vector<ProdPair> pairs;
-        std::vector<ProdTouch> tl;
-        pairs.reserve(nbv.size()); tl.reserve(2 * nbv.size() + 64);
-        int max_touch = 0;
-        for (int x = 0; x < nv; ++x) {
-            ProdRowView& r = rv[(size_t)x];
-            r.dense_base = P.seg_base[(size_t)x]; r.S = seg_count(x); r.own_k = own_k[(size_t)x]; r.t0 = r.t1 = 0; r.pad = 0;
-            if (x < dv0 || x >= dv1) continue;
-            const int pair0 = (int)pairs.size();
-            for (const ProdPair& pr : pairs_of[(size_t)x]) pairs.push_back(pr);
-            r.t0 = (int)tl.size();
-            for (int y : T[(size_t)x]) {
-                ProdTouch e;
-                e.y_base = P.seg_base[(size_t)y]; e.y_S = seg_count(y); e.fq = -1; e.pair = -1;
-                if (r.own_k >= 0) for (int q = 0; q < views[r.own_k].N; ++q) if (nbv[(size_t)nbv_off[(size_t)r.own_k] + q] == y) { e.fq = q; break; }
-                for (int p = pair0; p < (int)pairs.size(); ++p) if (P.chain_view[(size_t)pairs[(size_t)p].k] == y) { e.pair = p; break; }
-                tl.push_back(e);
-            }
-            r.t1 = (int)tl.size();
-            max_touch = std::max(max_touch, r.t1 - r.t0);
-        }
+        const std::vector<int>&nb_off = S.nb_off, &qs_sorted = S.qs_sorted, &pair_begin = S.pair_begin;
+        const std::vector<ProdNbQ>& nbt = S.nbt;
+        const std::vector<unsigned>& ids_sorted = S.ids_sorted;
+        const std::vector<ProdRowView>& rv = S.rv;
+        std::vector<ProdPair>& pairs = S.pairs;
+        const std::vector<ProdTouch>& tl = S.tl;
+        const int max_touch = S.max_touch;
         rep.max_touch = max_touch;
-        std::vector<int> pair_begin((size_t)nv + 1, 0);
-        {
-            int p = 0;
-            for (int x = 0; x < nv; ++x) { pair_begin[(size_t)x] = p; if (x >= dv0 && x < dv1) p += (int)pairs_of[(size_t)x].size(); }
-            pair_begin[(size_t)nv] = p;
-        }
         struct TBlock { int x0, x1; size_t item0, n_items, src0, n_srcs; long long rec_n, rt_n, boff_n, early_n; int maxS, pair0, pair1; };
         std::vector<TBlock> tblocks;
         std::vector<int> items;
@@ -889,12 +997,14 @@
                      q_sr = q_pr + al(pairs.size() * sizeof(ProdPair) + 16), q_job = q_sr + al(srcs.size() * 4 + 16), q_total = q_job + al((size_t)n_views * sizeof(RtJob) + 16);
         HIPCHK(c, P.ttab.reserve(q_total));
         char* tt = P.ttab.as<char>();
-        std::vector<char> blob(q_job);
-        auto put = [&](size_t off, const void* src, size_t bytes) { if (bytes) memcpy(blob.data() + off, src, bytes); };
+        HIPCHK(c, P.pin_ttab.reserve(q_job + 16));
+        char* blob = P.pin_ttab.as<char>();
+        memset(blob, 0, q_job);
+        auto put = [&](size_t off, const void* src, size_t bytes) { if (bytes) memcpy(blob + off, src, bytes); };
         put(q_vq, vqh.data(), vqh.size() * sizeof(ProdViewQ)); put(q_nb, nbt.data(), nbt.size() * sizeof(ProdNbQ)); put(q_ids, ids_sorted.data(), ids_sorted.size() * 4);
         put(q_qs, qs_sorted.data(), qs_sorted.size() * 4); put(q_rv, rv.data(), rv.size() * sizeof(ProdRowView)); put(q_tl, tl.data(), tl.size() * sizeof(ProdTouch));
         put(q_pr, pairs.data(), pairs.size() * sizeof(ProdPair)); put(q_sr, srcs.data(), srcs.size() * 4);
-        HIPCHK(c, hipMemcpyAsync(tt, blob.data(), blob.size(), hipMemcpyHostToDevice, st));
+        if (q_job) HIPCHK(c, hipMemcpyAsync(tt, blob, q_job, hipMemcpyHostToDevice, st));
         const ProdViewQ* dvq = reinterpret_cast<const ProdViewQ*>(tt + q_vq);
         const ProdNbQ* dnb = reinterpret_cast<const ProdNbQ*>(tt + q_nb);
         const unsigned* dids = reinterpret_cast<const unsigned*>(tt + q_ids);
@@ -922,7 +1032,18 @@
         const unsigned* poff_kq = use_early ? early->poff_kq : nullptr;
         const int e_maxN = use_early ? early->maxN : 0;
         int* err = spare + ra - 8;
-        HIPCHK(c, hipMemsetAsync(err, 0, 4, st));
+        if (rebuild) HIPCHK(c, hipMemsetAsync(err, 0, 4, st));
+        auto scan_counts = [&](int* in, int* out, int n) -> hipError_t {
+            if (n <= kFrontScanMax) return exclusive_sum_int_front(in, out, n, st);
+            const hipError_t e = hipMemsetAsync(in + n, 0, 4, st);
+            if (e != hipSuccess) return e;
+            size_t t1 = tbs;
+            return exclusive_sum_int(P.tmp.p, t1, in, out, n + 1, st);
+        };
+        constexpr long long kPotBound = 1ll << 26;
+        const long long pot_bound = tblocks.size() == 1 ? 2 * tblocks[0].rec_n + tblocks[0].early_n : 0;
+        const bool deferred = tblocks.size() == 1 && pot_bound <= kPotBound && P.seg_base[(size_t)tblocks[0].x1] > P.seg_base[(size_t)tblocks[0].x0];
+        if (deferred) HIPCHK(c, P.pot_tgt.reserve(((size_t)pot_bound + 2) * 4));
         long long base = 0;
         std::vector<RtJob> jobs;
         for (const TBlock& B : tblocks) {
@@ -958,9 +1079,7 @@
                     }
                     if (n_pairs > 0 && !use_early) {
                         hipLaunchKernelGGL(k_prodv_pair_counts, dim3((unsigned)n_pairs), dim3(256), 0, st, dpr + B.pair0, dvq, dpv, pcnt);
-                        HIPCHK(c, hipMemsetAsync(pcnt + n_pairs, 0, 4, st));
-                        size_t t1 = tbs;
-                        HIPCHK(c, exclusive_sum_int(P.tmp.p, t1, pcnt, poff, n_pairs + 1, st));
+                        HIPCHK(c, scan_counts(pcnt, poff, n_pairs));
                         double recs = 0, cells = 0;
                         for (size_t i = 0; i < B.n_items; ++i) { const int k = items[B.item0 + i]; recs += hres[k].n_kept; cells += (double)views[k].N * views[k].S_src; }
                         int g = 1;
@@ -980,8 +1099,7 @@
                         if (!rebuild) hipLaunchKernelGGL(HIP_KERNEL_NAME(k_prod_early_rt<1>), eg, dim3(256), 0, st, dpv, dvq, dps, dslot, dsr + B.src0, d0, d1, cnt, (const int*)bstart, ent,
                                                          (unsigned long long*)nullptr, (int*)nullptr);
                         else hipLaunchKernelGGL(HIP_KERNEL_NAME(k_prodt_early<false>), dim3(gx, (unsigned)B.n_srcs), dim3(256), 0, st, arena, dpv, dps, dsr + B.src0, dcv, d0, d1, cnt, (const int*)bstart, ent);
-                        size_t t1 = tbs;
-                        HIPCHK(c, exclusive_sum_int(P.tmp.p, t1, cnt, bstart, rows + 1, st));
+                        HIPCHK(c, scan_counts(cnt, bstart, rows));
                         if (!rebuild) hipLaunchKernelGGL(HIP_KERNEL_NAME(k_prod_early_rt<2>), eg, dim3(256), 0, st, dpv, dvq, dps, dslot, dsr + B.src0, d0, d1, cnt, (const int*)bstart, ent,
                                                          (unsigned long long*)nullptr, (int*)nullptr);
                         else hipLaunchKernelGGL(HIP_KERNEL_NAME(k_prodt_early<true>), dim3(gx, (unsigned)B.n_srcs), dim3(256), 0, st, arena, dpv, dps, dsr + B.src0, dcv, d0, d1, cnt, (const int*)bstart, ent);
@@ -994,22 +1112,25 @@
                 rep.block_staged.back() = stage ? 1 : 0;
                 {
                     ProfScope p(c, "prod_rows", st);
-                    HIPCHK(c, hipMemsetAsync(ucnt + rows, 0, 4, st));
                     hipLaunchKernelGGL(HIP_KERNEL_NAME(k_prodv_rows<false>), rg, dim3(256), 0, st, drv, B.x0, d0, dvq, dtl, dpr, (const int*)poff - B.pair0, (const int*)boff,
-                                       (const unsigned*)E, bs, (const unsigned*)ent, ucnt, (const int*)ustart, base, (int*)nullptr, stage, poff_kq, e_maxN);
-                    size_t t1 = tbs;
-                    HIPCHK(c, exclusive_sum_int(P.tmp.p, t1, ucnt, ustart, rows + 1, st));
+                                       (const unsigned*)E, bs, (const unsigned*)ent, ucnt, (const int*)ustart, base, (int*)nullptr, stage, poff_kq, e_maxN, 0ll);
+                    HIPCHK(c, scan_counts(ucnt, ustart, rows));
                 }
-                HIPCHK(c, hipMemcpyAsync(&scal[0], ustart + rows, 4, hipMemcpyDeviceToHost, st));
-                HIPCHK(c, hipMemcpyAsync(&scal[1], err, 4, hipMemcpyDeviceToHost, st));
-                HIPCHK(c, hipStreamSynchronize(st));
-                if (scal[1]) { rep.refused = 2; return kSortInstead; }
-                if (tblocks.size() == 1) HIPCHK(c, P.pot_tgt.reserve(((size_t)scal[0] + 2) * 4));
+                long long pot_cap = pot_bound;
+                if (!deferred) {
+                    HIPCHK(c, hipMemcpyAsync(&scal[0], ustart + rows, 4, hipMemcpyDeviceToHost, st));
+                    if (rebuild) HIPCHK(c, hipMemcpyAsync(&scal[1], err, 4, hipMemcpyDeviceToHost, st));
+                    HIPCHK(c, hipStreamSynchronize(st));
+                    if (scal[1]) { rep.refused = 2; return kSortInstead; }
+                    if (tblocks.size() == 1) HIPCHK(c, P.pot_tgt.reserve(((size_t)scal[0] + 2) * 4));
+                    pot_cap = base + scal[0];
+                }
                 {
                     ProfScope p(c, "prod_rows", st);
                     hipLaunchKernelGGL(HIP_KERNEL_NAME(k_prodv_rows<true>), rg, dim3(256), 0, st, drv, B.x0, d0, dvq, dtl, dpr, (const int*)poff - B.pair0, (const int*)boff,
-                                       (const unsigned*)E, bs, (const unsigned*)ent, ucnt, (const int*)ustart, base, P.pot_tgt.as<int>(), stage, poff_kq, e_maxN);
-                    hipLaunchKernelGGL(k_prodt_row_starts, dim3((unsigned)((rows + 256) / 256)), dim3(256), 0, st, (const int*)ustart, rows, base, P.pot_start.as<long long>() + d0);
+                                       (const unsigned*)E, bs, (const unsigned*)ent, ucnt, (const int*)ustart, base, P.pot_tgt.as<int>(), stage, poff_kq, e_maxN, pot_cap);
+                    hipLaunchKernelGGL(k_prodt_row_starts, dim3((unsigned)((rows + 256) / 256)), dim3(256), 0, st, (const int*)ustart, rows, base, P.pot_start.as<long long>() + d0,
+                                       deferred ? d_n_rows : (int*)nullptr);
                 }
             } else {
                 hipLaunchKernelGGL(k_prod_fill_rows, dim3(1), dim3(256), 0, st, P.pot_start.as<long long>(), (long long)d0, (long long)d0 + 1, base);
@@ -1019,6 +1140,9 @@
         if (tblocks.empty()) HIPCHK(c, P.pot_tgt.reserve(64));
         rep.build = 1; rep.n_blocks = (int)tblocks.size();
         n_pot_out = base;
+        n_pot_pending = deferred;
+        rep.no_round_trip = deferred ? 1 : 0;
+        n_pot_bound = pot_bound;
         return L3D_OK;
     };
     long long n_pot = 0;
@@ -1030,6 +1154,7 @@
         else if (c->opt.timing) fprintf(stderr, "[l3d products] transposed build refused (a slice is not ordered by segment, or a target outside the bit space): sorting instead\n");
     }
     if (!rows_built) {
+        if (int rc = launch_side()) return rc;
         if (blocks.size() > 1 && max_kept > 0) {
             HIPCHK(c, P.flag.reserve((size_t)n_views * nv + 256));
             HIPCHK(c, hipMemsetAsync(P.flag.p, 0, (size_t)n_views * nv, st));
@@ -1100,10 +1225,18 @@
         HIPCHK(c, hipStreamSynchronize(st));
         n_pot = base + n_last;
     }
-    std::vector<float> med((size_t)2 * n_views, 1.0f);
-    HIPCHK(c, hipMemcpyAsync(med.data(), P.median.p, (size_t)n_views * 8, hipMemcpyDeviceToHost, st));
+    if (!side.launched) { if (int rc = launch_side()) return rc; }
+    HIPCHK(c, P.pin_out.reserve((size_t)n_views * 8 + 16));
+    (void)hipStreamWaitEvent(st, side.done, 0);
+    side.joined = true;
+    const float* med = P.pin_out.as<float>();
+    HIPCHK(c, hipMemcpyAsync(P.pin_out.p, P.median.p, (size_t)n_views * 8 + 4, hipMemcpyDeviceToHost, st));
     HIPCHK(c, hipStreamSynchronize(st));
     { hipError_t e_ = hipGetLastError(); if (e_ != hipSuccess) return fail(c, L3D_ERR_HIP, std::string("products: ") + hipGetErrorString(e_)); }
+    if (n_pot_pending) {
+        n_pot = reinterpret_cast<const int*>(med + 2 * n_views)[0];
+        if (n_pot < 0 || n_pot > n_pot_bound) return fail(c, L3D_ERR_INVALID, "products: " + std::to_string(n_pot) + " entries counted against a bound of " + std::to_string(n_pot_bound));
+    }
     P.n_pot = n_pot;
     if (held) {
         const long long r0 = dv0 >= dv1 ? (long long)nd + 1 : (long long)P.seg_base[(size_t)dv0], r1 = dv0 >= dv1 ? (long long)nd + 1 : (long long)P.seg_base[(size_t)dv1] + 1;
@@ -1114,7 +1247,7 @@
     }
     for (int k = 0; k < n_views; ++k) {
         l3d_chain_summary& s = summary[k];
-        s.verified = pvh[k].verified; s.n_kept = pvh[k].verified ? hres[k].n_kept : reinterpret_cast<const int*>(med.data() + n_views)[k];
+        s.verified = pvh[k].verified; s.n_kept = pvh[k].verified ? hres[k].n_kept : reinterpret_cast<const int*>(med + n_views)[k];
         s.n_candidates = pvh[k].verified ? hres[k].R : 0;
         s.median_depth = med[(size_t)k]; s.pad = 0;
     }
@@ -1309,6 +1442,14 @@
     return L3D_OK;
 }
 
+int l3d_products_report(l3d_ctx* c, int32_t* out)
+{
+    if (!c || !out) return L3D_ERR_INVALID;
+    const ProductsReport& rep = c->products.report;
+    out[0] = rep.build; out[1] = rep.refused; out[2] = rep.n_blocks; out[3] = rep.max_touch; out[4] = rep.planned_ahead; out[5] = rep.no_round_trip;
+    return L3D_OK;
+}
+
 int l3d_chain_products_get(l3d_ctx* c, int64_t* pot_start, int32_t* pot_tgt, l3d_match* best_match)
 {
     if (!c) return L3D_ERR_INVALID;
diff --git a/line3d_amd/csrc/l3d_products.hpp b/line3d_amd/csrc/l3d_products.hpp
--- a/line3d_amd/csrc/l3d_products.hpp
+++ b/line3d_amd/csrc/l3d_products.hpp
@@ -22,6 +22,7 @@
 int build_products(l3d_ctx* c, const l3d_chain_view* views, int n_views, const ProdChainView* pv, const ChainResult* hres,
                    const l3d_dense_map* map, l3d_chain_summary* summary, int64_t* n_pot, int dv0 = 0, int dv1 = -1, const char* held = nullptr,
                    const unsigned* qt_arena = nullptr, const ProdEarly* early = nullptr);
+void plan_products(l3d_ctx* c, const l3d_chain_view* views, int n_views, const ProdChainView* pv, const l3d_dense_map* map);
 
 struct EarlyView { const int* rt; const int* St; const int* boff_off; int k, S, N, pad; };
 void launch_early_transposes(l3d_ctx* c, const EarlyView* views_dev, int k0, int nb, int maxN, int maxSt, const ChainResult* res,
diff --git a/line3d_amd/csrc/l3d_sort.hip b/line3d_amd/csrc/l3d_sort.hip
--- a/line3d_amd/csrc/l3d_sort.hip
+++ b/line3d_amd/csrc/l3d_sort.hip
@@ -1,5 +1,7 @@
 #include "l3d_rocprim_arch.gen.hpp"
 #include <hipcub/hipcub.hpp>
+
+#include <stdint.h>
 
 #include "l3d_sort.hpp"
 #include "l3d_kernels.hpp"
@@ -107,6 +109,66 @@
     return hipGetLastError();
 }
 
+namespace {
+constexpr int kFrontThreads = 1024, kFrontTile = 4 * kFrontThreads;
+__global__ __launch_bounds__(kFrontThreads) void k_scan_front(const int* __restrict__ in, int n, int* __restrict__ out)
+{
+    __shared__ int s_f[kFrontThreads / 64], s_w[kFrontThreads / 64];
+    const int tid = threadIdx.x, lane = tid & 63, wave = tid >> 6;
+    const int base = (int)blockIdx.x * kFrontTile, i = base + tid * 4;
+    const bool vec_in = (reinterpret_cast<uintptr_t>(in) & 15) == 0, vec_out = (reinterpret_cast<uintptr_t>(out) & 15) == 0;
+    int4 v = make_int4(0, 0, 0, 0);
+    if (i + 3 < n && vec_in) v = *reinterpret_cast<const int4*>(in + i);
+    else {
+        if (i < n) v.x = in[i];
+        if (i + 1 < n) v.y = in[i + 1];
+        if (i + 2 < n) v.z = in[i + 2];
+        if (i + 3 < n) v.w = in[i + 3];
+    }
+    int f0 = 0, f1 = 0, f2 = 0, f3 = 0;
+    int j = tid * 4;
+    if (vec_in) {
+        for (; j + 3 * kFrontTile < base; j += 4 * kFrontTile) {
+            const int4 a = *reinterpret_cast<const int4*>(in + j), b = *reinterpret_cast<const int4*>(in + j + kFrontTile),
+                       c = *reinterpret_cast<const int4*>(in + j + 2 * kFrontTile), d = *reinterpret_cast<const int4*>(in + j + 3 * kFrontTile);
+            f0 += a.x + a.y + a.z + a.w; f1 += b.x + b.y + b.z + b.w; f2 += c.x + c.y + c.z + c.w; f3 += d.x + d.y + d.z + d.w;
+        }
+        for (; j < base; j += kFrontTile) { const int4 a = *reinterpret_cast<const int4*>(in + j); f0 += a.x + a.y + a.z + a.w; }
+    } else {
+        for (; j < base; j += kFrontTile) f0 += in[j] + in[j + 1] + in[j + 2] + in[j + 3];
+    }
+    int front = f0 + f1 + f2 + f3;
+    for (int o = 32; o > 0; o >>= 1) front += __shfl_down(front, o);
+    const int t = v.x + v.y + v.z + v.w;
+    int incl = t;
+    for (int o = 1; o < 64; o <<= 1) { const int u = __shfl_up(incl, o); if (lane >= o) incl += u; }
+    if (lane == 0) s_f[wave] = front;
+    if (lane == 63) s_w[wave] = incl;
+    __syncthreads();
+    int carry = 0, woff = 0, tile = 0;
+#pragma unroll
+    for (int w = 0; w < kFrontThreads / 64; ++w) { carry += s_f[w]; const int x = s_w[w]; tile += x; if (w < wave) woff += x; }
+    const int e0 = carry + woff + incl - t;
+    const int4 e = make_int4(e0, e0 + v.x, e0 + v.x + v.y, e0 + v.x + v.y + v.z);
+    if (i + 3 < n && vec_out) *reinterpret_cast<int4*>(out + i) = e;
+    else {
+        if (i < n) out[i] = e.x;
+        if (i + 1 < n) out[i + 1] = e.y;
+        if (i + 2 < n) out[i + 2] = e.z;
+        if (i + 3 < n) out[i + 3] = e.w;
+    }
+    if (base + kFrontTile >= n && tid == 0) out[n] = carry + tile;
+}
+}
+
+hipError_t exclusive_sum_int_front(const int* in, int* out, int n, hipStream_t st)
+{
+    if (n < 0 || n > kFrontScanMax) return hipErrorInvalidValue;
+    const int tiles = n > 0 ? (n + kFrontTile - 1) / kFrontTile : 1;
+    hipLaunchKernelGGL(k_scan_front, dim3((unsigned)tiles), dim3(kFrontThreads), 0, st, in, n, out);
+    return hipGetLastError();
+}
+
 __global__ void k_sort_touch() {}
 void warm_sort() { touch_kernel(reinterpret_cast<const void*>(&k_sort_touch)); }
 
diff --git a/line3d_amd/csrc/l3d_sort.hpp b/line3d_amd/csrc/l3d_sort.hpp
--- a/line3d_amd/csrc/l3d_sort.hpp
+++ b/line3d_amd/csrc/l3d_sort.hpp
@@ -12,5 +12,7 @@
                               int n, int begin_bit, int end_bit, hipStream_t st);
 hipError_t sort_keys_u64(void* tmp, size_t& bytes, const unsigned long long* keys_in, unsigned long long* keys_out, int n, int begin_bit, int end_bit, hipStream_t st);
 hipError_t exclusive_sum_int(void* tmp, size_t& bytes, const int* in, int* out, int n, hipStream_t st);
+constexpr int kFrontScanMax = 64 * 4096;
+hipError_t exclusive_sum_int_front(const int* in, int* out, int n, hipStream_t st);
 
 }
```

New measurement: 109.5 billion. 6.3% lower.
